# SociallyIneptWeeb/AICoverGen

Hardware: AMD Instinct MI355X
Metric: real-time factor (audio-sec/wall-sec) for MDX+RVC on 4-min 44.1 kHz track (higher is better)
Workload: dtype f32

## Files before the change

### aicovergen_amd/csrc/conv.hip

```cpp
#include <initializer_list>
#include "conv_ws3s.h"
#include "conv_ws3w.h"
#include "conv_w2d.h"
#include "conv_g1.h"
#include "conv_g1s.h"
#include "conv_g1w.h"
#ifdef AICG_DEV_SWITCHES
#include "conv_g1k.h"
#endif

namespace aicg {

#ifdef AICG_CONV_TRACE
__device__ unsigned long long g_conv_trace[kTraceWgs * kTraceSlots];
__device__ unsigned long long g_conv_trace2[kTrace2Wgs * 2 * 32 * 4];
#endif

template <bool FEW_IN>
__global__ void __launch_bounds__(256) conv_pointwise_kernel(ConvArgs p) {
    const long q = (long)blockIdx.x * 256 + threadIdx.x;
    const long per_img = (long)p.Ho * (p.Wo >> 2);
    if (q >= per_img) return;
    const int n = blockIdx.y;
    const int h = (int)(q / (p.Wo >> 2));
    const int w4 = (int)(q - (long)h * (p.Wo >> 2)) * 4;
    const float* xp = p.x + (long)n * p.x_sn + (long)h * p.x_sh + w4;
    float* yp = p.y + (long)n * p.y_sn + (long)h * p.y_sh + w4;
    const float* rp = p.res ? p.res + (long)n * p.r_sn + (long)h * p.r_sh + w4 : nullptr;
    auto finish = [&](float4 a, int co) __attribute__((always_inline)) {
        if (rp) {
            const float4 r = *reinterpret_cast<const float4*>(rp + (long)co * p.r_sc);
            if (p.res_first) { a.x += r.x; a.y += r.y; a.z += r.z; a.w += r.w; }
            a.x = apply_act(a.x, p.act, p.act_slope); a.y = apply_act(a.y, p.act, p.act_slope);
            a.z = apply_act(a.z, p.act, p.act_slope); a.w = apply_act(a.w, p.act, p.act_slope);
            if (!p.res_first) { a.x += r.x; a.y += r.y; a.z += r.z; a.w += r.w; }
        } else {
            a.x = apply_act(a.x, p.act, p.act_slope); a.y = apply_act(a.y, p.act, p.act_slope);
            a.z = apply_act(a.z, p.act, p.act_slope); a.w = apply_act(a.w, p.act, p.act_slope);
        }
        a.x *= p.out_scale; a.y *= p.out_scale; a.z *= p.out_scale; a.w *= p.out_scale;
        *reinterpret_cast<float4*>(yp + (long)co * p.y_sc) = a;
    };
    if (FEW_IN) {
        float4 xv[8];
#pragma unroll
        for (int ci = 0; ci < 8; ++ci)
            xv[ci] = ci < p.Cin_g ? *reinterpret_cast<const float4*>(xp + (long)ci * p.x_sc) : make_float4(0.f, 0.f, 0.f, 0.f);
        for (int co = 0; co < p.Cout_g; ++co) {
            const float b = p.bias ? p.bias[co] : 0.f;
            float4 a = make_float4(b, b, b, b);
#pragma unroll
            for (int ci = 0; ci < 8; ++ci) {
                if (ci < p.Cin_g) {
                    const float wv = p.w[ci * p.Mpad + co];
                    a.x += wv * xv[ci].x; a.y += wv * xv[ci].y; a.z += wv * xv[ci].z; a.w += wv * xv[ci].w;
                }
            }
            finish(a, co);
        }
    } else {
        float4 a[8];
#pragma unroll
        for (int co = 0; co < 8; ++co) {
            const float b = (p.bias && co < p.Cout_g) ? p.bias[co] : 0.f;
            a[co] = make_float4(b, b, b, b);
        }
        for (int ci = 0; ci < p.Cin_g; ++ci) {
            const float4 xv = *reinterpret_cast<const float4*>(xp + (long)ci * p.x_sc);
#pragma unroll
            for (int co = 0; co < 8; ++co) {
                if (co < p.Cout_g) {
                    const float wv = p.w[ci * p.Mpad + co];
                    a[co].x += wv * xv.x; a[co].y += wv * xv.y; a[co].z += wv * xv.z; a[co].w += wv * xv.w;
                }
            }
        }
#pragma unroll
        for (int co = 0; co < 8; ++co)
            if (co < p.Cout_g) finish(a[co], co);
    }
}

}

using namespace aicg;

#ifdef AICG_CONV_TRACE
extern "C" int aicg_conv_trace_read(unsigned long long* host, int clear) {
    (void)hipDeviceSynchronize();
    if (hipMemcpyFromSymbol(host, HIP_SYMBOL(g_conv_trace), sizeof(unsigned long long) * kTraceWgs * kTraceSlots) != hipSuccess)
        return fail(AICG_E_HIP, "trace copy failed");
    if (clear) { static unsigned long long z[kTraceWgs * kTraceSlots]; (void)hipMemcpyToSymbol(HIP_SYMBOL(g_conv_trace), z, sizeof(z)); }
    return AICG_OK;
}
extern "C" int aicg_conv_trace2_read(unsigned long long* host) {
    (void)hipDeviceSynchronize();
    if (hipMemcpyFromSymbol(host, HIP_SYMBOL(g_conv_trace2), sizeof(unsigned long long) * kTrace2Wgs * 2 * 32 * 4) != hipSuccess)
        return fail(AICG_E_HIP, "trace copy failed");
    return AICG_OK;
}
#endif

extern "C" int aicg_conv_bkc(int taps) {
    (void)taps;
    return 32;
}

extern "C" int aicg_conv_desc_size(void) { return (int)sizeof(aicg_conv_desc); }

namespace {

struct ConvCall {
    const aicg_conv_desc* d;
    int pad_h_end, pad_w_end;
    hipStream_t st;
};

typedef int (*run_fn)(ConvArgs&, hipStream_t);

int least_padded_bm(int M, std::initializer_list<int> cands) {
    int bm = 32;
    long best = 1L << 40;
    for (const int c : cands) {
        const long padded = (long)idiv_up(M, c) * c;
        if (padded < best) { best = padded; bm = c; }
    }
    return bm;
}

int validate_desc(const aicg_conv_desc* d, const float* x, const float* w_packed, const float* res, const float* y, ConvCall& c) {
    if (!d || !x || !w_packed || !y) return fail(AICG_E_ARG, "aicg_conv_forward: null pointer");
    if (d->groups < 1 || d->Cin % d->groups || d->Cout % d->groups)
        return fail(AICG_E_SHAPE, "aicg_conv_forward: channels not divisible by groups");
    if (d->KH < 1 || d->KW < 1 || d->stride_h < 1 || d->stride_w < 1 || d->dil_h < 1 || d->dil_w < 1)
        return fail(AICG_E_SHAPE, "aicg_conv_forward: bad kernel geometry");
    c.d = d;
    c.pad_h_end = d->pad_h_end < 0 ? d->pad_h : d->pad_h_end;
    c.pad_w_end = d->pad_w_end < 0 ? d->pad_w : d->pad_w_end;
    const int Ho = (d->H + d->pad_h + c.pad_h_end - d->dil_h * (d->KH - 1) - 1) / d->stride_h + 1;
    const int Wo = (d->W + d->pad_w + c.pad_w_end - d->dil_w * (d->KW - 1) - 1) / d->stride_w + 1;
    if (d->Ho > Ho || d->Wo > Wo || d->Ho < 0 || d->Wo < 0)
        return fail(AICG_E_SHAPE, "aicg_conv_forward: output %dx%d exceeds geometry (%dx%d)", d->Ho, d->Wo, Ho, Wo);
    if (d->N == 0 || d->Ho <= 0 || d->Wo <= 0) return AICG_OK;
    if (d->shuffle != 0 && (d->shuffle != 2 || d->Cout % 4 || d->groups != 1))
        return fail(AICG_E_ARG, "aicg_conv_forward: shuffle must be 0 or 2 (Cout %% 4 == 0, groups == 1)");
    if (d->res_mul && (!res || d->res_before_act)) return fail(AICG_E_ARG, "aicg_conv_forward: res_mul needs res and res_before_act == 0");
    return 1;
}

void fill_args(ConvArgs& p, const aicg_conv_desc* d, const float* x, const float* w_packed, const float* bias, const float* res, float* y) {
    p.stagger = p.stagger_first = p.wide_ok = 0;
    p.x = x; p.w = w_packed; p.bias = bias; p.res = res; p.y = y;
    p.N = d->N; p.Cin_g = d->Cin / d->groups; p.H = d->H; p.W = d->W; p.Cout_g = d->Cout / d->groups;
    p.Ho = d->Ho; p.Wo = d->Wo; p.KH = d->KH; p.KW = d->KW; p.sh = d->stride_h; p.sw = d->stride_w;
    p.ph = d->pad_h; p.pw = d->pad_w; p.dh = d->dil_h; p.dw = d->dil_w; p.groups = d->groups;
    p.x_sn = d->x_sn; p.x_sc = d->x_sc; p.x_sh = d->x_sh;
    p.y_sn = d->y_sn; p.y_sc = d->y_sc; p.y_sh = d->y_sh;
    p.r_sn = d->r_sn; p.r_sc = d->r_sc; p.r_sh = d->r_sh;
    p.pre_act = d->pre_act; p.pre_slope = d->pre_slope; p.act = d->act; p.act_slope = d->act_slope;
    p.out_scale = d->out_scale; p.accumulate = d->accumulate; p.res_first = d->res_before_act;
    p.shuffle = d->shuffle; p.res_mul = d->res_mul;
    p.taps = p.KH * p.KW;
    p.Mpad = idiv_up(p.Cout_g, 32) * 32;
    p.Cin_pad = idiv_up(p.Cin_g, 32) * 32;
    p.w_group_stride = (long)p.taps * p.Cin_pad * p.Mpad;
    p.w3 = d->packed_v3 ? w_packed + (long)p.groups * p.w_group_stride : nullptr;
    p.wsplit = d->packed_v3 && d->split == 1 ? w_packed + 2L * p.groups * p.w_group_stride : nullptr;
    p.f16 = d->split == 2;
}


int route_wino1d(ConvArgs& p, const ConvCall& c) {
    const aicg_conv_desc* d = c.d;
    if (d->wino != 8) return 1;
    if (!d->packed_v3 || (p.KW != 3 && p.KW != 5 && p.KW != 7 && p.KW != 11))
        return fail(AICG_E_ARG, "aicg_conv_forward: wino 8 needs a packed k = 3 / 5 / 7 / 11 one-dimensional layer");
    const int nslot = p.KW == 3 ? 4 : p.KW == 5 ? 7 : p.KW == 7 ? 10 : 15;
    p.w3 = p.w + (long)nslot * p.Cin_pad * p.Mpad;
    if (!conv_g1w_applicable(p, c.pad_w_end))
        return fail(AICG_E_ARG, "aicg_conv_forward: wino 8 needs stride 1, dilation 1 / 3 / 5, same padding, one group, W %% 4 == 0, 16-byte aligned "
                                "rows (strides %% 4 == 0), no input activation but a leaky ReLU");
    int rc;
    p.dbg = 0;
#ifdef AICG_DEV_SWITCHES
    p.dbg = d->gemm_tile == 7 ? 3 : 0;
    if (p.dw == 1 && d->gemm_tile == 2) rc = run_g1w_64x256(p, c.st);
    else if (p.dw == 1 && d->gemm_tile == 5) rc = run_g1w_32x512_sched(p, c.st);
    else if (p.dw == 1 && (d->gemm_tile == 6 || d->gemm_tile == 7)) rc = run_g1w_32x512_pers(p, c.st);
    else
#endif
        rc = p.f16 ? run_g1w_32x512_h(p, c.st) : run_g1w_32x512(p, c.st);
    if (rc == 1) return fail(AICG_E_SHAPE, "aicg_conv_forward: wino 8 layer does not fit the kernel's LDS budget");
    return rc;
}

int route_wino2d(ConvArgs& p, const ConvCall& c) {
    const aicg_conv_desc* d = c.d;
    AICG_SWITCH(w2d_ablate, "AICG_CONV_ABLATE", 0);
    p.dbg = w2d_ablate;
    p.w3 = p.w;
    if (w2d_ablate && (d->wino == 2 || d->wino == 12)) {
        const int ra = d->wino == 2 ? run_w2d_ablation(p, c.st, (int)w2d_ablate) : run_w2d_pairs_ablation(p, c.st, (int)w2d_ablate);
        if (ra != 1) return ra;
        return fail(AICG_E_ARG, "aicg_conv_forward: AICG_CONV_ABLATE=%ld is not an instantiated variant of conv_w2d (or not the dev library)", (long)w2d_ablate);
    }
#ifdef AICG_DEV_SWITCHES
    if (d->wino == 6) return run_w2d_ablation(p, c.st, 512);
    if (d->wino == 7) return run_w2d_ablation(p, c.st, 1024);
    if (d->wino == 9) return run_w2d_ablation(p, c.st, 2048);
    if (d->wino == 10) return run_w2d_ablation(p, c.st, 1);
    if (d->wino == 14) return run_w2d_pairs_ablation(p, c.st, 16384);
    if (d->wino == 15) return run_w2d_pairs_ablation(p, c.st, 65536);
    if (d->wino == 13) return run_w2d_pairs_ablation(p, c.st, 8192);
#endif
    const int rc = d->wino == 2 ? run_w2d_8(p, c.st) : d->wino == 3 ? run_w2d_4(p, c.st) : d->wino == 4 ? run_w2d_8q(p, c.st)
                 : d->wino == 12 ? run_w2d_8p(p, c.st) : d->wino == 16 ? run_w2d_4p2(p, c.st) : run_w2d_4q(p, c.st);
    if (rc == 1)
        return fail(AICG_E_ARG, "aicg_conv_forward: wino 2 needs Cout %% 48 == 0, W %% 4 == 0, 16-byte aligned x with strides %% 4 == 0");
    return rc;
}

int route_wino_rows(ConvArgs& p, const ConvCall& c) {
    AICG_SWITCH(wino_ablate, "AICG_CONV_ABLATE", 0);
    p.dbg = wino_ablate;
    p.taps = 12;
    p.w_group_stride = (long)p.taps * p.Cin_pad * p.Mpad;
    p.w3 = p.w + p.w_group_stride;
    const int M = p.Cout_g;
    AICG_SWITCH(wino_bm, "AICG_WINO_BM", 0);
    const int bm = wino_bm ? (int)wino_bm : least_padded_bm(M, {96, 64, 48, 32});
    auto run = [&](ConvArgs& a, int tile) {
        return tile == 96 ? run_ws3w_96(a, c.st) : tile == 64 ? run_ws3w_64(a, c.st) : tile == 48 ? run_ws3w_48(a, c.st) : run_ws3w_32(a, c.st);
    };
    int rc;
    AICG_SWITCH(wino_split, "AICG_WINO_SPLIT", 1);
    const long tiles4 = (long)p.N * idiv_up(p.Ho, 4) * idiv_up(p.Wo, 64);
    AICG_SWITCH(wino_split_tiles, "AICG_WINO_SPLIT_TILES", 1024);
    if (wino_split && !wino_bm && M > 48 && M % 96 == 48 && tiles4 >= wino_split_tiles) {
        ConvArgs a = p, b = p;
        a.Cout_g = M - 48;
        b.Cout_g = 48;
        if (b.bias) b.bias += M - 48;
        b.y += (long)(M - 48) * p.y_sc;
        b.w3 += (long)(M - 48) * 4;
        rc = run(a, 96);
        if (rc == 0) rc = run(b, 48);
    } else {
        rc = run(p, bm);
    }
    if (rc == 1) return fail(AICG_E_SHAPE, "aicg_conv_forward: wino layer too large for the kernel's 32-bit offsets");
    return rc;
}

int route_wino(ConvArgs& p, const ConvCall& c) {
    const aicg_conv_desc* d = c.d;
    if (!d->wino) return 1;
    if (p.KH != 3 || p.KW != 3 || p.sh != 1 || p.sw != 1 || p.dh != 1 || p.dw != 1 || p.ph != 1 || p.pw != 1 || c.pad_h_end != 1 ||
        c.pad_w_end != 1 || p.groups != 1 || p.res || p.accumulate || p.shuffle || p.res_mul || p.pre_act != AICG_ACT_NONE ||
        p.out_scale != 1.f || (!d->packed_v3 && d->wino < 2) || (p.act != AICG_ACT_NONE && p.act != AICG_ACT_RELU) || p.Ho != p.H || p.Wo != p.W)
        return fail(AICG_E_ARG, "aicg_conv_forward: wino needs a plain 3x3 / stride 1 / padding 1 layer (bias + none|ReLU epilogue)");
    return d->wino >= 2 ? route_wino2d(p, c) : route_wino_rows(p, c);
}


int route_pointwise(ConvArgs& p, const ConvCall& c) {
    AICG_SWITCH(pointwise, "AICG_CONV_POINTWISE", 1);
    const bool few_in = p.Cin_g <= 8, few_out = p.Cout_g <= 8;
    auto al4 = [](long v) { return (v & 3) == 0; };
    const bool aligned = (p.Wo & 3) == 0 && al4(p.x_sn) && al4(p.x_sc) && al4(p.x_sh) && al4(p.y_sn) && al4(p.y_sc) && al4(p.y_sh) &&
                         (!p.res || (al4(p.r_sn) && al4(p.r_sc) && al4(p.r_sh) && ((uintptr_t)p.res & 15) == 0)) &&
                         ((uintptr_t)p.x & 15) == 0 && ((uintptr_t)p.y & 15) == 0;
    if (!(pointwise && p.taps == 1 && p.groups == 1 && p.sh == 1 && p.sw == 1 && p.ph == 0 && p.pw == 0 && c.pad_h_end == 0 &&
          c.pad_w_end == 0 && (few_in || few_out) && p.Cin_g <= 512 && p.Cout_g <= 512 && p.pre_act == AICG_ACT_NONE &&
          !p.accumulate && aligned && p.Ho == p.H && p.Wo == p.W && !p.shuffle && !p.res_mul))
        return 1;
    const long per_img = (long)p.Ho * (p.Wo >> 2);
    dim3 grid((unsigned)ldiv_up(per_img, 256), (unsigned)p.N);
    if (few_in) hipLaunchKernelGGL(HIP_KERNEL_NAME(conv_pointwise_kernel<true>), grid, dim3(256), 0, c.st, p);
    else hipLaunchKernelGGL(HIP_KERNEL_NAME(conv_pointwise_kernel<false>), grid, dim3(256), 0, c.st, p);
    return check_launch("conv_pointwise_kernel");
}

int route_g1(ConvArgs& p, const ConvCall& c) {
    AICG_SWITCH(g1env, "AICG_CONV_G1", 0);
    const long g1 = c.d->gemm_tile ? c.d->gemm_tile : g1env;
    if (!(g1 != 1 && !p.wsplit && p.Cout_g > 32 && conv_g1_applicable(p, c.pad_h_end, c.pad_w_end))) return 1;
    const long HW = (long)p.H * p.W;
    const int M = p.Cout_g;
    auto wgs = [&](int bm) { return (long)p.N * idiv_up(M, bm) * ldiv_up(HW, 256); };
    if (p.f16 && !p.shuffle) {
        const long t64 = wgs(64), t128 = wgs(128);
        if (g1 == 3 || (g1 != 2 && ldiv_up(t64, 768) * 64 < ldiv_up(t128, 512) * 128)) return run_g1_64x256_h(p, c.st);
        return run_g1_128x256_h(p, c.st);
    }
    if (g1 == 2) return run_g1_128x256(p, c.st);
    if (g1 == 3) return run_g1_64x256(p, c.st);
    if (g1 == 4) return run_g1_192x256(p, c.st);
#ifdef AICG_DEV_SWITCHES
    if (g1 == 5) return run_g1_256x256(p, c.st);
    if (g1 == 6) return run_g1_128x512(p, c.st);
    if (g1 >= 12 && g1 <= 14) return run_g1_burst(p, c.st, (int)g1 - 10);
#endif
    if (wgs(64) < 256) return 1;
    auto cost = [&](int bm, double f) { return (double)ldiv_up(wgs(bm), 256) * bm * f; };
    const double c64 = cost(64, 1.04), c128 = cost(128, 1.0);
    const double c192 = (M % 192 == 0 && p.Cin_g >= 256) ? cost(192, 0.98) : 1e30;
    if (c192 <= c64 && c192 <= c128) return run_g1_192x256(p, c.st);
    if (c128 <= c64) return run_g1_128x256(p, c.st);
    return run_g1_64x256(p, c.st);
}

int route_g1s(ConvArgs& p, const ConvCall& c) {
    const int tile = c.d->gemm_tile;
    if (!(tile != 1 && !p.wsplit && p.Cout_g > 32 && conv_g1s_applicable(p, c.pad_w_end))) return 1;
    const long w64 = (long)p.N * idiv_up(p.Cout_g, 64) * idiv_up(p.Wo, 256);
    if (tile == 2) return run_g1s_128x256(p, c.st);
    if (tile == 3 || w64 >= 160) return run_g1s_64x256(p, c.st);
    return 1;
}

#ifdef AICG_DEV_SWITCHES
int route_g1k(ConvArgs& p, const ConvCall& c) {
    const int tile = c.d->gemm_tile;
    if (tile != 12 && tile != 13) return 1;
    if (!(!p.wsplit && p.Cout_g > 32 && conv_g1k_applicable(p, c.pad_w_end))) return 1;
    return tile == 12 ? run_g1k_128x256(p, c.st) : run_g1k_64x256(p, c.st);
}
#endif


struct TilePlan {
    int M, BM, groups;
    long npos, want;
    hipStream_t st;
    long blocks(int bm, int bn) const { return (long)idiv_up(M, bm) * groups * ldiv_up(npos, bn); }
    bool fills(int bm, int bn) const { return blocks(bm, bn) >= want; }
};

TilePlan plan_tiles(ConvArgs& p, const ConvCall& c) {
    TilePlan t;
    t.M = p.Cout_g;
    t.BM = least_padded_bm(t.M, {160, 128, 96, 64, 32});
    AICG_SWITCH(force_bm, "AICG_CONV_FORCE_BM", 0);
    if (force_bm) t.BM = (int)force_bm;
    t.groups = p.groups;
    t.npos = (long)p.N * p.Ho * p.Wo;
    t.st = c.st;
    AICG_SWITCH(ablate, "AICG_CONV_ABLATE", 0);
    p.dbg = ablate;
    AICG_SWITCH(want, "AICG_CONV_WANT", 512);
    t.want = want;
    return t;
}

int small_tiles(ConvArgs& p, const TilePlan& t, run_fn r64x64, run_fn r32x256, run_fn r32x128) {
    if (t.M > 32) return !t.fills(64, 128) && (t.fills(64, 64) || t.M > 64) ? r64x64(p, t.st) : 1;
    return t.fills(32, 256) ? r32x256(p, t.st) : r32x128(p, t.st);
}

int route_ws3s(ConvArgs& p, const TilePlan& t) {
    const int M = t.M;
    if (!(p.wsplit && p.Cin_g >= 16 && M > 16)) return 1;
    const int bm = least_padded_bm(M, {128, 96, 64, 32});
    int rc = 1;
    if (bm == 128 && t.fills(128, 128)) rc = run_ws3s_128x128(p, t.st);
    else if (bm == 96 && t.fills(96, 128)) rc = run_ws3s_96x128(p, t.st);
    else if (M > 32) {
        if (t.fills(64, 256)) rc = run_ws3s_64x256(p, t.st);
        if (rc == 1 && t.fills(64, 128)) rc = run_ws3s_64x128(p, t.st);
    }
    if (rc == 1) {
        rc = small_tiles(p, t, run_ws3s_64x64, run_ws3s_32x256, run_ws3s_32x128);
        if (rc == 1 && M <= 32 && t.fills(32, 256)) rc = run_ws3s_32x128(p, t.st);
    }
    return rc;
}

int route_m16(ConvArgs& p, const TilePlan& t) {
    const int M = t.M;
    AICG_SWITCH(use16, "AICG_CONV_M16", 1);
    if (!(use16 && t.npos >= 256L * 256)) return 1;
    const bool rows48 = M > 32 && M <= 48, rows16 = M <= 16;
    AICG_SWITCH(v3m16, "AICG_CONV_V3M16", 0);
#ifdef AICG_DEV_SWITCHES
    if (v3m16 && p.w3 && p.Cin_g >= 16) {
        const int rc = rows48 ? run_ws3m16_48(p, t.st) : rows16 ? run_ws3m16_16(p, t.st) : 1;
        if (rc <= 0) return rc;
    }
#else
    (void)v3m16;
#endif
    AICG_SWITCH(m16h, "AICG_CONV_M16H", 1);
    if (m16h && p.w3 && p.Cin_g >= 8) {
        const int rc = rows48 ? run_ws3m16h_48(p, t.st) : rows16 ? run_ws3m16h_16(p, t.st) : 1;
        if (rc <= 0) return rc;
    }
    if (p.Cin_g >= 3) return rows48 ? run_m16_48(p, t.st) : rows16 ? run_m16_16(p, t.st) : 1;
    return 1;
}

int route_ws3(ConvArgs& p, const TilePlan& t) {
    const int M = t.M, BM = t.BM;
    AICG_SWITCH(ws, "AICG_CONV_WS", 1);
    AICG_SWITCH(v3, "AICG_CONV_V3", 1);
    if (!(ws && v3 && p.w3 && p.Cin_g >= 8)) return 1;
    int rc = 1;
    AICG_SWITCH(v3_160, "AICG_CONV_V3_160", 1);
    if (BM == 160 && v3_160 && !p.shuffle && !p.res_mul && t.fills(160, 128)) rc = run_ws3_160x128(p, t.st);
    else if (BM == 128 && t.fills(128, 128)) rc = run_ws3_128x128(p, t.st);
    else if (BM == 96 && t.fills(96, 128)) rc = run_ws3_96x128(p, t.st);
    else if (BM != 160 && M > 32 && t.fills(64, 128)) rc = run_ws3_64x128(p, t.st);
    if (rc == 1 && BM != 160) rc = small_tiles(p, t, run_ws3_64x64, run_ws3_32x256, run_ws3_32x128);
    return rc;
}

int route_ws(ConvArgs& p, const TilePlan& t) {
    const int M = t.M, BM = t.BM;
    AICG_SWITCH(ws, "AICG_CONV_WS", 1);
    if (!ws) return 1;
    int rc = 1;
    AICG_SWITCH(v2, "AICG_CONV_V2", 0);
#ifdef AICG_DEV_SWITCHES
    if (v2 & 1) { if (BM == 128 && t.fills(128, 128)) rc = run_ws_128x128_k32(p, t.st); }
    if (rc == 1 && (v2 & 2)) { if (M > 32 && M <= 64 && t.fills(64, 256)) rc = run_ws_64x256(p, t.st); }
    if (rc == 1 && (v2 & 4)) { if (M <= 32 && t.fills(32, 512)) rc = run_ws_32x512(p, t.st); }
    if (rc <= 0) return rc;
#else
    (void)v2;
#endif
    if (BM == 160 && t.fills(160, 128)) rc = run_ws_160x128(p, t.st);
    else if (BM == 128 && t.fills(128, 128)) {
        AICG_SWITCH(bm128e, "AICG_CONV_BM128", 0);
        const bool use64 = bm128e ? bm128e == 64 : M >= 256;
        rc = use64 ? run_ws_64x128(p, t.st) : run_ws_128x128(p, t.st);
    }
    else if (BM == 96 && t.fills(96, 128)) rc = run_ws_96x128(p, t.st);
    else if (M > 32 && t.fills(64, 128)) rc = run_ws_64x128(p, t.st);
    if (rc <= 0) return rc;
    AICG_SWITCH(smallws, "AICG_CONV_SMALLWS", 1);
    return smallws ? small_tiles(p, t, run_ws_64x64, run_ws_32x256, run_ws_32x128) : 1;
}

int route_single_role(ConvArgs& p, const TilePlan& t) {
    const int M = t.M, BM = t.BM;
    AICG_SWITCH(eight, "AICG_CONV_8WAVE", 1);
    auto tile = [&]() -> int {
        if (BM == 160 && t.fills(160, 128)) return run_sr_160x128(p, t.st);
#ifdef AICG_DEV_SWITCHES
        if (BM == 128 && t.fills(128, 128) && !eight) return run_sr_128x128_4w(p, t.st);
#else
        (void)eight;
#endif
        if (BM == 128 && t.fills(128, 128)) return run_sr_128x128_8w(p, t.st);
        if (BM == 96 && t.fills(96, 128)) return run_sr_96x128(p, t.st);
        if (M > 32) {
            if (t.fills(64, 128)) return run_sr_64x128(p, t.st);
            if (t.fills(64, 64) || M > 64) return run_sr_64x64(p, t.st);
        }
        if (t.fills(32, 256)) return run_sr_32x256(p, t.st);
        return run_sr_32x128(p, t.st);
    };
    int rc = tile();
    if (rc == AICG_E_LDS) rc = run_sr_64x64(p, t.st);
    return rc;
}

}

extern "C" int aicg_conv_forward(const aicg_conv_desc* d, const float* x, const float* w_packed, const float* bias,
                                 const float* res, float* y, void* stream) {
    ConvCall c;
    int rc = validate_desc(d, x, w_packed, res, y, c);
    if (rc <= 0) return rc;
    c.st = (hipStream_t)stream;
    ConvArgs p;
    fill_args(p, d, x, w_packed, bias, res, y);
    if ((rc = route_wino1d(p, c)) != 1) return rc;
    if ((rc = route_wino(p, c)) != 1) return rc;
    if ((rc = route_pointwise(p, c)) != 1) return rc;
    if ((rc = route_g1(p, c)) != 1) return rc;
    if ((rc = route_g1s(p, c)) != 1) return rc;
#ifdef AICG_DEV_SWITCHES
    if ((rc = route_g1k(p, c)) != 1) return rc;
#endif
    const TilePlan t = plan_tiles(p, c);
    if ((rc = route_ws3s(p, t)) != 1) return rc;
    if ((rc = route_m16(p, t)) != 1) return rc;
    if ((rc = route_ws3(p, t)) != 1) return rc;
    if ((rc = route_ws(p, t)) != 1) return rc;
    return route_single_role(p, t);
}
```

### aicovergen_amd/csrc/elementwise.hip

```cpp
#include "common.h"

#include <cstdint>

namespace aicg {

struct Col2imArgs {
    const float* cols;
    const float* bias;
    const float* add;
    float* out;
    int N, Cout, Hi, Wi, Ho, Wo, KH, KW, sh, sw, ph, pw, act;
    float slope;
    long o_sn, o_sc, o_sh, a_sn, a_sc, a_sh;
};

__global__ void __launch_bounds__(256) col2im_kernel(Col2imArgs p) {
    const long total = (long)p.N * p.Cout * p.Ho * p.Wo;
    const long plane = (long)p.Hi * p.Wi;
    for (long i = (long)blockIdx.x * blockDim.x + threadIdx.x; i < total; i += (long)gridDim.x * blockDim.x) {
        const int wo = (int)(i % p.Wo);
        long t = i / p.Wo;
        const int ho = (int)(t % p.Ho);
        t /= p.Ho;
        const int co = (int)(t % p.Cout);
        const int n = (int)(t / p.Cout);
        float acc = p.bias ? p.bias[co] : 0.f;
        const float* cn = p.cols + (long)n * p.Cout * p.KH * p.KW * plane;
        for (int kh = (ho + p.ph) % p.sh; kh < p.KH; kh += p.sh) {
            const int hi = (ho + p.ph - kh) / p.sh;
            if (ho + p.ph - kh < 0) break;
            if (hi >= p.Hi) continue;
            for (int kw = (wo + p.pw) % p.sw; kw < p.KW; kw += p.sw) {
                const int wi = (wo + p.pw - kw) / p.sw;
                if (wo + p.pw - kw < 0) break;
                if (wi >= p.Wi) continue;
                acc += cn[((long)(co * p.KH + kh) * p.KW + kw) * plane + (long)hi * p.Wi + wi];
            }
        }
        acc = apply_act(acc, p.act, p.slope);
        if (p.add) acc += p.add[(long)n * p.a_sn + (long)co * p.a_sc + (long)ho * p.a_sh + wo];
        p.out[(long)n * p.o_sn + (long)co * p.o_sc + (long)ho * p.o_sh + wo] = acc;
    }
}

template <int S>
__global__ void __launch_bounds__(256) col2im1d_kernel(Col2imArgs p, int J) {
    HIP_DYNAMIC_SHARED(float, c2i_tile)
    const int s = S > 0 ? S : p.sw;
    const int co = blockIdx.y, n = blockIdx.z, tid = threadIdx.x;
    const int q0 = blockIdx.x * 256, q = q0 + tid;
    const float* cn = p.cols + ((long)n * p.Cout + co) * p.KW * (long)p.Wi;
    const float b = p.bias ? p.bias[co] : 0.f;
#pragma unroll 2
    for (int r = 0; r < s; ++r) {
        float acc = b;
        for (int j = 0; j < J; ++j) {
            const int kk = r + s * j, qi = q - j;
            if (kk < p.KW && qi >= 0 && qi < p.Wi) acc += cn[(long)kk * p.Wi + qi];
        }
        c2i_tile[tid * s + r] = apply_act(acc, p.act, p.slope);
    }
    __syncthreads();
    const long nbase = (long)s * q0 - p.pw;
    float* orow = p.out + (long)n * p.o_sn + (long)co * p.o_sc;
    const float* arow = p.add ? p.add + (long)n * p.a_sn + (long)co * p.a_sc : nullptr;
    for (int i = tid; i < 256 * s; i += 256) {
        const long no = nbase + i;
        if (no >= 0 && no < p.Wo) orow[no] = c2i_tile[i] + (arow ? arow[no] : 0.f);
    }
}

__global__ void __launch_bounds__(256) sine_frame_prefix_kernel(const float* __restrict__ f0, double* __restrict__ prefix,
                                                                int T, int upp, float sr) {
    __shared__ double part[256];
    const int tid = threadIdx.x;
    const int per = (T + 255) / 256;
    const int t0 = tid * per, t1 = imin(T, t0 + per);
    double s = 0.0;
    for (int t = t0; t < t1; ++t) {
        const float rad = fmodf(f0[t] / sr, 1.0f);
        s += (double)rad * (double)upp;
        s -= floor(s);
    }
    part[tid] = s;
    __syncthreads();
    if (tid == 0) {
        double run = 0.0;
        for (int i = 0; i < 256; ++i) {
            const double v = part[i];
            part[i] = run;
            run += v;
            run -= floor(run);
        }
    }
    __syncthreads();
    double run = part[tid];
    for (int t = t0; t < t1; ++t) {
        prefix[t] = run;
        const float rad = fmodf(f0[t] / sr, 1.0f);
        run += (double)rad * (double)upp;
        run -= floor(run);
    }
}

__global__ void __launch_bounds__(256) sine_source4_kernel(const float* __restrict__ f0, const double* __restrict__ prefix,
                                                           const float* __restrict__ noise, float* __restrict__ out,
                                                           int T, int upp, float sr, float sine_amp, float noise_std,
                                                           float lin_w, float lin_b) {
    const int q_per = upp >> 2;
    const long total4 = (long)T * q_per;
    for (long n4 = (long)blockIdx.x * blockDim.x + threadIdx.x; n4 < total4; n4 += (long)gridDim.x * blockDim.x) {
        const int t = (int)(n4 / q_per);
        const int i0 = (int)(n4 - (long)t * q_per) * 4;
        const float f = f0[t];
        const float rad = fmodf(f / sr, 1.0f);
        const double base = prefix[t];
        const float uv = f > 0.f ? 1.f : 0.f;
        const float namp = uv * noise_std + (1.f - uv) * sine_amp / 3.f;
        const float4 nz = *reinterpret_cast<const float4*>(noise + (long)t * upp + i0);
        const float nv[4] = {nz.x, nz.y, nz.z, nz.w};
        float o[4];
#pragma unroll
        for (int j = 0; j < 4; ++j) {
            double ph = base + (double)(i0 + j + 1) * (double)rad;
            ph -= floor(ph);
            const float sine = sinf((float)(ph * 6.283185307179586476925)) * sine_amp;
            const float v = sine * uv + namp * nv[j];
            o[j] = tanhf(lin_w * v + lin_b);
        }
        *reinterpret_cast<float4*>(out + (long)t * upp + i0) = make_float4(o[0], o[1], o[2], o[3]);
    }
}

__global__ void __launch_bounds__(256) sine_source_kernel(const float* __restrict__ f0, const double* __restrict__ prefix,
                                                          const float* __restrict__ noise, float* __restrict__ out,
                                                          int T, int upp, float sr, float sine_amp, float noise_std,
                                                          float lin_w, float lin_b) {
    const long total = (long)T * upp;
    for (long n = (long)blockIdx.x * blockDim.x + threadIdx.x; n < total; n += (long)gridDim.x * blockDim.x) {
        const int t = (int)(n / upp);
        const int i = (int)(n - (long)t * upp);
        const float f = f0[t];
        const float rad = fmodf(f / sr, 1.0f);
        double ph = prefix[t] + (double)(i + 1) * (double)rad;
        ph -= floor(ph);
        const float sine = sinf((float)(ph * 6.283185307179586476925)) * sine_amp;
        const float uv = f > 0.f ? 1.f : 0.f;
        const float namp = uv * noise_std + (1.f - uv) * sine_amp / 3.f;
        const float v = sine * uv + namp * noise[n];
        out[n] = tanhf(lin_w * v + lin_b);
    }
}

__global__ void __launch_bounds__(256) gate_kernel(const float* __restrict__ a, float* __restrict__ out, int N, int C,
                                                   long T) {
    const long total = (long)N * C * T;
    for (long i = (long)blockIdx.x * blockDim.x + threadIdx.x; i < total; i += (long)gridDim.x * blockDim.x) {
        const long t = i % T;
        const long nc = i / T;
        const int c = (int)(nc % C);
        const long n = nc / C;
        const float ta = a[(n * 2 * C + c) * T + t];
        const float sa = a[(n * 2 * C + C + c) * T + t];
        out[i] = tanhf(ta) * (1.f / (1.f + expf(-sa)));
    }
}

__global__ void __launch_bounds__(256) prior_sample_kernel(const float* __restrict__ stats, const float* __restrict__ noise,
                                                           float* __restrict__ out, int C, long T, float scale) {
    const long total = (long)C * T;
    for (long i = (long)blockIdx.x * blockDim.x + threadIdx.x; i < total; i += (long)gridDim.x * blockDim.x) {
        const float m = stats[i], logs = stats[total + i];
        out[i] = m + expf(logs) * noise[i] * scale;
    }
}

__global__ void __launch_bounds__(256) feats_prepare_kernel(const float* __restrict__ feats, const float* __restrict__ feats0,
                                                            const float* __restrict__ pitchf, float* __restrict__ out,
                                                            int Th, int C, int T, float protect) {
    __shared__ float tile[32][33];
    const int t0 = blockIdx.x * 32, c0 = blockIdx.y * 32;
    const int tx = threadIdx.x & 31, ty = threadIdx.x >> 5;
    for (int r = ty; r < 32; r += 8) {
        const int t = t0 + r, c = c0 + tx;
        float v = 0.f;
        if (t < T && c < C) {
            const int th = imin(t >> 1, Th - 1);
            v = feats[(long)th * C + c];
            if (feats0) {
                const float f = pitchf[t];
                float pf = f;
                if (f > 0.f) pf = 1.f;
                if (f < 1.f) pf = protect;
                v = v * pf + feats0[(long)th * C + c] * (1.f - pf);
            }
        }
        tile[r][tx] = v;
    }
    __syncthreads();
    for (int r = ty; r < 32; r += 8) {
        const int c = c0 + r, t = t0 + tx;
        if (c < C && t < T) out[(long)c * T + t] = tile[tx][r];
    }
}

static unsigned ew_grid(long total) { return (unsigned)lmax(1, lmin((total + 255) / 256, 256L * 16)); }

}

using namespace aicg;

extern "C" int aicg_col2im(const float* cols, const float* bias, const float* add, float* out, int N, int Cout, int Hi,
                           int Wi, int Ho, int Wo, int KH, int KW, int stride_h, int stride_w, int pad_h, int pad_w,
                           int act, float slope, int64_t o_sn, int64_t o_sc, int64_t o_sh, int64_t a_sn, int64_t a_sc,
                           int64_t a_sh, void* stream) {
    if (!cols || !out) return fail(AICG_E_ARG, "aicg_col2im: null pointer");
    if (KH < 1 || KW < 1 || stride_h < 1 || stride_w < 1) return fail(AICG_E_SHAPE, "aicg_col2im: bad geometry");
    const long total = (long)N * Cout * Ho * Wo;
    if (total == 0) return AICG_OK;
    Col2imArgs p{cols, bias, add, out, N, Cout, Hi, Wi, Ho, Wo, KH, KW, stride_h, stride_w, pad_h, pad_w, act, slope,
                 (long)o_sn, (long)o_sc, (long)o_sh, (long)a_sn, (long)a_sc, (long)a_sh};
    if (Hi == 1 && Ho == 1 && KH == 1 && stride_h == 1 && pad_h == 0 && Cout <= 65535 && N <= 65535 && stride_w <= 32) {
        const int J = (KW + stride_w - 1) / stride_w;
        const long nq = ((long)Wo + pad_w + stride_w - 1) / stride_w + 1;
        dim3 grid((unsigned)ldiv_up(nq, 256), (unsigned)Cout, (unsigned)N);
        const size_t lds = (size_t)256 * stride_w * sizeof(float);
        if (stride_w == 2) hipLaunchKernelGGL(HIP_KERNEL_NAME(col2im1d_kernel<2>), grid, dim3(256), lds, (hipStream_t)stream, p, J);
        else if (stride_w == 10) hipLaunchKernelGGL(HIP_KERNEL_NAME(col2im1d_kernel<10>), grid, dim3(256), lds, (hipStream_t)stream, p, J);
        else hipLaunchKernelGGL(HIP_KERNEL_NAME(col2im1d_kernel<0>), grid, dim3(256), lds, (hipStream_t)stream, p, J);
        return check_launch("col2im1d_kernel");
    }
    hipLaunchKernelGGL(col2im_kernel, dim3(ew_grid(total)), dim3(256), 0, (hipStream_t)stream, p);
    return check_launch("col2im_kernel");
}

extern "C" int aicg_sine_source(const float* f0, const float* noise, double* prefix_scratch, float* out, int T, int upp,
                                float sr, float sine_amp, float noise_std, float lin_w, float lin_b, void* stream) {
    if (!f0 || !noise || !prefix_scratch || !out) return fail(AICG_E_ARG, "aicg_sine_source: null pointer");
    if (T < 0 || upp < 1) return fail(AICG_E_SHAPE, "aicg_sine_source: bad shape");
    if (T == 0) return AICG_OK;
    hipLaunchKernelGGL(sine_frame_prefix_kernel, dim3(1), dim3(256), 0, (hipStream_t)stream, f0, prefix_scratch, T, upp, sr);
    if ((upp & 3) == 0 && ((uintptr_t)noise & 15) == 0 && ((uintptr_t)out & 15) == 0)
        hipLaunchKernelGGL(sine_source4_kernel, dim3(ew_grid((long)T * (upp >> 2))), dim3(256), 0, (hipStream_t)stream, f0,
                           (const double*)prefix_scratch, noise, out, T, upp, sr, sine_amp, noise_std, lin_w, lin_b);
    else
        hipLaunchKernelGGL(sine_source_kernel, dim3(ew_grid((long)T * upp)), dim3(256), 0, (hipStream_t)stream, f0,
                           (const double*)prefix_scratch, noise, out, T, upp, sr, sine_amp, noise_std, lin_w, lin_b);
    return check_launch("sine_source_kernel");
}

extern "C" int aicg_gate_tanh_sigmoid(const float* a, float* out, int N, int C, int64_t T, void* stream) {
    if (!a || !out) return fail(AICG_E_ARG, "aicg_gate_tanh_sigmoid: null pointer");
    const long total = (long)N * C * T;
    if (total == 0) return AICG_OK;
    hipLaunchKernelGGL(gate_kernel, dim3(ew_grid(total)), dim3(256), 0, (hipStream_t)stream, a, out, N, C, (long)T);
    return check_launch("gate_kernel");
}

extern "C" int aicg_prior_sample(const float* stats, const float* noise, float* out, int C, int64_t T, float scale,
                                 void* stream) {
    if (!stats || !noise || !out) return fail(AICG_E_ARG, "aicg_prior_sample: null pointer");
    if ((long)C * T == 0) return AICG_OK;
    hipLaunchKernelGGL(prior_sample_kernel, dim3(ew_grid((long)C * T)), dim3(256), 0, (hipStream_t)stream, stats, noise,
                       out, C, (long)T, scale);
    return check_launch("prior_sample_kernel");
}

extern "C" int aicg_feats_prepare(const float* feats, const float* feats0, const float* pitchf, float* out, int Th, int C,
                                  int T, float protect, void* stream) {
    if (!feats || !out || (feats0 && !pitchf)) return fail(AICG_E_ARG, "aicg_feats_prepare: null pointer");
    if (T > 2 * Th) return fail(AICG_E_SHAPE, "aicg_feats_prepare: T=%d exceeds 2*Th=%d", T, 2 * Th);
    if (T == 0 || C == 0) return AICG_OK;
    dim3 grid((unsigned)idiv_up(T, 32), (unsigned)idiv_up(C, 32));
    hipLaunchKernelGGL(feats_prepare_kernel, grid, dim3(256), 0, (hipStream_t)stream, feats, feats0, pitchf, out, Th, C, T,
                       protect);
    return check_launch("feats_prepare_kernel");
}

namespace aicg {
__global__ void __launch_bounds__(256) mul_kernel(const float* __restrict__ a, const float* __restrict__ b, float* __restrict__ out, long n) {
    for (long i = (long)blockIdx.x * blockDim.x + threadIdx.x; i < n; i += (long)gridDim.x * blockDim.x) out[i] = a[i] * b[i];
}
__global__ void __launch_bounds__(256) axpbypcz_kernel(const float* __restrict__ a, float alpha, const float* __restrict__ b,
                                                       float beta, const float* __restrict__ c, float gamma,
                                                       float* __restrict__ out, long n) {
    for (long i = (long)blockIdx.x * blockDim.x + threadIdx.x; i < n; i += (long)gridDim.x * blockDim.x) {
        float v = alpha * a[i];
        if (b) v += beta * b[i];
        if (c) v += gamma * c[i];
        out[i] = v;
    }
}
}

extern "C" int aicg_mul(const float* a, const float* b, float* out, int64_t n, void* stream) {
    if (!a || !b || !out) return aicg::fail(AICG_E_ARG, "aicg_mul: null pointer");
    if (n == 0) return AICG_OK;
    hipLaunchKernelGGL(aicg::mul_kernel, dim3(aicg::ew_grid(n)), dim3(256), 0, (hipStream_t)stream, a, b, out, (long)n);
    return aicg::check_launch("mul_kernel");
}

extern "C" int aicg_axpbypcz(const float* a, float alpha, const float* b, float beta, const float* c, float gamma, float* out,
                             int64_t n, void* stream) {
    if (!a || !out) return aicg::fail(AICG_E_ARG, "aicg_axpbypcz: null pointer");
    if (n == 0) return AICG_OK;
    hipLaunchKernelGGL(aicg::axpbypcz_kernel, dim3(aicg::ew_grid(n)), dim3(256), 0, (hipStream_t)stream, a, alpha, b, beta, c,
                       gamma, out, (long)n);
    return aicg::check_launch("axpbypcz_kernel");
}

namespace aicg {
__global__ void __launch_bounds__(256) frame_normalize_kernel(const float* __restrict__ x, float* __restrict__ out, int L) {
    __shared__ float sh[4];
    const float* xr = x + (long)blockIdx.x * L;
    float s = 0.f;
    for (int i = threadIdx.x; i < L; i += 256) s += xr[i];
    for (int o = 32; o > 0; o >>= 1) s += __shfl_xor(s, o);
    if ((threadIdx.x & 63) == 0) sh[threadIdx.x >> 6] = s;
    __syncthreads();
    const float mean = (sh[0] + sh[1] + sh[2] + sh[3]) / (float)L;
    __syncthreads();
    float v = 0.f;
    for (int i = threadIdx.x; i < L; i += 256) { const float d = xr[i] - mean; v += d * d; }
    for (int o = 32; o > 0; o >>= 1) v += __shfl_xor(v, o);
    if ((threadIdx.x & 63) == 0) sh[threadIdx.x >> 6] = v;
    __syncthreads();
    const float sd = fmaxf(1e-10f, sqrtf((sh[0] + sh[1] + sh[2] + sh[3]) / (float)(L - 1)));
    float* orow = out + (long)blockIdx.x * L;
    for (int i = threadIdx.x; i < L; i += 256) orow[i] = (xr[i] - mean) / sd;
}

__global__ void __launch_bounds__(256) affine_maxpool2_kernel(const float* __restrict__ x, const float* __restrict__ scale,
                                                              const float* __restrict__ shift, float* __restrict__ out, int C,
                                                              int Wo, long total) {
    for (long i = (long)blockIdx.x * blockDim.x + threadIdx.x; i < total; i += (long)gridDim.x * blockDim.x) {
        const int c = (int)((i / Wo) % C);
        const float s = scale[c], t = shift[c];
        const float a = x[2 * i] * s + t, b = x[2 * i + 1] * s + t;
        out[i] = fmaxf(a, b);
    }
}
}

extern "C" int aicg_frame_normalize(const float* x, float* out, int64_t n_frames, int frame_len, void* stream) {
    if (!x || !out) return aicg::fail(AICG_E_ARG, "aicg_frame_normalize: null pointer");
    if (frame_len < 2) return aicg::fail(AICG_E_SHAPE, "aicg_frame_normalize: frame too short");
    if (n_frames <= 0) return AICG_OK;
    hipLaunchKernelGGL(aicg::frame_normalize_kernel, dim3((unsigned)n_frames), dim3(256), 0, (hipStream_t)stream, x, out, frame_len);
    return aicg::check_launch("frame_normalize_kernel");
}

extern "C" int aicg_affine_maxpool2(const float* x, const float* scale, const float* shift, float* out, int N, int C, int W,
                                    void* stream) {
    if (!x || !scale || !shift || !out) return aicg::fail(AICG_E_ARG, "aicg_affine_maxpool2: null pointer");
    if (W & 1) return aicg::fail(AICG_E_SHAPE, "aicg_affine_maxpool2: W must be even");
    const long total = (long)N * C * (W / 2);
    if (total == 0) return AICG_OK;
    hipLaunchKernelGGL(aicg::affine_maxpool2_kernel, dim3(aicg::ew_grid(total)), dim3(256), 0, (hipStream_t)stream, x, scale, shift,
                       out, C, W / 2, total);
    return aicg::check_launch("affine_maxpool2_kernel");
}
```

### aicovergen_amd/infer_pack/models.py

```python
import contextlib
import math
import os
from collections import namedtuple

import numpy as np
import torch
from .. import _env
import torch.nn.functional as F

from .. import ops

_Incompatible = namedtuple("IncompatibleKeys", ["missing_keys", "unexpected_keys"])
LRELU_SLOPE = 0.1

sr2sr = {"32k": 32000, "40k": 40000, "48k": 48000}


def _fold_weight_norm(sd, name):
    if name + ".weight" in sd:
        return sd[name + ".weight"].float()
    v, g = sd[name + ".weight_v"].float(), sd[name + ".weight_g"].float()
    return v * (g / v.flatten(1).norm(dim=1).view(-1, *([1] * (v.dim() - 1))))


class _SynthesizerBase:
    phone_dim = 768
    use_f0 = True

    def __init__(self, spec_channels, segment_size, inter_channels, hidden_channels, filter_channels, n_heads,
                 n_layers, kernel_size, p_dropout, resblock, resblock_kernel_sizes, resblock_dilation_sizes,
                 upsample_rates, upsample_initial_channel, upsample_kernel_sizes, spk_embed_dim, gin_channels, sr=None,
                 **kwargs):
        if isinstance(sr, str):
            sr = sr2sr[sr]
        self.spec_channels, self.segment_size = spec_channels, segment_size
        self.inter_channels, self.hidden_channels, self.filter_channels = inter_channels, hidden_channels, filter_channels
        self.n_heads, self.n_layers, self.kernel_size, self.p_dropout = n_heads, n_layers, kernel_size, p_dropout
        self.resblock = str(resblock)
        self.resblock_kernel_sizes = list(resblock_kernel_sizes)
        self.resblock_dilation_sizes = [list(d) for d in resblock_dilation_sizes]
        self.upsample_rates = list(upsample_rates)
        self.upsample_initial_channel = upsample_initial_channel
        self.upsample_kernel_sizes = list(upsample_kernel_sizes)
        self.spk_embed_dim, self.gin_channels = spk_embed_dim, gin_channels
        self.sr = sr
        self.upp = int(np.prod(self.upsample_rates))
        self.is_half = bool(kwargs.get("is_half", False))
        self.enc_q = None
        self.device = torch.device("cpu")
        self._sd = None
        self._p = None
        assert kernel_size % 2 == 1, "FFN same-padding is symmetric only for odd kernels"
        print("gin_channels:", gin_channels, "self.spk_embed_dim:", self.spk_embed_dim)

    def load_state_dict(self, state_dict, strict=True):
        self._sd = {k: v.detach().to("cpu") for k, v in state_dict.items() if not k.startswith("enc_q.")}
        self._p = None
        unexpected = [k for k in state_dict if k.startswith("enc_q.")] if strict else []
        return _Incompatible([], unexpected)

    def eval(self):
        return self

    def to(self, device):
        self.device = torch.device(device)
        self._p = None
        return self

    def half(self):
        self._half = ops.half_requested()
        if self._p is not None:
            ops.mark_half(self._p, self._half)
        return self

    def float(self):
        self._half = False
        if self._p is not None:
            ops.mark_half(self._p, False)
        return self

    def remove_weight_norm(self):
        return None

    def _prepare(self):
        if self._p is not None:
            return self._p
        assert self._sd is not None, "load_state_dict() first"
        sd, dev = self._sd, self.device
        P = {}
        H, C = self.n_heads, self.hidden_channels
        dk = C // H
        P["emb_phone"] = ops.PackedConv(sd["enc_p.emb_phone.weight"].float(), sd["enc_p.emb_phone.bias"], device=dev)
        if self.use_f0:
            P["emb_pitch"] = sd["enc_p.emb_pitch.weight"].float().to(dev)
        layers = []
        for i in range(self.n_layers):
            a = "enc_p.encoder.attn_layers.%d." % i
            L = {}
            L["q"] = ops.PackedConv(sd[a + "conv_q.weight"].float(), sd[a + "conv_q.bias"], device=dev)
            L["kv"] = ops.PackedConv(torch.cat([sd[a + "conv_k.weight"], sd[a + "conv_v.weight"]], 0).float(),
                                     torch.cat([sd[a + "conv_k.bias"], sd[a + "conv_v.bias"]], 0), device=dev)
            ek = sd[a + "emb_rel_k"].float()
            ev = sd[a + "emb_rel_v"].float()
            assert ek.shape[0] == 1, "heads_share=True is the only configuration the reference instantiates"
            self.window = (ek.shape[1] - 1) // 2
            L["relk"] = ops.PackedConv(ek[0].repeat(H, 1).unsqueeze(-1).contiguous(), None, groups=H, device=dev)
            L["relv"] = ev[0].contiguous().to(dev)
            L["o"] = ops.PackedConv(sd[a + "conv_o.weight"].float(), sd[a + "conv_o.bias"], device=dev)
            for n in (1, 2):
                L["g%d" % n] = sd["enc_p.encoder.norm_layers_%d.%d.gamma" % (n, i)].float().to(dev)
                L["b%d" % n] = sd["enc_p.encoder.norm_layers_%d.%d.beta" % (n, i)].float().to(dev)
            f = "enc_p.encoder.ffn_layers.%d." % i
            pad = (self.kernel_size - 1) // 2
            L["ffn1"] = ops.PackedConv(sd[f + "conv_1.weight"].float(), sd[f + "conv_1.bias"], padding=pad, device=dev)
            L["ffn2"] = ops.PackedConv(sd[f + "conv_2.weight"].float(), sd[f + "conv_2.bias"], padding=pad, device=dev)
            layers.append(L)
        P["enc_layers"] = layers
        P["proj"] = ops.PackedConv(sd["enc_p.proj.weight"].float(), sd["enc_p.proj.bias"], device=dev)
        P["emb_g"] = sd["emb_g.weight"].float().to(dev)
        flows = {}
        for fidx in (0, 2, 4, 6):
            p = "flow.flows.%d." % fidx
            Fl = {"pre": ops.PackedConv(sd[p + "pre.weight"].float(), sd[p + "pre.bias"], device=dev)}
            n_wn = 0
            while (p + "enc.in_layers.%d.weight_v" % n_wn) in sd or (p + "enc.in_layers.%d.weight" % n_wn) in sd:
                n_wn += 1
            Fl["n_wn"] = n_wn
            in_bias = []
            for l in range(n_wn):
                w = _fold_weight_norm(sd, p + "enc.in_layers.%d" % l)
                Fl["in%d" % l] = ops.PackedConv(w, None, padding=(w.shape[2] - 1) // 2, device=dev)
                in_bias.append(sd[p + "enc.in_layers.%d.bias" % l].float())
                rs_w = _fold_weight_norm(sd, p + "enc.res_skip_layers.%d" % l)
                rs_b = sd[p + "enc.res_skip_layers.%d.bias" % l].float()
                if l < n_wn - 1:
                    Fl["res%d" % l] = ops.PackedConv(rs_w[:C], rs_b[:C], device=dev)
                    Fl["skip%d" % l] = ops.PackedConv(rs_w[C:], rs_b[C:], device=dev)
                else:
                    Fl["skip%d" % l] = ops.PackedConv(rs_w, rs_b, device=dev)
            Fl["cond"] = ops.PackedConv(_fold_weight_norm(sd, p + "enc.cond_layer"), sd[p + "enc.cond_layer.bias"], device=dev)
            Fl["in_bias"] = torch.cat(in_bias).view(1, -1, 1).contiguous().to(dev)
            Fl["post_neg"] = ops.PackedConv(-sd[p + "post.weight"].float(), -sd[p + "post.bias"].float(), device=dev)
            flows[fidx] = Fl
        P["flows"] = flows
        up_init = self.upsample_initial_channel
        P["conv_pre"] = ops.PackedConv(sd["dec.conv_pre.weight"].float(), None, padding=3, device=dev)
        P["conv_pre_bias"] = sd["dec.conv_pre.bias"].float().view(1, -1, 1).contiguous().to(dev)
        P["cond"] = ops.PackedConv(sd["dec.cond.weight"].float(), sd["dec.cond.bias"], device=dev)
        ups, noise = [], []
        for i, (u, k) in enumerate(zip(self.upsample_rates, self.upsample_kernel_sizes)):
            ups.append(ops.PackedConvTranspose(_fold_weight_norm(sd, "dec.ups.%d" % i), sd["dec.ups.%d.bias" % i], stride=u,
                                               padding=(k - u) // 2, device=dev))
            if self.use_f0:
                w, b = sd["dec.noise_convs.%d.weight" % i].float(), sd["dec.noise_convs.%d.bias" % i]
                cc = w.shape[0]
                if i + 1 < len(self.upsample_rates):
                    s = int(np.prod(self.upsample_rates[i + 1:]))
                    assert w.shape[2] == 2 * s
                    w2 = w.view(cc, 2, s).permute(0, 2, 1).contiguous()
                    noise.append((s, ops.PackedConv(w2, b, device=dev)))
                else:
                    noise.append((1, ops.PackedConv(w, b, device=dev)))
        P["ups"], P["noise"] = ups, noise
        rbs = []
        nres = len(self.upsample_rates) * len(self.resblock_kernel_sizes)
        for j in range(nres):
            k = self.resblock_kernel_sizes[j % len(self.resblock_kernel_sizes)]
            dil = self.resblock_dilation_sizes[j % len(self.resblock_kernel_sizes)]
            r = "dec.resblocks.%d." % j
            convs = []
            if self.resblock == "1":
                for m, d in enumerate(dil):
                    c1 = ops.PackedConv(_fold_weight_norm(sd, r + "convs1.%d" % m), sd[r + "convs1.%d.bias" % m], dilation=d,
                                        padding=(k * d - d) // 2, device=dev)
                    c2 = ops.PackedConv(_fold_weight_norm(sd, r + "convs2.%d" % m), sd[r + "convs2.%d.bias" % m],
                                        padding=(k - 1) // 2, device=dev)
                    convs.append((c1, c2))
            else:
                for m, d in enumerate(dil):
                    convs.append((ops.PackedConv(_fold_weight_norm(sd, r + "convs.%d" % m), sd[r + "convs.%d.bias" % m],
                                                 dilation=d, padding=(k * d - d) // 2, device=dev), None))
            rbs.append(convs)
        P["resblocks"] = rbs
        P["conv_post"] = ops.PackedConv(sd["dec.conv_post.weight"].float(), None, padding=3, device=dev)
        if self.use_f0:
            P["lin_w"] = float(sd["dec.m_source.l_linear.weight"].reshape(-1)[0])
            P["lin_b"] = float(sd["dec.m_source.l_linear.bias"].reshape(-1)[0])
        if getattr(self, "_half", False):
            ops.mark_half(P, True)
        self._p = P
        return P

    def _enc_p(self, P, phone_ct, pitch):
        C, H = self.hidden_channels, self.n_heads
        dk = C // H
        T = phone_ct.shape[2]
        res = None
        if pitch is not None:
            res = P["emb_pitch"][pitch[0]].t().contiguous().unsqueeze(0)
        x = ops.conv(phone_ct, P["emb_phone"], res=res, res_before_act=True, act=ops.ACT_LRELU, act_slope=0.1,
                     out_scale=math.sqrt(C))
        for L in P["enc_layers"]:
            q = ops.conv(x, L["q"], out_scale=1.0 / math.sqrt(dk))
            kv = ops.conv(x, L["kv"])
            relk = ops.conv(q, L["relk"])
            o = ops.attention(q[0], kv[0, :C], kv[0, C:], H, relk=relk[0].view(H, 2 * self.window + 1, T),
                              relv_emb=L["relv"], window=self.window)
            y = ops.conv(o.unsqueeze(0), L["o"])
            x = ops.layernorm_ct(x, L["g1"], L["b1"], res=y)
            y = ops.conv(x, L["ffn1"], act=ops.ACT_RELU)
            y = ops.conv(y, L["ffn2"])
            x = ops.layernorm_ct(x, L["g2"], L["b2"], res=y)
        return ops.conv(x, P["proj"])

    def _flow_reverse(self, P, z, g):
        C = self.hidden_channels
        half = self.inter_channels // 2
        for fidx in (6, 4, 2, 0):
            Fl = P["flows"][fidx]
            z = torch.flip(z, [1])
            x0, x1 = z[:, :half], z[:, half:]
            h = ops.conv(x0, Fl["pre"])
            bias_all = ops.conv(g, Fl["cond"], res=Fl["in_bias"])
            out = None
            for l in range(Fl["n_wn"]):
                a = ops.conv(h, Fl["in%d" % l], bias=bias_all[0, 2 * C * l: 2 * C * (l + 1), 0].contiguous())
                acts = ops.gate_tanh_sigmoid(a)
                if l < Fl["n_wn"] - 1:
                    if out is None:
                        out = ops.conv(acts, Fl["skip%d" % l])
                    else:
                        ops.conv(acts, Fl["skip%d" % l], out=out, accumulate=True)
                    ops.conv(acts, Fl["res%d" % l], res=h, out=h)
                else:
                    if out is None:
                        out = ops.conv(acts, Fl["skip%d" % l])
                    else:
                        ops.conv(acts, Fl["skip%d" % l], out=out, accumulate=True)
            ops.conv(out, Fl["post_neg"], res=x1, out=x1)
        return z

    def _decoder(self, P, x, f0, g, noise_src):
        T = x.shape[2]
        har = None
        if self.use_f0:
            if noise_src is None:
                noise_src = torch.randn(T * self.upp, device=x.device)
            har = ops.sine_source(f0.reshape(-1)[:T], noise_src.to(x.device).reshape(-1), self.upp, float(self.sr), P["lin_w"], P["lin_b"])
        pre_bias = ops.conv(g, P["cond"], res=P["conv_pre_bias"])
        x = ops.conv(x, P["conv_pre"], bias=pre_bias.reshape(-1))
        nk = len(self.resblock_kernel_sizes)
        for i, pt in enumerate(P["ups"]):
            add = None
            if har is not None:
                s, nc = P["noise"][i]
                L = har.numel()
                if s > 1:
                    xp = F.pad(har, (s // 2, s // 2))
                    phases = xp.view(L // s + 1, s).t().contiguous()
                    add = ops.conv(phases.unsqueeze(0), nc)
                else:
                    add = ops.conv(har.view(1, 1, L), nc)
            x = ops.conv_transpose(x, pt, add=add, pre_act=ops.ACT_LRELU, pre_slope=LRELU_SLOPE)
            acc = torch.empty_like(x)
            streams = self._rb_streams(x.device, nk)
            main = torch.cuda.current_stream(x.device) if streams else None
            bufs = [tuple(torch.empty_like(x) for _ in range(3)) for _ in range(nk if streams else 1)]
            if streams:
                ready = torch.cuda.Event()
                ready.record(main)
            prev_acc = None
            for j in range(nk):
                convs = P["resblocks"][i * nk + j]
                st = streams[j - 1] if (streams and j > 0) else main
                if streams and j > 0:
                    st.wait_event(ready)
                with (torch.cuda.stream(st) if streams else contextlib.nullcontext()):
                    tmp, ya, yb = bufs[j] if streams else bufs[0]
                    y = x
                    for m, (c1, c2) in enumerate(convs):
                        last = m == len(convs) - 1
                        if c2 is None:
                            src = c1
                            inp = y
                        else:
                            ops.conv(y, c1, out=tmp, pre_act=ops.ACT_LRELU, pre_slope=LRELU_SLOPE, act=ops.ACT_LRELU, act_slope=LRELU_SLOPE)
                            src, inp = c2, tmp
                        if last:
                            if streams and prev_acc is not None:
                                st.wait_event(prev_acc)
                            pre = ops.ACT_NONE if c2 is not None else ops.ACT_LRELU
                            ops.conv(inp, src, res=y, out=acc, pre_act=pre, pre_slope=LRELU_SLOPE, out_scale=1.0 / nk, accumulate=j > 0)
                            if streams:
                                prev_acc = torch.cuda.Event()
                                prev_acc.record(st)
                        else:
                            dst = ya if y is not ya else yb
                            ops.conv(inp, src, res=y, out=dst, pre_act=ops.ACT_NONE if c2 is not None else ops.ACT_LRELU, pre_slope=LRELU_SLOPE)
                            y = dst
            if streams:
                main.wait_event(prev_acc)
            x = acc
        return ops.conv(x, P["conv_post"], pre_act=ops.ACT_LRELU, pre_slope=0.01, act=ops.ACT_TANH)

    def _rb_streams(self, device, nk):
        if device.type != "cuda" or nk < 2 or _env.dev("AICG_RB_STREAMS", "0") != "1":
            return None
        have = getattr(self, "_rb_side", None)
        if have is None or len(have) != nk - 1:
            have = self._rb_side = [torch.cuda.Stream(device=device) for _ in range(nk - 1)]
        return have

    def infer(self, phone, phone_lengths, pitch=None, nsff0=None, sid=None, max_len=None, noise_z=None, noise_src=None,
              phone_ct=None):
        if not self.use_f0 and sid is None:
            sid, pitch = pitch, None
        P = self._prepare()
        dev = self.device
        if phone_ct is None:
            phone = phone.to(dev).float()
            assert phone.shape[0] == 1, "batch 1 (the reference pipeline never batches chunks)"
            T = phone.shape[1]
            phone_ct = phone[0].t().contiguous().unsqueeze(0)
        else:
            T = phone_ct.shape[2]
        front = self.infer_front(phone_ct, pitch, sid, noise_z)
        return self.infer_back(front, nsff0, noise_src, max_len)

    def infer_front(self, phone_ct, pitch, sid, noise_z=None):
        P = self._prepare()
        dev = self.device
        T = phone_ct.shape[2]
        g = P["emb_g"][sid.to(dev).reshape(-1)[:1]].unsqueeze(-1).contiguous()
        stats = self._enc_p(P, phone_ct, None if pitch is None else pitch.to(dev))
        if noise_z is None:
            noise_z = torch.randn((1, self.inter_channels, T), device=dev)
        z_p = ops.prior_sample(stats, noise_z.to(dev).float().contiguous(), 0.66666)
        z = self._flow_reverse(P, z_p.clone(), g)
        return {"z": z, "z_p": z_p, "stats": stats, "g": g, "T": T}

    def infer_back(self, front, nsff0=None, noise_src=None, max_len=None):
        P = self._prepare()
        dev = self.device
        z, z_p, stats, g, T = front["z"], front["z_p"], front["stats"], front["g"], front["T"]
        zz = z if max_len is None else z[:, :, :max_len].contiguous()
        o = self._decoder(P, zz, None if nsff0 is None else nsff0.to(dev).float(), g, noise_src)
        x_mask = torch.ones((1, 1, T), dtype=torch.float32, device=dev)
        m_p, logs_p = stats[:, : self.inter_channels], stats[:, self.inter_channels:]
        return o, x_mask, (z, z_p, m_p, logs_p)


class SynthesizerTrnMs768NSFsid(_SynthesizerBase):
    phone_dim, use_f0 = 768, True


class SynthesizerTrnMs256NSFsid(_SynthesizerBase):
    phone_dim, use_f0 = 256, True


class SynthesizerTrnMs768NSFsid_nono(_SynthesizerBase):
    phone_dim, use_f0 = 768, False


class SynthesizerTrnMs256NSFsid_nono(_SynthesizerBase):
    phone_dim, use_f0 = 256, False
```

### aicovergen_amd/ops.py

```python
import contextlib
import functools
import math
import os
import threading

import numpy as np
import torch
from . import _env

from . import _lib


def _ptr(t):
    return 0 if t is None else t.data_ptr()


def _stream(t):
    if t.is_cuda:
        return torch.cuda.current_stream(t.device).cuda_stream
    return 0


_tls = threading.local()


def _check(*tensors):
    be = _lib.backend()
    dev = None
    for t in tensors:
        if t is None:
            continue
        if be == "hip" and not t.is_cuda:
            raise RuntimeError("aicovergen_amd: tensor on %s, but the HIP kernels need device memory" % t.device)
        if be == "emu" and t.is_cuda:
            raise RuntimeError("emulator backend needs host tensors")
        if t.is_cuda:
            if dev is None:
                dev = t.device.index
            elif dev != t.device.index:
                raise RuntimeError("aicovergen_amd: operands on different devices (cuda:%d and cuda:%d)" % (dev, t.device.index))
    _tls.dev = dev


def _call(name, *args):
    dev = getattr(_tls, "dev", None)
    if dev is not None and dev != torch.cuda.current_device():
        with torch.cuda.device(dev):
            return _lib.call(name, *args)
    return _lib.call(name, *args)


_fft_tables = {}


def fft_tables(n_fft, device, window=None):
    key = (n_fft, str(device))
    if key not in _fft_tables:
        m = n_fft // 2
        k = np.arange(m, dtype=np.float64)
        th = np.exp(-2j * np.pi * k / m)
        k2 = np.arange(m + 1, dtype=np.float64)
        tf = np.exp(-2j * np.pi * k2 / n_fft)
        tw_half = torch.from_numpy(np.stack([th.real, th.imag], -1).astype(np.float32)).contiguous().to(device)
        tw_full = torch.from_numpy(np.stack([tf.real, tf.imag], -1).astype(np.float32)).contiguous().to(device)
        hann = torch.hann_window(n_fft, periodic=True, dtype=torch.float32).to(device)
        _fft_tables[key] = (hann, tw_half, tw_full)
    hann, tw_half, tw_full = _fft_tables[key]
    if window is None:
        window = hann
    return window, tw_half, tw_full


def stft(x, n_fft, hop, n_bins_out=None, frame_major=False, window=None):
    assert x.dim() == 2 and x.dtype == torch.float32
    x = x.contiguous()
    n_sig, L = x.shape
    n_frames = 1 + L // hop
    nb = n_fft // 2 + 1 if n_bins_out is None else n_bins_out
    window, tw_half, tw_full = fft_tables(n_fft, x.device, window)
    _check(x, window)
    if frame_major:
        out = torch.empty((n_sig, 2, n_frames, nb), dtype=torch.float32, device=x.device)
        o_bin, o_frame = 1, nb
    else:
        out = torch.empty((n_sig, 2, nb, n_frames), dtype=torch.float32, device=x.device)
        o_bin, o_frame = n_frames, 1
    _call("aicg_stft", _ptr(x), _ptr(out), _ptr(window), _ptr(tw_half), _ptr(tw_full), n_sig, L, n_fft, hop,
              n_frames, nb, 2 * nb * n_frames, nb * n_frames, o_bin, o_frame, _stream(x))
    return out


def istft(spec, n_fft, hop, length, frame_major=False, window=None):
    assert spec.dim() == 4 and spec.shape[1] == 2 and spec.dtype == torch.float32
    spec = spec.contiguous()
    n_sig = spec.shape[0]
    if frame_major:
        n_frames, nb = spec.shape[2], spec.shape[3]
        i_bin, i_frame = 1, nb
    else:
        nb, n_frames = spec.shape[2], spec.shape[3]
        i_bin, i_frame = n_frames, 1
    window, tw_half, tw_full = fft_tables(n_fft, spec.device, window)
    _check(spec, window)
    frames = torch.empty((n_sig, n_frames, n_fft), dtype=torch.float32, device=spec.device)
    out = torch.empty((n_sig, length), dtype=torch.float32, device=spec.device)
    st = _stream(spec)
    _call("aicg_istft_frames", _ptr(spec), _ptr(frames), _ptr(window), _ptr(tw_half), _ptr(tw_full), n_sig,
              n_fft, n_frames, nb, 2 * nb * n_frames, nb * n_frames, i_bin, i_frame, st)
    _call("aicg_istft_ola", _ptr(frames), _ptr(window), _ptr(out), n_sig, length, n_fft, hop, n_frames, st)
    return out


import ctypes

ACT_NONE, ACT_RELU, ACT_LRELU, ACT_GELU, ACT_TANH, ACT_SIGMOID = 0, 1, 2, 3, 4, 5


class ConvDesc(ctypes.Structure):
    _fields_ = [(n, ctypes.c_int32) for n in
                ("N", "Cin", "H", "W", "Cout", "Ho", "Wo", "KH", "KW", "stride_h", "stride_w", "pad_h", "pad_w",
                 "dil_h", "dil_w", "groups")] + \
               [(n, ctypes.c_int64) for n in ("x_sn", "x_sc", "x_sh", "y_sn", "y_sc", "y_sh", "r_sn", "r_sc", "r_sh")] + \
               [("pre_act", ctypes.c_int32), ("pre_slope", ctypes.c_float), ("act", ctypes.c_int32),
                ("act_slope", ctypes.c_float), ("out_scale", ctypes.c_float), ("accumulate", ctypes.c_int32),
                ("res_before_act", ctypes.c_int32), ("pad_h_end", ctypes.c_int32), ("pad_w_end", ctypes.c_int32),
                ("shuffle", ctypes.c_int32), ("res_mul", ctypes.c_int32), ("packed_v3", ctypes.c_int32),
                ("split", ctypes.c_int32), ("wino", ctypes.c_int32), ("gemm_tile", ctypes.c_int32)]


def conv_bkc(taps):
    return _lib.get().aicg_conv_bkc(int(taps))


split_precision = os.environ.get("AICG_PRECISION", "fp32").lower() in ("bf16x3", "split")


def half_requested():
    return os.environ.get("AICG_HALF", "0") == "1"


def mark_half(tree, on=True):
    if isinstance(tree, PackedConv):
        tree.f16 = bool(on) and not tree.fp32_only and not tree.split
    elif isinstance(tree, PackedConvTranspose):
        mark_half(tree.gemm, on)
    elif isinstance(tree, dict):
        for v in tree.values():
            mark_half(v, on)
    elif isinstance(tree, (list, tuple)):
        for v in tree:
            mark_half(v, on)


_fp32_depth = 0


@contextlib.contextmanager
def fp32_layers():
    global split_precision, _fp32_depth
    old, split_precision = split_precision, False
    _fp32_depth += 1
    try:
        yield
    finally:
        split_precision = old
        _fp32_depth -= 1


def fp32_only(fn):
    @functools.wraps(fn)
    def wrapped(*a, **k):
        with fp32_layers():
            return fn(*a, **k)
    return wrapped


def _split_image(out):
    g, taps, cpad, mpad = out.shape
    hi = out.to(torch.bfloat16)
    lo = (out - hi.to(torch.float32)).to(torch.bfloat16)
    both = torch.stack([hi, lo], 0)
    both = both.reshape(2, g, taps, cpad // 16, 2, 8, mpad).permute(1, 2, 3, 0, 4, 6, 5).contiguous()
    return both.view(torch.int16).reshape(-1).view(torch.float32)


def pack_conv_weight(w, groups=1, split=False):
    w = w.detach().to(torch.float32)
    cout, cin_g, kh, kw = w.shape
    taps = kh * kw
    cpad = (cin_g + 31) // 32 * 32
    cout_g = cout // groups
    mpad = (cout_g + 31) // 32 * 32
    out = torch.zeros((groups, taps, cpad, mpad), dtype=torch.float32, device=w.device)
    out[:, :, :cin_g, :cout_g] = w.reshape(groups, cout_g, cin_g, taps).permute(0, 3, 2, 1)
    v3 = out.reshape(groups, taps, cpad // 8, 4, 2, mpad).permute(0, 1, 2, 4, 5, 3)
    parts = [out.reshape(-1), v3.reshape(-1)]
    if split:
        parts.append(_split_image(out))
    return torch.cat(parts).contiguous()


winograd = _env.dev("AICG_WINOGRAD", "1") != "0"
winograd_min_positions = 32768


def winograd_kernel(w):
    g0, g1, g2 = w[..., 0], w[..., 1], w[..., 2]
    return torch.stack([g0, (g0 + g1 + g2) * 0.5, (g0 - g1 + g2) * 0.5, g2], -1).contiguous()


winograd2d = _env.dev("AICG_WINOGRAD", "2") == "2"
winograd2d_waves = int(_env.dev("AICG_W2D_WAVES", "8"))


winograd2d_code = int(_env.dev("AICG_W2D_CODE", "0"))
winograd2d_quads = _env.dev("AICG_W2D_QUADS", "0") == "1"
winograd2d_pairs = _env.dev("AICG_W2D_PAIRS", "1") != "0"


def _w2d_code():
    code = winograd2d_code or ((4 if winograd2d_quads else 12 if winograd2d_pairs else 2) if winograd2d_waves == 8
                               else (5 if winograd2d_quads else 3))
    return code, ("pairs" if code in (12, 13, 14, 15, 16) else "quads" if code in (4, 5) else "dword")


def winograd2d_image(w, quads=False, pairs=False):
    co, ci = w.shape[:2]
    assert co % 48 == 0 and tuple(w.shape[2:]) == (3, 3)
    G = torch.tensor([[1.0, 0.0, 0.0], [0.5, 0.5, 0.5], [0.5, -0.5, 0.5], [0.0, 0.0, 1.0]], dtype=torch.float64, device=w.device)
    U = torch.einsum("ia,ocab,jb->ocij", G, w.double(), G).to(torch.float32)
    cpad = (ci + 7) // 8 * 8
    Up = torch.zeros((co, cpad, 16), dtype=torch.float32, device=w.device)
    Up[:, :ci] = U.reshape(co, ci, 16)
    if quads:
        return Up.view(co // 48, 48, cpad // 8, 2, 4, 4, 4).permute(0, 2, 3, 5, 4, 1, 6).contiguous().view(-1)
    if pairs:
        return Up.view(co // 48, 48, cpad // 8, 2, 4, 8, 2).permute(0, 2, 3, 5, 4, 1, 6).contiguous().view(-1)
    return Up.view(co // 48, 48, cpad // 8, 2, 4, 16).permute(0, 2, 3, 5, 4, 1).contiguous().view(-1)


winograd1d = _env.dev("AICG_WINOGRAD1D", "1") != "0"
winograd1d_min_positions = int(_env.dev("AICG_WINOGRAD1D_MIN", "16384"))


def winograd1d_kernel(w):
    k = w.shape[-1]
    assert k in (3, 5, 7, 11)
    wd = w.detach().double()
    slots = []
    for g in range(k // 3):
        g0, g1, g2 = wd[..., 3 * g], wd[..., 3 * g + 1], wd[..., 3 * g + 2]
        slots += [g0, (g0 + g1 + g2) * 0.5, (g0 - g1 + g2) * 0.5, g2]
    if k % 3 == 2:
        a, b = wd[..., k - 2], wd[..., k - 1]
        slots += [a, a + b, b]
    elif k % 3 == 1:
        a = wd[..., k - 1]
        slots += [a, -a]
    return torch.stack(slots, -1).to(torch.float32).contiguous()


class PackedConv:

    def __init__(self, weight, bias=None, stride=1, padding=0, dilation=1, groups=1, device=None, padding_end=None):
        self.padding_end = None if padding_end is None else (0, _one(padding_end)) if weight.dim() == 3 else _pair(padding_end)
        if weight.dim() == 3:
            weight = weight.unsqueeze(2)
            stride, padding, dilation = (1, _one(stride)), (0, _one(padding)), (1, _one(dilation))
        elif weight.dim() == 2:
            weight = weight[:, :, None, None]
            stride, padding, dilation = (1, 1), (0, 0), (1, 1)
        else:
            stride, padding, dilation = _pair(stride), _pair(padding), _pair(dilation)
        self.cout, cin_g, self.kh, self.kw = weight.shape
        self.cin = cin_g * groups
        self.groups = groups
        self.stride, self.padding, self.dilation = stride, padding, dilation
        device = weight.device if device is None else device
        self.split = bool(split_precision)
        self.fp32_only = _fp32_depth > 0
        self.f16 = False
        self.w = pack_conv_weight(weight.to(device), groups, self.split)
        self.bias = None if bias is None else bias.detach().to(device=device, dtype=torch.float32).contiguous()
        self.w_wino = self.w_wino2 = self.w_wino1 = None
        if (winograd1d and not self.split and not _fp32_depth and self.kh == 1 and self.kw in (3, 5, 7, 11) and stride == (1, 1)
                and dilation[1] in ((1, 3, 5) if self.kw != 5 else (1,)) and padding == (0, (self.kw - 1) // 2 * dilation[1]) and self.padding_end is None
                and groups == 1 and cin_g >= 16):
            self.w_wino1 = pack_conv_weight(winograd1d_kernel(weight.detach().to(device=device, dtype=torch.float32)[:, :, 0]).unsqueeze(2), 1, False)
        if (winograd and not self.split and not _fp32_depth and (self.kh, self.kw) == (3, 3) and stride == (1, 1) and dilation == (1, 1)
                and padding == (1, 1) and self.padding_end is None and groups == 1 and cin_g >= 8):
            self.w_wino = pack_conv_weight(winograd_kernel(weight.detach().to(device=device, dtype=torch.float32)), 1, False)
            if winograd2d and self.cout % 48 == 0:
                self._wino2_src, self._wino2_dev, self._wino2_images = weight.detach(), device, {}
                self.w_wino2 = self.wino2_image(_w2d_code()[1])

    def wino2_image(self, kind):
        if kind not in self._wino2_images:
            self._wino2_images[kind] = winograd2d_image(self._wino2_src.to(device=self._wino2_dev, dtype=torch.float32),
                                                         quads=kind == "quads", pairs=kind == "pairs")
        return self._wino2_images[kind]

    def wino2q(self):
        return self.wino2_image("quads")

    def out_hw(self, h, w):
        pe = self.padding if self.padding_end is None else self.padding_end
        ho = (h + self.padding[0] + pe[0] - self.dilation[0] * (self.kh - 1) - 1) // self.stride[0] + 1
        wo = (w + self.padding[1] + pe[1] - self.dilation[1] * (self.kw - 1) - 1) // self.stride[1] + 1
        return ho, wo


def _one(v):
    return int(v[0]) if isinstance(v, (tuple, list)) else int(v)


def _pair(v):
    return (int(v[0]), int(v[1])) if isinstance(v, (tuple, list)) else (int(v), int(v))


def _as4d(t):
    return t.unsqueeze(2) if t.dim() == 3 else t


class ConvProfile:

    def __init__(self):
        self.events = []
        self.flops = 0.0
        self.flops_executed = 0.0
        self.bytes = 0.0
        self.launches = 0
        self.shapes = []

    def by_shape(self):
        torch.cuda.synchronize()
        agg = {}
        for (key, fl), (a, b) in zip(self.shapes, self.events):
            r = agg.setdefault(key, [0, 0.0, 0.0])
            r[0] += 1
            r[1] += a.elapsed_time(b)
            r[2] += fl
        rows = [{"shape": k, "launches": v[0], "ms": v[1], "gflop": v[2] / 1e9, "tflops": v[2] / (v[1] * 1e-3) / 1e12 if v[1] > 0 else 0.0}
                for k, v in agg.items()]
        return sorted(rows, key=lambda r: -r["ms"])

    def summary(self):
        torch.cuda.synchronize()
        ms = sum(a.elapsed_time(b) for a, b in self.events)
        return {"launches": self.launches, "flops": self.flops, "flops_executed": self.flops_executed, "ms": ms, "bytes": self.bytes,
                "tflops": (self.flops / (ms * 1e-3) / 1e12) if ms > 0 else 0.0,
                "tflops_executed": (self.flops_executed / (ms * 1e-3) / 1e12) if ms > 0 else 0.0}


conv_profile = None

gemm_tile = 0


def conv(x, pc, res=None, out=None, pre_act=ACT_NONE, pre_slope=0.0, act=ACT_NONE, act_slope=0.0, out_scale=1.0,
         accumulate=False, bias=None, res_before_act=False, out_len=None, shuffle=0, res_mul=False):
    is1d = x.dim() == 3
    x4 = _as4d(x)
    n, c, h, w = x4.shape
    assert c == pc.cin, "conv: input has %d channels, layer expects %d" % (c, pc.cin)
    assert x4.stride(3) == 1 or w == 1
    assert h == 1 or c == 1 or x4.stride(1) >= x4.stride(2) * (h - 1) + w, "conv: input rows must lie inside the channel stride"
    ho, wo = pc.out_hw(h, w)
    if out_len is not None:
        assert out_len <= wo
        wo = out_len
    oshape = (n, pc.cout // 4, 2 * ho, 2 * wo) if shuffle else (n, pc.cout, ho, wo)
    if out is None:
        out = torch.empty((n, pc.cout, wo) if is1d else oshape, dtype=torch.float32, device=x.device)
        assert not accumulate
    o4 = _as4d(out)
    assert o4.shape == oshape, (o4.shape, oshape)
    assert o4.stride(3) == 1 or wo == 1
    r4 = None
    if res is not None:
        r4 = _as4d(res)
        assert r4.shape == o4.shape and (r4.stride(3) == 1 or wo == 1)
    b = pc.bias if bias is None else bias
    if o4.numel() == 0:
        return out
    _check(x, out, res, pc.w, b)
    d = ConvDesc()
    d.N, d.Cin, d.H, d.W, d.Cout, d.Ho, d.Wo = n, c, h, w, pc.cout, ho, wo
    d.KH, d.KW = pc.kh, pc.kw
    d.stride_h, d.stride_w = pc.stride
    d.pad_h, d.pad_w = pc.padding
    d.dil_h, d.dil_w = pc.dilation
    d.groups = pc.groups
    d.x_sn, d.x_sc, d.x_sh = x4.stride(0), x4.stride(1), x4.stride(2)
    d.y_sn, d.y_sc, d.y_sh = o4.stride(0), o4.stride(1), o4.stride(2)
    if r4 is not None:
        d.r_sn, d.r_sc, d.r_sh = r4.stride(0), r4.stride(1), r4.stride(2)
    d.pre_act, d.pre_slope, d.act, d.act_slope = pre_act, pre_slope, act, act_slope
    d.out_scale, d.accumulate = out_scale, 1 if accumulate else 0
    d.res_before_act = 1 if res_before_act else 0
    d.pad_h_end, d.pad_w_end = (-1, -1) if pc.padding_end is None else pc.padding_end
    d.shuffle, d.res_mul = int(shuffle), 1 if res_mul else 0
    d.packed_v3 = 1
    d.split = 1 if getattr(pc, "split", False) else 2 if getattr(pc, "f16", False) else 0
    wino = (getattr(pc, "w_wino", None) is not None and not is1d and res is None and not accumulate and pre_act == ACT_NONE
            and out_scale == 1.0 and act in (ACT_NONE, ACT_RELU) and not shuffle and out_len is None and wo % 2 == 0
            and n * ho * wo >= winograd_min_positions)
    wino2 = (wino and winograd2d and getattr(pc, "w_wino2", None) is not None and w % 4 == 0 and x4.stride(0) % 4 == 0 and x4.stride(1) % 4 == 0
             and x4.stride(2) % 4 == 0 and x4.data_ptr() % 16 == 0)
    wino1 = (winograd1d and getattr(pc, "w_wino1", None) is not None and pc.cout >= 16 and is1d and not shuffle and out_len is None and w % 4 == 0
             and n * w >= winograd1d_min_positions and pre_act in (ACT_NONE, ACT_LRELU) and 0.0 <= pre_slope <= 1.0
             and not res_mul and w < (1 << 24) and x4.stride(1) < (1 << 24)
             and 15 * (-(-(c // pc.groups) // 32) * 32) * (-(-pc.cout // 32) * 32) * 4 < (1 << 31)
             and x4.data_ptr() % 16 == 0 and x4.stride(0) % 4 == 0 and x4.stride(1) % 4 == 0 and x4.stride(1) >= w
             and o4.data_ptr() % 16 == 0 and o4.stride(0) % 4 == 0 and o4.stride(1) % 4 == 0
             and (r4 is None or (r4.data_ptr() % 16 == 0 and r4.stride(0) % 4 == 0 and r4.stride(1) % 4 == 0)))
    d.gemm_tile = gemm_tile
    w2code, w2kind = _w2d_code()
    d.wino = w2code if wino2 else 1 if wino else 8 if wino1 else 0
    prof = conv_profile
    if prof is not None and x.is_cuda:
        e0, e1 = torch.cuda.Event(enable_timing=True), torch.cuda.Event(enable_timing=True)
        e0.record()
    _call("aicg_conv_forward", ctypes.addressof(d), _ptr(x4), _ptr(pc.wino2_image(w2kind) if wino2 else pc.w_wino if wino else pc.w_wino1 if wino1 else pc.w), _ptr(b), _ptr(r4), _ptr(o4), _stream(x))
    if prof is not None and x.is_cuda:
        e1.record()
        prof.events.append((e0, e1))
        prof.flops += 2.0 * n * pc.cout * (pc.cin // pc.groups) * pc.kh * pc.kw * ho * wo
        exe = 4.0 / 9.0 if wino2 else 2.0 / 3.0 if wino else 1.0
        if wino1:
            exe = {3: 4, 5: 7, 7: 10, 11: 15}[pc.kw] / (2.0 * pc.kw) * (1.0 if pc.dilation[1] == 1 else 32.0 / 30.0)
        prof.flops_executed += 2.0 * n * pc.cout * (pc.cin // pc.groups) * pc.kh * pc.kw * ho * wo * exe
        prof.bytes += 4.0 * (n * c * h * w + pc.cout * (pc.cin // pc.groups) * pc.kh * pc.kw
                             + n * pc.cout * ho * wo * (1 + (r4 is not None) + bool(accumulate)))
        prof.launches += 1
        prof.shapes.append(("N%d C%d>%d %dx%d k%dx%d s%d,%d d%d,%d g%d%s%s%s" % (
            n, c, pc.cout, h, w, pc.kh, pc.kw, pc.stride[0], pc.stride[1], pc.dilation[0], pc.dilation[1], pc.groups,
            " res" if r4 is not None else "", " acc" if accumulate else "", (" shuf" if shuffle else "") + (" wino2" if wino2 else " wino" if wino else " wino1d" if wino1 else "")),
            2.0 * n * pc.cout * (pc.cin // pc.groups) * pc.kh * pc.kw * ho * wo))
    return out


class PackedConvTranspose:

    def __init__(self, weight, bias=None, stride=1, padding=0, output_padding=0, device=None):
        if weight.dim() == 3:
            weight = weight.unsqueeze(2)
            stride, padding, output_padding = (1, _one(stride)), (0, _one(padding)), (0, _one(output_padding))
        else:
            stride, padding, output_padding = _pair(stride), _pair(padding), _pair(output_padding)
        self.cin, self.cout, self.kh, self.kw = weight.shape
        self.stride, self.padding, self.output_padding = stride, padding, output_padding
        device = weight.device if device is None else device
        gemm_w = weight.detach().permute(1, 2, 3, 0).reshape(self.cout * self.kh * self.kw, self.cin)
        self.gemm = PackedConv(gemm_w.contiguous(), None, device=device)
        self.bias = None if bias is None else bias.detach().to(device=device, dtype=torch.float32).contiguous()
        self.bias4 = None if self.bias is None else self.bias.repeat_interleave(self.kh * self.kw).contiguous()

    def out_hw(self, h, w):
        ho = (h - 1) * self.stride[0] - 2 * self.padding[0] + self.kh + self.output_padding[0]
        wo = (w - 1) * self.stride[1] - 2 * self.padding[1] + self.kw + self.output_padding[1]
        return ho, wo


def conv_transpose(x, pt, out=None, add=None, pre_act=ACT_NONE, pre_slope=0.0, act=ACT_NONE, act_slope=0.0, mul=None):
    is1d = x.dim() == 3
    x4 = _as4d(x)
    n, c, h, w = x4.shape
    assert add is None or mul is None
    if (not is1d and (pt.kh, pt.kw) == (2, 2) and pt.stride == (2, 2) and pt.padding == (0, 0)
            and pt.output_padding == (0, 0)):
        return conv(x4, pt.gemm, res=add if mul is None else mul, out=out, pre_act=pre_act, pre_slope=pre_slope, act=act,
                    act_slope=act_slope, bias=pt.bias4, shuffle=2, res_mul=mul is not None)
    cols = conv(x4, pt.gemm, pre_act=pre_act, pre_slope=pre_slope)
    ho, wo = pt.out_hw(h, w)
    if out is None:
        out = torch.empty((n, pt.cout, wo) if is1d else (n, pt.cout, ho, wo), dtype=torch.float32, device=x.device)
    o4 = _as4d(out)
    assert o4.shape == (n, pt.cout, ho, wo) and (o4.stride(3) == 1 or wo == 1)
    a4 = None if add is None else _as4d(add)
    if a4 is not None:
        assert a4.shape == o4.shape and (a4.stride(3) == 1 or wo == 1)
    _check(cols, out, add, pt.bias)
    asn, asc, ash = (a4.stride(0), a4.stride(1), a4.stride(2)) if a4 is not None else (0, 0, 0)
    _call("aicg_col2im", _ptr(cols), _ptr(pt.bias), _ptr(a4), _ptr(o4), n, pt.cout, h, w, ho, wo, pt.kh, pt.kw,
              pt.stride[0], pt.stride[1], pt.padding[0], pt.padding[1], act, act_slope,
              o4.stride(0), o4.stride(1), o4.stride(2), asn, asc, ash, _stream(x))
    if mul is not None:
        globals()["mul"](out, mul, out=out)
    return out


def sine_source(f0, noise, upp, sr, lin_w, lin_b, sine_amp=0.1, noise_std=0.003):
    f0 = f0.contiguous().float()
    noise = noise.contiguous().float()
    t = f0.numel()
    assert noise.numel() == t * upp
    _check(f0, noise)
    prefix = torch.empty(t, dtype=torch.float64, device=f0.device)
    out = torch.empty(t * upp, dtype=torch.float32, device=f0.device)
    _call("aicg_sine_source", _ptr(f0), _ptr(noise), _ptr(prefix), _ptr(out), t, int(upp), float(sr), sine_amp,
              noise_std, float(lin_w), float(lin_b), _stream(f0))
    return out


def gate_tanh_sigmoid(a, out=None):
    assert a.is_contiguous() and a.dim() == 3 and a.shape[1] % 2 == 0
    n, c2, t = a.shape
    if out is None:
        out = torch.empty((n, c2 // 2, t), dtype=torch.float32, device=a.device)
    assert out.is_contiguous()
    _check(a, out)
    _call("aicg_gate_tanh_sigmoid", _ptr(a), _ptr(out), n, c2 // 2, t, _stream(a))
    return out


def prior_sample(stats, noise, scale):
    assert stats.is_contiguous() and noise.is_contiguous() and stats.shape[0] == 1
    c, t = noise.shape[1], noise.shape[2]
    assert stats.shape[1] == 2 * c and stats.shape[2] == t
    out = torch.empty_like(noise)
    _check(stats, noise)
    _call("aicg_prior_sample", _ptr(stats), _ptr(noise), _ptr(out), c, t, float(scale), _stream(stats))
    return out


def feats_prepare(feats, t_out, feats0=None, pitchf=None, protect=0.5):
    feats = feats.contiguous()
    th, c = feats.shape
    out = torch.empty((1, c, t_out), dtype=torch.float32, device=feats.device)
    if feats0 is not None:
        feats0 = feats0.contiguous()
        pitchf = pitchf.contiguous().float()
        assert pitchf.numel() >= t_out
    _check(feats, feats0, pitchf)
    _call("aicg_feats_prepare", _ptr(feats), _ptr(feats0), _ptr(pitchf), _ptr(out), th, c, int(t_out), float(protect),
              _stream(feats))
    return out


def layernorm_ct(x, gamma, beta, res=None, out=None, eps=1e-5):
    assert x.is_contiguous() and x.dim() == 3
    n, c, t = x.shape
    if out is None:
        out = torch.empty_like(x)
    if res is not None:
        assert res.is_contiguous() and res.shape == x.shape
    _check(x, res, gamma, beta, out)
    _call("aicg_layernorm_ct", _ptr(x), _ptr(res), _ptr(gamma), _ptr(beta), _ptr(out), n, c, t, float(eps), c * t, c * t,
              c * t, _stream(x))
    return out


def rownorm_act(x, gamma, beta, act=ACT_NONE, eps=1e-5, out=None):
    assert x.dim() == 2 and (x.stride(1) == 1 or x.shape[1] == 1)
    rows, t = x.shape
    ld = x.stride(0) if rows > 1 else max(x.stride(0), t)
    if out is None:
        out = torch.empty((rows, ld), dtype=torch.float32, device=x.device)[:, :t] if ld != t else torch.empty_like(x)
    assert out.shape == x.shape and (out.stride(1) == 1 or t == 1) and (rows <= 1 or out.stride(0) == ld)
    _check(x, gamma, beta, out)
    need = ctypes.c_int64(0)
    _call("aicg_rownorm_act_workspace_floats", rows, t, ctypes.addressof(need))
    ws = torch.empty(need.value, dtype=torch.float32, device=x.device) if need.value else None
    _call("aicg_rownorm_act_ld", _ptr(x), _ptr(gamma), _ptr(beta), _ptr(out), rows, t, ld, float(eps), act, _ptr(ws), _stream(x))
    return out


def attention(q, k, v, n_heads, relk=None, relv_emb=None, window=0, scale=1.0, n_splits=None):
    c, t = q.shape
    d = c // n_heads
    assert q.stride(1) == 1 and k.stride(1) == 1 and v.stride(1) == 1
    o = torch.empty((c, t), dtype=torch.float32, device=q.device)
    lse = torch.empty((n_heads, t), dtype=torch.float32, device=q.device) if relv_emb is not None else None
    if relk is not None:
        assert relk.is_contiguous() and relk.shape == (n_heads, 2 * window + 1, t)
    _check(q, k, v, relk, relv_emb)
    st = _stream(q)
    blocks = -(-t // 128) * n_heads
    splits = max(1, min(4, -(-t // 32), -(-1024 // blocks))) if n_splits is None else n_splits
    if splits > 1:
        scratch = torch.empty(splits * n_heads * (d + 2) * t, dtype=torch.float32, device=q.device)
        _call("aicg_attention_split", _ptr(q), _ptr(k), _ptr(v), _ptr(relk), _ptr(o), _ptr(lse), t, n_heads, d, window,
                  q.stride(0), k.stride(0), v.stride(0), o.stride(0), float(scale), splits, _ptr(scratch), st)
    else:
        _call("aicg_attention", _ptr(q), _ptr(k), _ptr(v), _ptr(relk), _ptr(o), _ptr(lse), t, n_heads, d, window,
                  q.stride(0), k.stride(0), v.stride(0), o.stride(0), float(scale), st)
    if relv_emb is not None:
        relv_emb = relv_emb.contiguous()
        _call("aicg_attention_relv", _ptr(q), _ptr(k), _ptr(relk), _ptr(relv_emb), _ptr(lse), _ptr(o), t, n_heads, d,
                  window, q.stride(0), k.stride(0), o.stride(0), float(scale), st)
    return o


ACT_LOGCLAMP = 6


def complex_abs(re, im):
    assert re.is_contiguous() and im.is_contiguous() and re.shape == im.shape
    out = torch.empty_like(re)
    _check(re, im)
    _call("aicg_complex_abs", _ptr(re), _ptr(im), _ptr(out), re.numel(), _stream(re))
    return out


def channel_affine(x, scale, shift, act=ACT_NONE):
    assert x.is_contiguous() and x.dim() >= 2
    n, c = x.shape[0], x.shape[1]
    hw = x.numel() // (n * c)
    out = torch.empty_like(x)
    _check(x, scale, shift)
    _call("aicg_channel_affine", _ptr(x), _ptr(scale), _ptr(shift), _ptr(out), n, c, hw, act, _stream(x))
    return out


def avgpool2x2(x):
    n, c, h, w = x.shape
    assert x.stride(3) == 1
    out = torch.empty((n, c, h // 2, w // 2), dtype=torch.float32, device=x.device)
    _check(x)
    _call("aicg_avgpool2x2", _ptr(x), _ptr(out), n, c, h, w, x.stride(0), x.stride(1), x.stride(2), _stream(x))
    return out


GRU_TWO_WORKGROUPS = _env.dev("AICG_GRU_2WG", "1") != "0"
GRU_WORKGROUPS = int(_env.dev("AICG_GRU_WG", "4"))


_gru_pending = []


def gru_timed_out():
    pend, _gru_pending[:] = list(_gru_pending), []
    bad = False
    for f, _ in pend:
        bad = bad or int(f.item()) != 0
    return bad


def gru_check_pending():
    if gru_timed_out():
        raise RuntimeError("aicg_gru_bidir_2wg: partner workgroup exchange timed out")


def _gru_repair_backlog():
    import warnings
    pend, _gru_pending[:] = list(_gru_pending), []
    for f, (gi, whh_t, bhh, out, hidden) in pend:
        if int(f.item()) != 0:
            warnings.warn("aicg_gru_bidir: a multi-workgroup launch timed out %d launches ago and nobody polled gru_timed_out(); its "
                          "output is recomputed in place now -- results already derived from it are stale" % len(pend))
            _call("aicg_gru_bidir", _ptr(gi), _ptr(whh_t), _ptr(bhh), _ptr(out), hidden, gi.shape[1], _stream(gi))


def gru_bidir(gi, whh_t, bhh, hidden, two_workgroups=None):
    assert gi.is_contiguous() and gi.shape[0] == 6 * hidden
    t = gi.shape[1]
    out = torch.empty((2 * hidden, t), dtype=torch.float32, device=gi.device)
    _check(gi, whh_t, bhh)
    if GRU_TWO_WORKGROUPS if two_workgroups is None else two_workgroups:
        scratch = torch.empty(32 * hidden + 64, dtype=torch.uint8, device=gi.device)
        _call("aicg_gru_bidir_4wg" if hidden == 256 and GRU_WORKGROUPS == 4 else "aicg_gru_bidir_2wg", _ptr(gi), _ptr(whh_t), _ptr(bhh),
              _ptr(out), hidden, t, _ptr(scratch), _stream(gi))
        _gru_pending.append((scratch[32 * hidden: 32 * hidden + 4].view(torch.int32), (gi, whh_t, bhh, out, hidden)))
        if len(_gru_pending) > 16:
            _gru_repair_backlog()
        return out
    _call("aicg_gru_bidir", _ptr(gi), _ptr(whh_t), _ptr(bhh), _ptr(out), hidden, t, _stream(gi))
    return out


class GruSegments:

    def __init__(self, gi, whh_t, bhh, hidden, two_workgroups=None):
        assert gi.is_contiguous() and gi.shape[0] == 6 * hidden
        _check(gi, whh_t, bhh)
        self.gi, self.whh_t, self.bhh, self.hidden, self.T = gi, whh_t, bhh, hidden, gi.shape[1]
        self.out = torch.empty((2 * hidden, self.T), dtype=torch.float32, device=gi.device)
        self.state = torch.zeros((2, hidden), dtype=torch.float32, device=gi.device)
        multi = GRU_TWO_WORKGROUPS if two_workgroups is None else two_workgroups
        self.multi = bool(multi) and hidden == 256 and GRU_WORKGROUPS == 4
        self.scratch = torch.empty(32 * hidden + 64, dtype=torch.uint8, device=gi.device) if self.multi else None
        self.done = 0
        self._first_done = None

    def run(self, s1):
        s0, s1 = self.done, min(int(s1), self.T)
        if s1 <= s0:
            return
        if self.multi:
            _call("aicg_gru_bidir_4wg_seg", _ptr(self.gi), _ptr(self.whh_t), _ptr(self.bhh), _ptr(self.out), self.hidden, self.T, s0, s1,
                  _ptr(self.state), _ptr(self.scratch), _stream(self.gi))
            if s0 == 0 and self.gi.is_cuda:
                self._first_done = torch.cuda.Event()
                self._first_done.record(torch.cuda.current_stream(self.gi.device))
            if s1 == self.T:
                _gru_pending.append((self.scratch[32 * self.hidden: 32 * self.hidden + 4].view(torch.int32),
                                     (self.gi, self.whh_t, self.bhh, self.out, self.hidden)))
        else:
            _call("aicg_gru_bidir_seg", _ptr(self.gi), _ptr(self.whh_t), _ptr(self.bhh), _ptr(self.out), self.hidden, self.T, s0, s1,
                  _ptr(self.state), _stream(self.gi))
        self.done = s1

    def timed_out(self):
        if not self.multi or self.done == 0:
            return False
        if self._first_done is not None and not self._first_done.query():
            return False
        return int(self.scratch[32 * self.hidden: 32 * self.hidden + 4].view(torch.int32).item()) != 0

    def ready(self):
        return max(0, self.T - self.done), min(self.T, self.done)


def salience_decode(salience, thred=0.03, want_center=False):
    salience = salience.contiguous().float()
    t, nb = salience.shape
    cents = torch.empty(t, dtype=torch.float64, device=salience.device)
    f0 = torch.empty(t, dtype=torch.float64, device=salience.device)
    center = torch.empty(t, dtype=torch.int32, device=salience.device) if want_center else None
    _check(salience)
    _call("aicg_salience_decode", _ptr(salience), _ptr(cents), _ptr(f0), _ptr(center), t, nb, float(thred), _stream(salience))
    return (cents, f0, center) if want_center else (cents, f0)


def f0_coarse(f0, factor, mel_min, mel_max):
    f0 = f0.contiguous().double()
    out = torch.empty_like(f0)
    coarse = torch.empty(f0.shape, dtype=torch.int64, device=f0.device)
    _check(f0)
    _call("aicg_f0_coarse", _ptr(f0), float(factor), _ptr(out), _ptr(coarse), f0.numel(), float(mel_min), float(mel_max),
              _stream(f0))
    return out, coarse


def linear_last(x, weight, bias=None, ch_scale=None, ch_shift=None, act=ACT_NONE, res=None, out=None, fp32=False):
    assert x.is_contiguous() and x.dim() == 4 and weight.is_contiguous()
    b, c, t, f = x.shape
    o = weight.shape[0]
    assert weight.shape[1] == f
    if out is None:
        out = torch.empty((b, c, t, o), dtype=torch.float32, device=x.device)
    if res is not None:
        assert res.is_contiguous() and res.shape == out.shape
    _check(x, weight, bias, ch_scale, ch_shift, res, out)
    _call("aicg_gemm_nt_split" if split_precision and not fp32 else "aicg_gemm_nt", _ptr(x), _ptr(weight), _ptr(bias), _ptr(ch_scale),
          _ptr(ch_shift), _ptr(res), _ptr(out), b * c * t, f, o, f, f, o, o, t, c, act, _stream(x))
    return out


def pack_tdf_w1(w1):
    h, f = w1.shape
    assert f % 8 == 0
    return w1.detach().float().t().reshape(f // 8, 4, 2, h).permute(0, 2, 3, 1).contiguous()


def pack_tdf_w2(w2):
    f, h = w2.shape
    assert f % 32 == 0
    slab = (32 * (h + 4) + 255) // 256 * 256
    out = torch.zeros((f // 32, slab), dtype=torch.float32, device=w2.device)
    rows = torch.zeros((f // 32, 32, h + 4), dtype=torch.float32, device=w2.device)
    rows[:, :, :h] = w2.detach().float().reshape(f // 32, 32, h)
    out[:, : 32 * (h + 4)] = rows.reshape(f // 32, -1)
    return out.contiguous()


def tdf_pair_supported(f, h, rows_per_ch):
    return bool(_lib.get().aicg_tdf_pair_supported(int(f), int(h), int(rows_per_ch)))


def tdf_pair(x, w1p, b1, s1, t1, w2p, b2, s2, t2, out=None):
    assert x.is_contiguous() and x.dim() == 4 and w2p.is_contiguous() and w1p.is_contiguous()
    b, c, t, f = x.shape
    h = w1p.numel() // f
    assert w1p.numel() == f * h and w2p.shape[0] == f // 32
    if out is None:
        out = torch.empty_like(x)
    _check(x, w1p, b1, s1, t1, w2p, b2, s2, t2, out)
    _call("aicg_tdf_pair", _ptr(x), _ptr(w1p), _ptr(b1), _ptr(s1), _ptr(t1), _ptr(w2p), _ptr(b2), _ptr(s2), _ptr(t2), _ptr(out),
          b * c * t, f, h, t, c, _stream(x))
    return out


def mul(a, b, out=None):
    assert a.is_contiguous() and b.is_contiguous() and a.shape == b.shape
    if out is None:
        out = torch.empty_like(a)
    _check(a, b, out)
    _call("aicg_mul", _ptr(a), _ptr(b), _ptr(out), a.numel(), _stream(a))
    return out


def axpbypcz(a, alpha, b=None, beta=0.0, c=None, gamma=0.0, out=None):
    assert a.is_contiguous() and (b is None or b.is_contiguous()) and (c is None or c.is_contiguous())
    if out is None:
        out = torch.empty_like(a)
    _check(a, b, c, out)
    _call("aicg_axpbypcz", _ptr(a), float(alpha), _ptr(b), float(beta), _ptr(c), float(gamma), _ptr(out), a.numel(),
              _stream(a))
    return out


def box_sum_f64(x, n, window):
    x = x.contiguous()
    assert x.dtype == torch.float64 and x.numel() >= n + window - 1
    out = torch.empty(n, dtype=torch.float64, device=x.device)
    _check(x)
    _call("aicg_box_sum_f64", _ptr(x), _ptr(out), n, window, _stream(x))
    return out


def argmin_abs_f64(x, starts, lens):
    assert x.dtype == torch.float64
    st = torch.tensor(list(starts), dtype=torch.int64, device=x.device)
    ln = torch.tensor(list(lens), dtype=torch.int64, device=x.device)
    out = torch.empty(len(st), dtype=torch.int64, device=x.device)
    _check(x)
    _call("aicg_argmin_abs_f64", _ptr(x), _ptr(st), _ptr(ln), _ptr(out), len(st), _stream(x))
    return out


def frame_rms(x, frame_length, hop_length):
    x = x.contiguous()
    assert x.dim() == 1 and x.dtype in (torch.float32, torch.float64)
    n = x.numel()
    out = torch.empty(1 + n // hop_length, dtype=torch.float64, device=x.device)
    _check(x)
    _call("aicg_frame_rms", _ptr(x), 1 if x.dtype == torch.float64 else 0, _ptr(out), n, frame_length, hop_length, _stream(x))
    return out


def rms_mix_(data, rms1, rms2, rate):
    assert data.is_contiguous() and data.dtype == torch.float32
    _check(data, rms1, rms2)
    _call("aicg_rms_mix", _ptr(data), data.numel(), _ptr(rms1), rms1.numel(), _ptr(rms2), rms2.numel(), float(rate),
              _stream(data))
    return data


def absmax(x):
    assert x.is_contiguous() and x.dtype == torch.float32
    out = torch.zeros(1, dtype=torch.float32, device=x.device)
    _check(x)
    _call("aicg_absmax", _ptr(x), x.numel(), _ptr(out), _stream(x))
    return out


def to_int16(x, scale):
    assert x.is_contiguous() and x.dtype == torch.float32
    out = torch.empty(x.shape, dtype=torch.int16, device=x.device)
    _check(x)
    _call("aicg_to_int16", _ptr(x), _ptr(out), x.numel(), float(scale), _stream(x))
    return out


FX_HPF, FX_COMP = 1, 2


def fx_reverb_state_size(sr):
    n = ctypes.c_int64(0)
    _lib.call("aicg_fx_reverb_state_size", int(sr), ctypes.addressof(n))
    return n.value


def fx_dynamics(x, state_in, seg_len, warm, coefs, flags):
    assert x.dim() == 2 and x.is_contiguous() and x.dtype == torch.float32
    C, n = x.shape
    y = torch.empty_like(x)
    st = torch.empty((C, 2), dtype=torch.float32, device=x.device)
    assert state_in is None or (state_in.shape == st.shape and state_in.is_contiguous() and state_in.dtype == torch.float32)
    _check(x, state_in)
    _call("aicg_fx_dynamics", _ptr(x), _ptr(y), _ptr(state_in), _ptr(st), C, n, int(seg_len), int(warm),
          *[float(v) for v in coefs], int(flags), _stream(x))
    return y, st


def fx_reverb(x, sr, state_in, seg_len, warm, coefs):
    assert x.dim() == 2 and x.is_contiguous() and x.dtype == torch.float32
    C, n = x.shape
    y = torch.empty_like(x)
    st = torch.empty((C, fx_reverb_state_size(sr)), dtype=torch.float32, device=x.device)
    assert state_in is None or (state_in.shape == st.shape and state_in.is_contiguous() and state_in.dtype == torch.float32)
    _check(x, state_in)
    _call("aicg_fx_reverb", _ptr(x), _ptr(y), _ptr(state_in), _ptr(st), C, n, int(sr), int(seg_len), int(warm),
          *[float(v) for v in coefs], _stream(x))
    return y, st


def fx_to_pcm16(x):
    assert x.dim() == 2 and x.is_contiguous() and x.dtype == torch.float32
    C, n = x.shape
    out = torch.empty((n, C), dtype=torch.int16, device=x.device)
    _check(x)
    _call("aicg_fx_to_pcm16", _ptr(x), _ptr(out), C, n, _stream(x))
    return out


def pcm16_mix(a, a_rate, a_gains, b, b_rate, b_gains, out_frames):
    for t in (a, b):
        assert t.dim() == 2 and t.is_contiguous() and t.dtype == torch.int16
    ch = max(a.shape[1], b.shape[1])
    out = torch.empty((int(out_frames), ch), dtype=torch.int16, device=a.device)
    _check(a, b, out)
    _call("aicg_pcm16_mix", _ptr(a), a.shape[1], int(a_rate), a.shape[0], float(a_gains[0]), float(a_gains[1]),
          _ptr(b), b.shape[1], int(b_rate), b.shape[0], float(b_gains[0]), float(b_gains[1]), _ptr(out), int(out_frames), _stream(a))
    return out


STEM_PCM16, STEM_F32 = 0, 1


def stem_normalise(x):
    if x.dim() != 2:
        raise ValueError("stem_normalise takes (frames, channels) int16 or (channels, n) float32, got %s" % (tuple(x.shape),))
    if not x.is_contiguous():
        raise ValueError("stem_normalise takes a contiguous tensor (strides %s of shape %s)" % (x.stride(), tuple(x.shape)))
    fmt = {torch.int16: STEM_PCM16, torch.float32: STEM_F32}.get(x.dtype, -1)
    n, C = (x.shape[1], x.shape[0]) if fmt == STEM_F32 else (x.shape[0], x.shape[1])
    out = torch.empty((2, n), dtype=torch.float32, device=x.device)
    peak = torch.empty(1, dtype=torch.float32, device=x.device)
    _check(x)
    _call("aicg_stem_normalise", _ptr(x), fmt, C, n, _ptr(out), _ptr(peak), _stream(x))
    return out, peak


def mdx_stems_pcm16(wave, separated, peak, compensation, want_main=True, want_inverted=True):
    for t in (wave, separated):
        if t.dtype != torch.float32 or t.dim() != 2 or t.shape[0] != 2:
            raise TypeError("mdx_stems_pcm16 takes (2, n) float32 signals, got %s %s" % (t.dtype, tuple(t.shape)))
        if not t.is_contiguous():
            raise ValueError("mdx_stems_pcm16 takes contiguous tensors (strides %s of shape %s)" % (t.stride(), tuple(t.shape)))
    if wave.shape != separated.shape:
        raise ValueError("mdx_stems_pcm16: wave %s and separated %s differ in shape" % (tuple(wave.shape), tuple(separated.shape)))
    if peak.dtype != torch.float32 or peak.numel() != 1:
        raise TypeError("mdx_stems_pcm16: peak is one float32 on the device, got %s %s" % (peak.dtype, tuple(peak.shape)))
    n = wave.shape[1]
    main = torch.empty((n, 2), dtype=torch.int16, device=wave.device) if want_main else None
    inv = torch.empty((n, 2), dtype=torch.int16, device=wave.device) if want_inverted else None
    _check(wave, separated, peak)
    _call("aicg_mdx_stems_pcm16", _ptr(wave), _ptr(separated), _ptr(peak), float(compensation), n, _ptr(main), _ptr(inv), _stream(wave))
    return main, inv


def tempo_wsola_geometry(sr, tempo, n):
    g = (ctypes.c_int64 * 6)()
    _lib.call("aicg_tempo_wsola_geometry", int(sr), float(tempo), int(n), ctypes.addressof(g))
    return tuple(int(v) for v in g)


def tempo_wsola(x, sr, tempo, offsets=None):
    assert x.dim() in (2, 3) and x.is_contiguous() and x.dtype == torch.float32
    S = 1 if x.dim() == 2 else x.shape[0]
    C, n = x.shape[-2:]
    steps, n_out = tempo_wsola_geometry(sr, tempo, n)[4:]
    y = torch.empty(x.shape[:-1] + (n_out,), dtype=torch.float32, device=x.device)
    offs = torch.zeros(x.shape[:-2] + (steps,), dtype=torch.int32, device=x.device)
    if offsets is not None:
        assert offsets.shape == offs.shape and offsets.dtype == torch.int32 and offsets.is_contiguous()
    _check(x, offsets)
    _call("aicg_tempo_wsola", _ptr(x), _ptr(y), _ptr(offs), _ptr(offsets), S, C, n, int(sr), float(tempo), _stream(x))
    return y, offs


RESAMPLE_ATT_DB = 100.0
RESAMPLE_PASS = 0.90
RESAMPLE_PHASES = 1024


def resample_ratio_design(ratio):
    nu = min(1.0, 1.0 / float(ratio))
    beta = 0.1102 * (RESAMPLE_ATT_DB - 8.7)
    width = (1.0 - RESAMPLE_PASS) * nu / 2.0
    half = int(math.ceil((RESAMPLE_ATT_DB - 7.95) / (2.285 * 2.0 * math.pi * width) / 2.0))
    return (1.0 + RESAMPLE_PASS) / 2.0 * nu / 2.0, beta, half


def resample_ratio_filter(tau, ratio):
    fc, beta, half = resample_ratio_design(ratio)
    tau = np.asarray(tau, np.float64)
    u = 1.0 - (tau / half) ** 2
    w = np.where(u > 0.0, np.i0(beta * np.sqrt(np.maximum(u, 0.0))) / np.i0(beta), 0.0)
    return 2.0 * fc * np.sinc(2.0 * fc * tau) * w


_ratio_tables = {}


def resample_ratio_table(ratio):
    half = resample_ratio_design(ratio)[2]
    r = np.arange(RESAMPLE_PHASES + 1, dtype=np.float64)[:, None] / RESAMPLE_PHASES
    j = np.arange(-half, half + 1, dtype=np.float64)[None, :]
    return resample_ratio_filter(r + j, ratio).astype(np.float32), half


def resample_ratio(x, ratio, n_out):
    assert x.dim() in (2, 3) and x.is_contiguous() and x.dtype == torch.float32
    S = 1 if x.dim() == 2 else x.shape[0]
    C, n_in = x.shape[-2:]
    key = (float(ratio), str(x.device))
    if key not in _ratio_tables:
        t, half = resample_ratio_table(ratio)
        _ratio_tables[key] = (torch.from_numpy(t).to(x.device), half)
    table, half = _ratio_tables[key]
    y = torch.empty(x.shape[:-1] + (int(n_out),), dtype=torch.float32, device=x.device)
    _check(x, table)
    _call("aicg_resample_ratio", _ptr(x), _ptr(y), S, C, n_in, int(n_out), float(ratio), _ptr(table), RESAMPLE_PHASES, half, _stream(x))
    return y


def frame_normalize(frames):
    assert frames.is_contiguous() and frames.dim() == 2
    out = torch.empty_like(frames)
    _check(frames)
    _call("aicg_frame_normalize", _ptr(frames), _ptr(out), frames.shape[0], frames.shape[1], _stream(frames))
    return out


def affine_maxpool2(x, scale, shift):
    assert x.is_contiguous() and x.dim() == 3
    n, c, w = x.shape
    out = torch.empty((n, c, w // 2), dtype=torch.float32, device=x.device)
    _check(x, scale, shift)
    _call("aicg_affine_maxpool2", _ptr(x), _ptr(scale), _ptr(shift), _ptr(out), n, c, w, _stream(x))
    return out


def crepe_viterbi(probs, seq_len, bin_lo, bin_hi):
    probs = probs.contiguous()
    n_seq, nb, ms = probs.shape
    sl = torch.tensor(list(seq_len), dtype=torch.int32, device=probs.device)
    logp = torch.empty((n_seq, ms, nb), dtype=torch.float32, device=probs.device)
    ptr = torch.empty((n_seq, ms, nb), dtype=torch.int16, device=probs.device)
    bins = torch.zeros((n_seq, ms), dtype=torch.int64, device=probs.device)
    _check(probs)
    _call("aicg_crepe_viterbi", _ptr(probs), _ptr(sl), _ptr(logp), _ptr(ptr), _ptr(bins), n_seq, nb, ms, int(bin_lo),
              int(bin_hi), _stream(probs))
    return bins


def filter3(x, mode):
    x = x.contiguous().float()
    out = torch.empty_like(x)
    _check(x)
    _call("aicg_filter3", _ptr(x), _ptr(out), x.numel(), {"median": 0, "mean": 1}[mode], _stream(x))
    return out


_filtfilt_plans = {}


def _filtfilt_plan(b, a):
    key = (tuple(np.asarray(b, np.float64)), tuple(np.asarray(a, np.float64)))
    if key not in _filtfilt_plans:
        from scipy.signal import lfilter_zi
        bb, aa = np.asarray(b, np.float64), np.asarray(a, np.float64)
        n = max(len(aa), len(bb))
        bb = np.concatenate([bb, np.zeros(n - len(bb))])
        aa = np.concatenate([aa, np.zeros(n - len(aa))])
        zi = np.ascontiguousarray(lfilter_zi(bb, aa), dtype=np.float64)
        rmax = float(np.max(np.abs(np.roots(aa)))) if n > 1 else 0.0
        if not rmax < 1.0:
            raise ValueError("filtfilt: unstable filter (max |pole| = %g)" % rmax)
        from scipy.signal import lfilter
        imp = np.zeros(1 << 17)
        imp[0] = 1.0
        env = np.maximum.accumulate(np.abs(lfilter(bb, aa, imp))[::-1])[::-1]
        below = np.nonzero(env < 1e-18 * env[0])[0]
        if len(below) == 0:
            raise ValueError("filtfilt: impulse response too long for the block-parallel recurrence")
        warm = (int(below[0]) + 255) // 256 * 256
        _filtfilt_plans[key] = (np.ascontiguousarray(bb), np.ascontiguousarray(aa), zi, n - 1, 3 * n, warm)
    return _filtfilt_plans[key]


def filtfilt_f64(x, b, a, block=1024):
    x = x.contiguous().double()
    bb, aa, zi, order, padlen, warm = _filtfilt_plan(b, a)
    n = x.numel()
    y = torch.empty_like(x)
    ext = torch.empty(n + 2 * padlen, dtype=torch.float64, device=x.device)
    mid = torch.empty_like(ext)
    _check(x)
    _call("aicg_filtfilt_f64", _ptr(x), _ptr(y), n, bb.ctypes.data, aa.ctypes.data, zi.ctypes.data, order, padlen, int(block),
          int(warm), _ptr(ext), _ptr(mid), _stream(x))
    return y


_resample_plans = {}


def _resample_plan(up, down, n_in, device):
    g = math.gcd(int(up), int(down))
    up, down = int(up) // g, int(down) // g
    key = (up, down, str(device))
    if key not in _resample_plans:
        from scipy.signal import firwin
        max_rate = max(up, down)
        half_len = 10 * max_rate
        h = firwin(2 * half_len + 1, 1.0 / max_rate, window=("kaiser", 5.0)).astype(np.float32)
        h *= up
        n_pre_pad = down - half_len % down
        hpad = np.concatenate([np.zeros(n_pre_pad, np.float32), h])
        taps = (len(hpad) + up - 1) // up
        table = np.zeros((up, taps), np.float32)
        for ph in range(up):
            col = hpad[ph::up]
            table[ph, :len(col)] = col
        _resample_plans[key] = (torch.from_numpy(table).to(device), taps, (half_len + n_pre_pad) // down)
    table, taps, pre = _resample_plans[key]
    n_out = n_in * up
    n_out = n_out // down + bool(n_out % down)
    return up, down, table, taps, pre, n_out


def resample_poly_mono(x, sr_in, sr_out):
    x = x.float()
    if x.dim() == 1:
        x = x.unsqueeze(0)
    assert x.stride(1) == 1
    c, n = x.shape
    up, down, table, taps, pre, n_out = _resample_plan(sr_out, sr_in, n, x.device)
    y = torch.empty(n_out, dtype=torch.float32, device=x.device)
    _check(x, table)
    _call("aicg_resample_poly", _ptr(x), _ptr(y), n, n_out, c, x.stride(0), up, down, _ptr(table), taps, pre, _stream(x))
    return y


def row_sqnorm(v):
    v = v.contiguous().float()
    out = torch.empty(v.shape[0], dtype=torch.float32, device=v.device)
    _check(v)
    _call("aicg_row_sqnorm", _ptr(v), _ptr(out), v.shape[0], v.shape[1], _stream(v))
    return out


def knn8_update(dots, xnorm, qnorm, col_off, best_d, best_i, merge):
    assert dots.dim() == 2 and dots.stride(1) == 1
    _check(dots, xnorm, qnorm, best_d, best_i)
    _call("aicg_knn8", _ptr(dots), dots.stride(0), _ptr(xnorm), _ptr(qnorm), dots.shape[0], dots.shape[1], int(col_off),
          _ptr(best_d), _ptr(best_i), 1 if merge else 0, _stream(dots))


def ivf_scan8(feats, vecs, list_off, probe, nprobe):
    assert feats.is_contiguous() and vecs.is_contiguous() and probe.is_contiguous() and list_off.dtype == torch.int64
    rows, dim = feats.shape
    best_d = torch.empty((rows, 8), dtype=torch.float32, device=feats.device)
    best_p = torch.empty((rows, 8), dtype=torch.int64, device=feats.device)
    _check(feats, vecs, list_off, probe)
    _call("aicg_ivf_scan8", _ptr(feats), _ptr(vecs), _ptr(list_off), _ptr(probe), probe.shape[1], int(nprobe), rows, dim,
          _ptr(best_d), _ptr(best_p), _stream(feats))
    return best_d, best_p


def index_mix_(feats, big, best_d, best_i, rate, recompute=False):
    assert feats.is_contiguous() and big.is_contiguous() and best_d.is_contiguous() and best_i.is_contiguous()
    _check(feats, big, best_d, best_i)
    _call("aicg_index_mix", _ptr(feats), _ptr(big), _ptr(best_d), _ptr(best_i), feats.shape[0], feats.shape[1], float(rate),
          1 if recompute else 0, _stream(feats))
    return feats


class StageProfile:

    def __init__(self):
        self.rec = {}

    def add(self, name, e0, e1, flops, nbytes):
        r = self.rec.setdefault(name, {"events": [], "flops": 0.0, "bytes": 0.0, "launches": 0})
        r["events"].append((e0, e1))
        r["flops"] += flops
        r["bytes"] += nbytes
        r["launches"] += 1

    def summary(self):
        torch.cuda.synchronize()
        out = {}
        for name, r in self.rec.items():
            ms = sum(a.elapsed_time(b) for a, b in r["events"])
            out[name] = {"launches": r["launches"], "ms": ms, "flops": r["flops"], "bytes": r["bytes"]}
        return out


stage_profile = None


def _staged(name, fn, work):
    def wrapped(*a, **k):
        prof = stage_profile
        t = a[0] if a and torch.is_tensor(a[0]) else None
        if prof is None or t is None or not t.is_cuda:
            return fn(*a, **k)
        e0, e1 = torch.cuda.Event(enable_timing=True), torch.cuda.Event(enable_timing=True)
        e0.record()
        r = fn(*a, **k)
        e1.record()
        fl, by = work(a, k, r)
        prof.add(name, e0, e1, fl, by)
        return r
    wrapped.__name__, wrapped.__doc__ = fn.__name__, fn.__doc__
    return wrapped


def _numel(*ts):
    return float(sum(t.numel() for t in ts if t is not None))


stft = _staged("stft", stft, lambda a, k, r: (0.0, 4.0 * _numel(a[0], r)))
istft = _staged("istft", istft, lambda a, k, r: (0.0, 4.0 * _numel(a[0], r)))
def dense_nt(x, weight, bias=None, act=ACT_NONE):
    return _linear_last_raw(x.view(1, 1, x.shape[0], x.shape[1]), weight, bias, act=act, fp32=True).view(x.shape[0], weight.shape[0])


_linear_last_raw = linear_last
_gemm_work = lambda a, k, r: (2.0 * r.numel() * a[1].shape[1], 4.0 * _numel(a[0], a[1], r, k.get("res")))
linear_last = _staged("tdf_gemm_nt", linear_last, _gemm_work)
tdf_pair = _staged("tdf_pair", tdf_pair, lambda a, k, r: (4.0 * a[0].numel() * (a[1].numel() // a[0].shape[3]),
                                                          4.0 * _numel(a[0], r, a[1], a[1])))
dense_nt = _staged("dense_gemm_nt", dense_nt, _gemm_work)
attention = _staged("attention", attention, lambda a, k, r: (4.0 * a[0].numel() * a[0].shape[1],
                                                             4.0 * _numel(a[0], a[1], a[2], r)))
sine_source = _staged("sine_source", sine_source, lambda a, k, r: (0.0, 4.0 * _numel(a[0], a[1], r)))
layernorm_ct = _staged("layernorm", layernorm_ct, lambda a, k, r: (0.0, 4.0 * _numel(a[0], k.get("res"), r)))
rownorm_act = _staged("groupnorm_gelu", rownorm_act, lambda a, k, r: (0.0, 4.0 * _numel(a[0], r)))
```

### aicovergen_amd/vc_infer_pipeline.py

```python
import functools
import os
import traceback
import warnings
from time import time as ttime

import numpy as np
import torch
import torch.nn.functional as F
from scipy import signal

from . import _env
from . import ops
from . import dist as adist

BASE_DIR = os.path.dirname(os.path.dirname(os.path.abspath(__file__)))

bh, ah = signal.butter(N=5, Wn=48, btype="high", fs=16000)

input_audio_path2wav = {}

_NO_GROUP = "single"


class _HostStream:

    def wait_stream(self, other): pass
    def wait_event(self, ev): pass
    def synchronize(self): pass
    def __enter__(self): return self
    def __exit__(self, *a): return False


class _HostEvent:
    def record(self, stream=None): pass


def _rms_frames(y, frame_length, hop_length):
    y = np.asarray(y)
    pad = frame_length // 2
    yp = np.pad(y, (pad, pad), mode="reflect")
    n_frames = 1 + (len(yp) - frame_length) // hop_length
    idx = np.arange(frame_length)[None, :] + hop_length * np.arange(n_frames)[:, None]
    power = np.mean(np.abs(yp[idx]) ** 2, axis=1)
    return np.sqrt(power)[None, :].astype(y.dtype if y.dtype in (np.float32, np.float64) else np.float32)


def change_rms(data1, sr1, data2, sr2, rate):
    rms1 = _rms_frames(data1, sr1 // 2 * 2, sr1 // 2)
    rms2 = _rms_frames(data2, sr2 // 2 * 2, sr2 // 2)
    rms1 = F.interpolate(torch.from_numpy(rms1).unsqueeze(0), size=data2.shape[0], mode="linear").squeeze()
    rms2 = F.interpolate(torch.from_numpy(rms2).unsqueeze(0), size=data2.shape[0], mode="linear").squeeze()
    rms2 = torch.max(rms2, torch.zeros_like(rms2) + 1e-6)
    data2 *= (torch.pow(rms1, torch.tensor(1 - rate)) * torch.pow(rms2, torch.tensor(rate - 1))).numpy()
    return data2


def _bracket_pipeline(fn):
    @functools.wraps(fn)
    def wrapper(self, *args, **kwargs):
        self._in_pipeline = True
        try:
            return fn(self, *args, **kwargs)
        finally:
            self._in_pipeline = False
            self._group = None
    return wrapper


class _Call:

    def __init__(self, **args):
        self.__dict__.update(args)
        self.overlap, self.progressive = self.schedule != "serial", self.schedule == "progressive"
        self.pitch = self.pitchf = self.main = self.side = self.enc = None
        self.pad_dev = None
        self.feats_of, self.pieces = {}, {}
        self.fronts = {}
        self.gru_seg, self.f0_bad = None, False
        self.marks, self.cover = [], (self.p_len, 0)
        self.tf0 = self.t2 = self.f0_wait = 0.0

    def noise(self, ci):
        return self.noise_fn(ci, *self.bounds[ci]) if self.noise_fn is not None else None

    def frames_of(self, ci):
        s, e = self.bounds[ci]
        return s // self.window, (self.p_len if ci == len(self.bounds) - 1 else (e - self.window) // self.window)

    def chunk_pitch(self, ci):
        if self.if_f0 != 1:
            return None, None
        fa, fb = self.frames_of(ci)
        return self.pitch[:, fa:fb], self.pitchf[:, fa:fb]

    def publish(self, lo, hi, f0bak, coarse):
        hi = min(hi, self.p_len)
        if lo < hi:
            self.pitch[0, lo:hi] = coarse[: hi - lo]
            self.pitchf[0, lo:hi] = f0bak[: hi - lo].float()
        self.cover = (min(self.cover[0], lo), max(self.cover[1], hi))
        ev = torch.cuda.Event() if self.on_gpu else _HostEvent()
        ev.record(self.side)
        self.marks.append(self.cover + (ev,))

    def mark_of(self, ci):
        fa, fb = self.frames_of(ci)
        for m, (lo, hi, _) in enumerate(self.marks):
            if lo <= fa and min(fb, self.p_len) <= hi:
                return m
        return len(self.marks) - 1

    def order(self):
        return sorted(self.mine, key=lambda ci: (self.mark_of(ci), ci)) if self.progressive else list(self.mine)

    def wait_pitch(self, stream, ci):
        if self.progressive:
            stream.wait_event(self.marks[self.mark_of(ci)][2])

    def drain(self):
        if not self.on_gpu:
            return
        if self.progressive:
            torch.cuda.current_stream(self.device).synchronize()
        else:
            torch.cuda.synchronize()


class VC(object):
    def __init__(self, tgt_sr, config):
        self.x_pad, self.x_query, self.x_center, self.x_max, self.is_half = (
            config.x_pad, config.x_query, config.x_center, config.x_max, config.is_half)
        self.sr = 16000
        self.window = 160
        self.t_pad = self.sr * self.x_pad
        self.t_pad_tgt = tgt_sr * self.x_pad
        self.t_pad2 = self.t_pad * 2
        self.t_query = self.sr * self.x_query
        self.t_center = self.sr * self.x_center
        self.t_max = self.sr * self.x_max
        self.device = config.device
        self.rmvpe_path = None

    def get_optimal_torch_device(self, index: int = 0) -> torch.device:
        if torch.cuda.is_available():
            return torch.device(f"cuda:{index % torch.cuda.device_count()}")
        return torch.device("cpu")

    def get_f0_crepe_computation(self, x, f0_min, f0_max, p_len, hop_length=160, model="full", dither=None):
        from . import crepe
        print("Initiating prediction with a crepe_hop_length of: " + str(hop_length))
        return crepe.mangio_crepe_f0(self._crepe(model), x, p_len, hop_length, dither=dither, group=self._f0_group(False))

    def _crepe(self, model):
        from . import crepe
        if not hasattr(self, "model_crepe"):
            self.model_crepe = {}
        if model not in self.model_crepe:
            self.model_crepe[model] = crepe.load_crepe(model, self.device)
        return self.model_crepe[model]

    def get_f0_official_crepe_computation(self, x, f0_min, f0_max, model="full", dither=None):
        from . import crepe
        return crepe.official_crepe_f0(self._crepe(model), x, self.window, f0_min, f0_max, dither=dither,
                                       group=self._f0_group(False))

    def get_f0_hybrid_computation(self, methods_str, input_audio_path, x, f0_min, f0_max, p_len, filter_radius,
                                  crepe_hop_length, time_step):
        methods = methods_str.split("hybrid")[1].replace("[", "").replace("]", "").split("+")
        print("Calculating f0 pitch estimations for methods: %s" % str(methods))
        x = x.astype(np.float32)
        x = x / np.quantile(np.abs(x), 0.999)
        stack = []
        for method in methods:
            if method in ("crepe", "crepe-tiny"):
                f0 = self.get_f0_official_crepe_computation(x, f0_min, f0_max, "tiny" if method.endswith("tiny") else "full")[1:]
            elif method in ("mangio-crepe", "mangio-crepe-tiny"):
                f0 = self.get_f0_crepe_computation(x, f0_min, f0_max, p_len, crepe_hop_length,
                                                   "tiny" if method.endswith("tiny") else "full")
            else:
                raise NotImplementedError("hybrid f0: method %r needs parselmouth / pyworld (supported inside hybrid[...]: "
                                          "crepe, crepe-tiny, mangio-crepe, mangio-crepe-tiny)" % method)
            stack.append(np.asarray(f0, dtype=np.float64))
        for fc in stack:
            print(len(fc))
        print("Calculating hybrid median f0 from the stack of: %s" % str(methods))
        if len(stack) == 1:
            return stack[0]
        return np.nanmedian(stack, axis=0)

    def _f0_group(self, explicit=True):
        import torch.distributed as td
        if not getattr(self, "_in_pipeline", False) or not (td.is_available() and td.is_initialized()):
            return _NO_GROUP if not explicit else None
        g = getattr(self, "_group", None)
        if adist.single(td.get_world_size(g) if g is not None else td.get_world_size(), g):
            return _NO_GROUP if not explicit else None
        return g if (g is not None or not explicit) else td.group.WORLD

    _rmvpe_group = _f0_group

    @staticmethod
    def _default_rmvpe_path():
        import sys
        cands = []
        for name in ("__main__", "main"):
            d = getattr(sys.modules.get(name), "rvc_models_dir", None)
            if isinstance(d, str):
                cands.append(os.path.join(d, "rmvpe.pt"))
        for q in sys.path:
            if q:
                cands.append(os.path.join(os.path.dirname(os.path.abspath(q)), "rvc_models", "rmvpe.pt"))
        cands.append(os.path.join(BASE_DIR, "rvc_models", "rmvpe.pt"))
        for c in cands:
            if os.path.exists(c):
                return c
        return cands[-1]

    def _rmvpe(self):
        if not hasattr(self, "model_rmvpe"):
            from .rmvpe import RMVPE
            self.model_rmvpe = RMVPE(self.rmvpe_path or self._default_rmvpe_path(), is_half=self.is_half, device=self.device)
        return self.model_rmvpe

    def get_f0(self, input_audio_path, x, p_len, f0_up_key, f0_method, filter_radius, crepe_hop_length, inp_f0=None,
               _raw_f0=None):
        f0_min, f0_max = 50, 1100
        f0_mel_min = 1127 * np.log(1 + f0_min / 700)
        f0_mel_max = 1127 * np.log(1 + f0_max / 700)
        def host(a):
            return a.detach().cpu().numpy() if torch.is_tensor(a) else np.asarray(a)

        if _raw_f0 is not None:
            f0 = _raw_f0
        elif f0_method == "rmvpe":
            f0 = self._rmvpe().infer_from_audio(x, thred=0.03, group=self._rmvpe_group())
        elif f0_method in ("mangio-crepe", "mangio-crepe-tiny"):
            f0 = self.get_f0_crepe_computation(host(x), f0_min, f0_max, p_len, crepe_hop_length,
                                               "tiny" if f0_method.endswith("tiny") else "full")
        elif f0_method in ("crepe", "crepe-tiny"):
            f0 = self.get_f0_official_crepe_computation(host(x), f0_min, f0_max, "tiny" if f0_method.endswith("tiny") else "full")
        elif "hybrid" in f0_method:
            f0 = self.get_f0_hybrid_computation(f0_method, input_audio_path, host(x), f0_min, f0_max, p_len, filter_radius,
                                                crepe_hop_length, self.window / self.sr * 1000)
        else:
            raise NotImplementedError(
                "f0_method %r needs parselmouth / pyworld, which are outside the MI355X hot path "
                "(supported: rmvpe, mangio-crepe[-tiny], crepe[-tiny], hybrid[...] of the crepe methods)" % f0_method)
        tf0 = self.sr // self.window
        f0 = np.asarray(self._estimated_f0(0, len(f0), np.asarray(f0, dtype=np.float64)), dtype=np.float64)
        factor = pow(2, f0_up_key / 12)
        if inp_f0 is not None:
            f0 = f0 * factor
            factor = 1.0
            delta_t = np.round((inp_f0[:, 0].max() - inp_f0[:, 0].min()) * tf0 + 1).astype("int16")
            replace_f0 = np.interp(list(range(delta_t)), inp_f0[:, 0] * 100, inp_f0[:, 1])
            shape = f0[self.x_pad * tf0: self.x_pad * tf0 + len(replace_f0)].shape[0]
            f0[self.x_pad * tf0: self.x_pad * tf0 + len(replace_f0)] = replace_f0[:shape]
        f0bak, coarse = self._f0_tail(torch.from_numpy(f0).to(self.device), factor)
        return coarse.cpu().numpy(), f0bak.cpu().numpy()

    def _estimated_f0(self, lo, hi, f0):
        return f0

    def _f0_tail(self, f0, factor):
        f0_mel_min = 1127 * np.log(1 + 50 / 700)
        f0_mel_max = 1127 * np.log(1 + 1100 / 700)
        return ops.f0_coarse(f0, factor, f0_mel_min, f0_mel_max)

    def vc(self, model, net_g, sid, audio0, pitch, pitchf, times, index, big_npy, index_rate, version, protect,
           noise=None, keep_on_device=False):
        t0 = ttime()
        feats, feats0 = self._vc_features(model, audio0, index, big_npy, index_rate, version,
                                          protect < 0.5 and pitch is not None and pitchf is not None)
        if self._sync():
            torch.cuda.synchronize()
        t1 = ttime()
        o = self._vc_synth(net_g, sid, audio0.shape[0], feats, feats0, pitch, pitchf, protect, noise)
        if keep_on_device:
            if self._sync():
                torch.cuda.synchronize()
            audio1 = o[0, 0]
        else:
            audio1 = o[0, 0].data.cpu().float().numpy()
        t2 = ttime()
        times[0] += t1 - t0
        times[2] += t2 - t1
        return audio1

    def _vc_features(self, model, audio0, index, big_npy, index_rate, version, use_protect):
        return self._vc_features_many(model, [audio0], index, big_npy, index_rate, version, use_protect)[0]

    def _vc_features_many(self, model, audios, index, big_npy, index_rate, version, use_protect):
        srcs = []
        for audio0 in audios:
            feats = audio0.float() if torch.is_tensor(audio0) else torch.from_numpy(np.ascontiguousarray(audio0)).float()
            if feats.dim() == 2:
                feats = feats.mean(-1)
            assert feats.dim() == 1, feats.dim()
            srcs.append(feats.view(1, -1).to(self.device))
        layer = 9 if version == "v1" else 12
        if len(srcs) > 1 and hasattr(model, "extract_features_many"):
            logits = model.extract_features_many(srcs, layer)
        else:
            logits = [model.extract_features(source=s, padding_mask=torch.zeros(s.shape, dtype=torch.bool), output_layer=layer)[0]
                      for s in srcs]
        return [self._vc_features_post(model, lg, index, big_npy, index_rate, version, use_protect) for lg in logits]

    def _vc_features_post(self, model, logits, index, big_npy, index_rate, version, use_protect):
        feats = model.final_proj(logits) if version == "v1" else logits
        feats0 = feats.clone() if use_protect else None
        if index is not None and hasattr(index, "mix_") and index_rate != 0:
            feats = index.mix_(feats[0].contiguous(), index_rate).unsqueeze(0)
        elif index is not None and big_npy is not None and index_rate != 0:
            npy = feats[0].cpu().numpy().astype("float32")
            score, ix = index.search(npy, k=8)
            weight = np.square(1 / score)
            weight /= weight.sum(axis=1, keepdims=True)
            npy = np.sum(big_npy[ix] * np.expand_dims(weight, axis=2), axis=1)
            feats = torch.from_numpy(npy.astype("float32")).unsqueeze(0).to(self.device) * index_rate + (1 - index_rate) * feats
        return feats, feats0

    def _vc_synth(self, net_g, sid, n_samples, feats, feats0, pitch, pitchf, protect, noise):
        return self._vc_synth_back(net_g, self._vc_synth_front(net_g, sid, n_samples, feats, feats0, pitch, pitchf, protect, noise))

    def _vc_synth_back(self, net_g, st):
        if "front" not in st:
            return st["o"]
        return net_g.infer_back(st["front"], st["pitchf"], st["ns"])[0]

    def _vc_synth_front(self, net_g, sid, n_samples, feats, feats0, pitch, pitchf, protect, noise):
        p_len = n_samples // self.window
        if 2 * feats.shape[1] < p_len:
            p_len = 2 * feats.shape[1]
        if pitch is not None and pitchf is not None:
            pitch = pitch[:, :p_len]
            pitchf = pitchf[:, :p_len]
        use_protect = feats0 is not None
        phone_ct = ops.feats_prepare(feats[0], p_len, feats0[0] if use_protect else None,
                                     pitchf[0].float() if use_protect else None, protect)
        nz, ns = noise if noise is not None else (None, None)
        if hasattr(net_g, "infer_front"):
            return {"front": net_g.infer_front(phone_ct, pitch, sid, nz), "pitchf": pitchf, "ns": ns}
        lens = torch.tensor([p_len], device=self.device).long()
        if pitch is not None and pitchf is not None:
            return {"o": net_g.infer(None, lens, pitch, pitchf, sid, noise_z=nz, noise_src=ns, phone_ct=phone_ct)[0]}
        return {"o": net_g.infer(None, lens, sid, noise_z=nz, noise_src=ns, phone_ct=phone_ct)[0]}

    def _sync(self):
        return torch.cuda.is_available() and str(self.device).startswith("cuda")

    def plan(self, audio):
        dev = self.device if ops._lib.backend() != "emu" else torch.device("cpu")
        if torch.is_tensor(audio):
            a = audio.detach().to(dev).double().view(-1)
        else:
            a = torch.from_numpy(np.ascontiguousarray(audio, dtype=np.float64)).to(dev)
        if _env.dev("AICG_FILTFILT", "device") == "host" or a.numel() <= 3 * max(len(ah), len(bh)):
            audio = torch.from_numpy(np.ascontiguousarray(signal.filtfilt(bh, ah, a.cpu().numpy()))).to(dev)
        else:
            audio = ops.filtfilt_f64(a, bh, ah)
        n = audio.numel()

        def reflect_pad(x, k):
            if k < n:
                return F.pad(x.view(1, 1, -1), (k, k), mode="reflect").view(-1)
            period = max(2 * (n - 1), 1)
            i = (torch.arange(-k, n + k, device=x.device) % period)
            return x[torch.where(i >= n, period - i, i)]

        opt_ts = []
        if n + self.window > self.t_max:
            audio_sum = ops.box_sum_f64(reflect_pad(audio, self.window // 2), n, self.window)
            centers = list(range(self.t_center, n, self.t_center))
            starts = [t - self.t_query for t in centers]
            lens = [min(t + self.t_query, n) - (t - self.t_query) for t in centers]
            idx = ops.argmin_abs_f64(audio_sum, starts, lens).cpu().numpy()
            opt_ts = [int(s0 + i) for s0, i in zip(starts, idx)]
        audio_pad = reflect_pad(audio, self.t_pad)
        return audio, audio_pad, opt_ts, audio_pad.shape[0] // self.window

    def chunk_bounds(self, audio_pad, opt_ts):
        bounds = []
        s = 0
        t = None
        for t in opt_ts:
            t = t // self.window * self.window
            bounds.append((s, t + self.t_pad2 + self.window))
            s = t
        bounds.append((t if t is not None else 0, audio_pad.shape[0]))
        return bounds

    def _seeded_noise(self, net_g, seed):
        inter, upp = net_g.inter_channels, net_g.upp

        def noise_fn(ci, s, e, _seed=int(seed)):
            g = torch.Generator(device=self.device).manual_seed(_seed + ci)
            T = 2 * ((e - s - 400) // 320 + 1)
            return (torch.randn((1, inter, T), generator=g, device=self.device),
                    torch.randn(T * upp, generator=g, device=self.device))
        return noise_fn

    def _load_index(self, file_index, index_rate):
        if file_index == "" or not os.path.exists(file_index) or index_rate == 0:
            return None, None
        try:
            if _env.dev("AICG_GPU_KNN", "1") != "0":
                from . import retrieval
                return retrieval.load_index(file_index, self.device), None
            import faiss
            index = faiss.read_index(file_index)
            return index, index.reconstruct_n(0, index.ntotal)
        except Exception:
            traceback.print_exc()
            return None, None

    @staticmethod
    def _read_f0_file(f0_file):
        try:
            with open(f0_file.name, "r") as f:
                lines = f.read().strip("\n").split("\n")
            return np.array([[float(i) for i in line.split(",")] for line in lines], dtype="float32")
        except Exception:
            traceback.print_exc()

    def _schedule(self, net_g, if_f0, f0_method, world, inp_f0):
        on_gpu = self._sync()
        env_seg = int(_env.dev("AICG_F0_SEGMENTS", "0"))
        nseg = env_seg or (16 if world > 1 else (8 if on_gpu else 0))
        if not (if_f0 == 1 and f0_method == "rmvpe" and (on_gpu or nseg > 1) and _env.dev("AICG_OVERLAP_F0", "1") != "0"):
            return "serial", nseg, False
        two_streams = on_gpu and hasattr(net_g, "infer_front") and _env.dev("AICG_OVERLAP_SYNTH", "1") != "0"
        return ("progressive" if nseg > 1 and inp_f0 is None else "one_launch"), nseg, two_streams

    def _run_f0(self, c, raw=None):
        pc, pcf = self.get_f0(*c.f0_args, _raw_f0=raw)
        return (torch.tensor(pc[:c.p_len], device=self.device).unsqueeze(0).long(),
                torch.tensor(pcf[:c.p_len], device=self.device).unsqueeze(0).float())

    def _features(self, c):
        many = self._vc_features_many(c.model, [c.pad_dev[c.bounds[ci][0]:c.bounds[ci][1]] for ci in c.mine], c.index, c.big_npy,
                                      c.index_rate, c.version, c.protect < 0.5 and c.if_f0 == 1)
        c.feats_of = dict(zip(c.mine, many))

    def _f0_serial(self, c):
        if c.if_f0 == 1:
            c.pitch, c.pitchf = self._run_f0(c)
        if self._sync():
            torch.cuda.synchronize()
        c.t2 = ttime()
        c.times[1] += c.t2 - c.t1

    def _open_side(self, c):
        c.main = torch.cuda.current_stream(self.device) if c.on_gpu else _HostStream()
        c.side = getattr(self, "_f0_stream", None) if c.on_gpu else _HostStream()
        if c.side is None:
            prio = -1 if _env.dev("AICG_F0_PRIORITY", "1") != "0" else 0
            c.side = self._f0_stream = torch.cuda.Stream(device=self.device, priority=prio)
        c.pad_dev = c.audio_pad.float()

    def _f0_one_launch(self, c):
        self._open_side(c)
        c.side.wait_stream(c.main)
        c.tf0 = ttime()
        with (torch.cuda.stream(c.side) if c.on_gpu else c.side):
            f0_dev = self._rmvpe().infer_from_audio_device(c.pad_dev, thred=0.03, group=self._rmvpe_group())
        self._features(c)
        self._settle(c, f0_dev)
        self._open_enc(c)

    def _f0_progressive(self, c):
        self._open_side(c)
        c.pitch = torch.ones((1, c.p_len), dtype=torch.long, device=self.device)
        c.pitchf = torch.zeros((1, c.p_len), dtype=torch.float32, device=self.device)
        c.side.wait_stream(c.main)
        c.tf0 = ttime()
        factor = pow(2, c.f0_args[3] / 12)

        def on_f0(lo, hi, f0):
            c.publish(lo, hi, *self._f0_tail(self._estimated_f0(lo, hi, f0), factor))
        with (torch.cuda.stream(c.side) if c.on_gpu else c.side):
            self._rmvpe().infer_progressive(c.pad_dev, 0.03, c.nseg, on_f0, group=self._rmvpe_group())
        c.gru_seg = self._rmvpe().last_segments
        self._features(c)
        self._open_enc(c)
        self._settle(c)

    def _settle(self, c, f0_dev=None):
        c.main.synchronize()
        tf1 = c.t2 = ttime()
        c.f0_bad = bool(c.progressive and c.gru_seg.timed_out())
        if f0_dev is not None:
            c.side.synchronize()
            c.main.wait_stream(c.side)
            f0_host = f0_dev.cpu().numpy()
            if ops.gru_timed_out():
                f0_host = self._rmvpe().infer_from_audio_device(c.pad_dev, thred=0.03, two_workgroups=False).cpu().numpy()
            c.pitch, c.pitchf = self._run_f0(c, f0_host)
            c.t2 = ttime()
        c.f0_wait = c.t2 - tf1
        c.times[0] += tf1 - c.tf0
        c.times[1] += c.t2 - c.tf0

    def _open_enc(self, c):
        if not c.two_streams:
            return
        c.enc = getattr(self, "_enc_stream", None)
        if c.enc is None:
            c.enc = self._enc_stream = torch.cuda.Stream(device=self.device)
        c.enc.wait_stream(c.main)
        if c.order():
            self._queue_front(c, c.order()[0])

    def _queue_front(self, c, ci):
        s, e = c.bounds[ci]
        pc, pcf = c.chunk_pitch(ci)
        feats, feats0 = c.feats_of.pop(ci)
        c.wait_pitch(c.enc, ci)
        with torch.cuda.stream(c.enc):
            noise = c.noise(ci)
            st = self._vc_synth_front(c.net_g, c.sid, e - s, feats, feats0, pc, pcf, c.protect, noise)
            ev = torch.cuda.Event()
            ev.record(c.enc)
        c.fronts[ci] = (st, ev, (feats, feats0, pc, pcf, noise))

    def _chunk(self, c, ci, front=None, after=None):
        s, e = c.bounds[ci]
        pc, pcf = c.chunk_pitch(ci)
        if not c.overlap:
            out = self.vc(c.model, c.net_g, c.sid, c.audio_pad[s:e], pc, pcf, c.times, c.index, c.big_npy, c.index_rate, c.version,
                          c.protect, noise=c.noise(ci), keep_on_device=True)
        else:
            noise = c.noise(ci) if front is None else None
            ts0 = ttime()
            if front is not None:
                st, ev, keep = front
                c.main.wait_event(ev)
                out = self._vc_synth_back(c.net_g, st)[0, 0]
                if after is not None:
                    self._queue_front(c, after)
            else:
                feats, feats0 = c.feats_of.pop(ci)
                c.wait_pitch(c.main, ci)
                out = self._vc_synth(c.net_g, c.sid, e - s, feats, feats0, pc, pcf, c.protect, noise)[0, 0]
            c.drain()
            c.times[2] += ttime() - ts0
        c.pieces[ci] = out[self.t_pad_tgt: -self.t_pad_tgt]
        return c.pieces[ci]

    def _chunk_loop(self, c):
        order = c.order()
        for ci, after in zip(order, order[1:] + [None]):
            if c.f0_bad:
                break
            self._chunk(c, ci, c.fronts.pop(ci, None), after)
            if c.progressive and c.gru_seg.timed_out():
                c.f0_bad = True
        if c.progressive:
            if c.on_gpu:
                torch.cuda.synchronize()
            c.fronts.clear()

    def _recover(self, c):
        warnings.warn("aicovergen_amd: the multi-workgroup BiGRU timed out waiting for its partner workgroups (busy or shared GPU); "
                      "f0 and this rank's chunks are recomputed on the single-workgroup kernel -- this call costs about twice "
                      "its usual time", RuntimeWarning)
        c.pitch, c.pitchf = self._run_f0(c, self._rmvpe().infer_from_audio_device(c.pad_dev, thred=0.03, two_workgroups=False).cpu().numpy())
        self._features(c)
        for ci in c.mine:
            self._chunk(c, ci)
        if c.on_gpu:
            torch.cuda.synchronize()

    def _post(self, audio_opt, audio, tgt_sr, resample_sr, rms_mix_rate, device_out=False):
        if resample_sr >= 16000 and tgt_sr != resample_sr:
            a = audio_opt.cpu().numpy()
            if rms_mix_rate != 1:
                a = change_rms(audio.cpu().numpy(), 16000, a, tgt_sr, rms_mix_rate)
            g = np.gcd(int(tgt_sr), int(resample_sr))
            audio_opt = torch.from_numpy(signal.resample_poly(a, resample_sr // g, tgt_sr // g).astype(np.float32)).to(self.device)
        elif rms_mix_rate != 1:
            rms1 = ops.frame_rms(audio, 16000 // 2 * 2, 16000 // 2)
            rms2 = ops.frame_rms(audio_opt, tgt_sr // 2 * 2, tgt_sr // 2)
            ops.rms_mix_(audio_opt, rms1, rms2, rms_mix_rate)
        audio_max = float(ops.absmax(audio_opt).item()) / 0.99
        max_int16 = 32768
        if audio_max > 1:
            max_int16 /= audio_max
        out = ops.to_int16(audio_opt, max_int16)
        return out if device_out else out.cpu().numpy()

    @_bracket_pipeline
    def pipeline(self, model, net_g, sid, audio, input_audio_path, times, f0_up_key, f0_method, file_index, index_rate,
                 if_f0, filter_radius, tgt_sr, resample_sr, rms_mix_rate, version, protect, crepe_hop_length, f0_file=None,
                 noise_fn=None, group=None, noise_seed=None, device_out=False):
        if noise_fn is None and noise_seed is not None:
            noise_fn = self._seeded_noise(net_g, noise_seed)
        index, big_npy = self._load_index(file_index, index_rate)
        self._group = group
        tp0 = ttime()
        audio, audio_pad, opt_ts, p_len = self.plan(audio)
        t1 = ttime()
        inp_f0 = self._read_f0_file(f0_file) if hasattr(f0_file, "name") else None
        sid = torch.tensor(sid, device=self.device).unsqueeze(0).long()
        bounds = self.chunk_bounds(audio_pad, opt_ts)
        rank, world = adist.world(group)
        schedule, nseg, two_streams = self._schedule(net_g, if_f0, f0_method, world, inp_f0)
        c = _Call(device=self.device, on_gpu=self._sync(), window=self.window, model=model, net_g=net_g, sid=sid, index=index,
                  big_npy=big_npy, index_rate=index_rate, version=version, protect=protect, if_f0=if_f0, noise_fn=noise_fn, times=times,
                  f0_args=(input_audio_path, audio_pad, p_len, f0_up_key, f0_method, filter_radius, crepe_hop_length, inp_f0),
                  audio_pad=audio_pad, bounds=bounds, mine=[ci for ci in range(len(bounds)) if ci % world == rank], p_len=p_len,
                  schedule=schedule, nseg=nseg, two_streams=two_streams, t1=t1)
        {"serial": self._f0_serial, "one_launch": self._f0_one_launch, "progressive": self._f0_progressive}[schedule](c)
        self._chunk_loop(c)
        if c.progressive and (ops.gru_timed_out() or c.f0_bad):
            self._recover(c)
        tc1 = ttime()
        pieces = adist.gather_pieces(c.pieces, len(bounds), self.device, group)
        tj1 = ttime()
        audio_opt = self._post(torch.cat([pieces[i] for i in range(len(bounds))]).contiguous(), audio, tgt_sr, resample_sr, rms_mix_rate,
                               device_out)
        self.last_profile = {"plan_s": t1 - tp0, "f0_s": c.t2 - t1, "chunks_s": tc1 - c.t2, "post_s": ttime() - tc1,
                             "f0_wait_s": c.f0_wait, "overlap_f0": float(c.overlap), "join_s": tj1 - tc1,
                             "f0_progressive": float(c.progressive)}
        return audio_opt


Pipeline = VC
```

### include/aicg.h

```cpp
#ifndef AICG_H_
#define AICG_H_

#include <stdint.h>

#ifdef __cplusplus
extern "C" {
#endif

#define AICG_OK 0
#define AICG_E_SHAPE (-1)
#define AICG_E_ARG (-2)
#define AICG_E_HIP (-3)
#define AICG_E_LDS (-4)

#define AICG_ACT_NONE 0
#define AICG_ACT_RELU 1
#define AICG_ACT_LRELU 2
#define AICG_ACT_GELU 3
#define AICG_ACT_TANH 4
#define AICG_ACT_SIGMOID 5
#define AICG_ACT_LOGCLAMP 6

const char* aicg_last_error(void);
const char* aicg_last_launch(void);
int aicg_abi_version(void);
int aicg_mfma_probe(float* out, int n_blocks, int iters, float seed, void* stream);


int aicg_stft(const float* x, float* out, const float* window, const float* tw_half, const float* tw_full,
              int n_sig, int L, int n_fft, int hop, int n_frames, int n_bins_out,
              int64_t o_sig, int64_t o_im, int64_t o_bin, int64_t o_frame, void* stream);

int aicg_istft_frames(const float* spec, float* frames, const float* window, const float* tw_half,
                      const float* tw_full, int n_sig, int n_fft, int n_frames, int n_bins_in,
                      int64_t i_sig, int64_t i_im, int64_t i_bin, int64_t i_frame, void* stream);
int aicg_istft_ola(const float* frames, const float* window, float* out, int n_sig, int L, int n_fft,
                   int hop, int n_frames, void* stream);

typedef struct aicg_conv_desc {
    int32_t N, Cin, H, W;
    int32_t Cout, Ho, Wo;
    int32_t KH, KW, stride_h, stride_w, pad_h, pad_w, dil_h, dil_w, groups;
    int64_t x_sn, x_sc, x_sh;
    int64_t y_sn, y_sc, y_sh;
    int64_t r_sn, r_sc, r_sh;
    int32_t pre_act;
    float pre_slope;
    int32_t act;
    float act_slope;
    float out_scale;
    int32_t accumulate;
    int32_t res_before_act;
    int32_t pad_h_end, pad_w_end;
    int32_t shuffle;
    int32_t res_mul;
    int32_t packed_v3;
    int32_t split;
    int32_t wino;
    int32_t gemm_tile;
} aicg_conv_desc;

int aicg_conv_bkc(int taps);
int aicg_conv_desc_size(void);
int aicg_conv_forward(const aicg_conv_desc* desc, const float* x, const float* w_packed, const float* bias,
                      const float* res, float* y, void* stream);

int aicg_col2im(const float* cols, const float* bias, const float* add, float* out, int N, int Cout, int Hi,
                int Wi, int Ho, int Wo, int KH, int KW, int stride_h, int stride_w, int pad_h, int pad_w,
                int act, float slope, int64_t o_sn, int64_t o_sc, int64_t o_sh, int64_t a_sn, int64_t a_sc,
                int64_t a_sh, void* stream);

int aicg_sine_source(const float* f0, const float* noise, double* prefix_scratch, float* out, int T, int upp,
                     float sr, float sine_amp, float noise_std, float lin_w, float lin_b, void* stream);

int aicg_gate_tanh_sigmoid(const float* a, float* out, int N, int C, int64_t T, void* stream);

int aicg_prior_sample(const float* stats, const float* noise, float* out, int C, int64_t T, float scale, void* stream);

int aicg_feats_prepare(const float* feats, const float* feats0, const float* pitchf, float* out, int Th, int C,
                       int T, float protect, void* stream);

int aicg_layernorm_ct(const float* x, const float* res, const float* gamma, const float* beta, float* out, int N,
                      int C, int64_t T, float eps, int64_t x_sn, int64_t r_sn, int64_t o_sn, void* stream);

int aicg_rownorm_act_workspace_floats(int rows, int64_t T, int64_t* n_floats);
int aicg_rownorm_act(const float* x, const float* gamma, const float* beta, float* out, int rows, int64_t T,
                     float eps, int act, float* workspace, void* stream);
int aicg_rownorm_act_ld(const float* x, const float* gamma, const float* beta, float* out, int rows, int64_t T, int64_t ld,
                        float eps, int act, float* workspace, void* stream);

int aicg_attention(const float* q, const float* k, const float* v, const float* relk, float* o, float* lse, int T,
                   int H, int D, int window, int64_t ldq, int64_t ldk, int64_t ldv, int64_t ldo, float scale,
                   void* stream);
int aicg_attention_split(const float* q, const float* k, const float* v, const float* relk, float* o, float* lse,
                         int T, int H, int D, int window, int64_t ldq, int64_t ldk, int64_t ldv, int64_t ldo,
                         float scale, int n_splits, float* scratch, void* stream);
int aicg_attention_relv(const float* q, const float* k, const float* relk, const float* relv_emb,
                        const float* lse, float* o, int T, int H, int D, int window, int64_t ldq, int64_t ldk,
                        int64_t ldo, float scale, void* stream);

int aicg_complex_abs(const float* re, const float* im, float* out, int64_t n, void* stream);
int aicg_channel_affine(const float* x, const float* scale, const float* shift, float* out, int N, int C,
                        int64_t HW, int act, void* stream);
int aicg_avgpool2x2(const float* x, float* out, int N, int C, int H, int W, int64_t x_sn, int64_t x_sc,
                    int64_t x_sh, void* stream);
int aicg_gru_bidir(const float* gi, const float* whh_t, const float* bhh, float* out, int hidden, int64_t T,
                   void* stream);
int aicg_gru_bidir_2wg(const float* gi, const float* whh_t, const float* bhh, float* out, int hidden, int64_t T,
                       void* xchg_scratch, void* stream);
int aicg_gru_bidir_4wg(const float* gi, const float* whh_t, const float* bhh, float* out, int hidden, int64_t T,
                       void* xchg_scratch, void* stream);
int aicg_gru_bidir_seg(const float* gi, const float* whh_t, const float* bhh, float* out, int hidden, int64_t T, int64_t s_begin,
                       int64_t s_end, float* h_state, void* stream);
int aicg_gru_bidir_4wg_seg(const float* gi, const float* whh_t, const float* bhh, float* out, int hidden, int64_t T, int64_t s_begin,
                           int64_t s_end, float* h_state, void* xchg_scratch, void* stream);
int aicg_salience_decode(const float* salience, double* cents, double* f0, int* center, int64_t T, int n_bins,
                         float thred, void* stream);
int aicg_f0_coarse(const double* f0_in, double factor, double* f0_out, int64_t* coarse, int64_t n, double mel_min,
                   double mel_max, void* stream);

int aicg_gemm_nt(const float* a, const float* w, const float* bias, const float* row_scale,
                 const float* row_shift, const float* res, float* c, int64_t R, int K, int O, int64_t lda,
                 int64_t ldw, int64_t ldc, int64_t ldr, int rows_per_ch, int n_ch, int act, void* stream);
int aicg_gemm_nt_split(const float* a, const float* w, const float* bias, const float* row_scale,
                       const float* row_shift, const float* res, float* c, int64_t R, int K, int O, int64_t lda,
                       int64_t ldw, int64_t ldc, int64_t ldr, int rows_per_ch, int n_ch, int act, void* stream);

int aicg_tdf_pair_supported(int F, int H, int rows_per_ch);
int aicg_tdf_pair(const float* x, const float* w1_packed, const float* b1, const float* s1, const float* t1, const float* w2_packed,
                  const float* b2, const float* s2, const float* t2, float* out, int64_t R, int F, int H, int rows_per_ch,
                  int n_ch, void* stream);
int aicg_mul(const float* a, const float* b, float* out, int64_t n, void* stream);
int aicg_axpbypcz(const float* a, float alpha, const float* b, float beta, const float* c, float gamma, float* out,
                  int64_t n, void* stream);

int aicg_box_sum_f64(const double* x, double* out, int64_t n, int window, void* stream);
int aicg_argmin_abs_f64(const double* x, const int64_t* starts, const int64_t* lens, int64_t* out, int n_seg,
                        void* stream);
int aicg_frame_rms(const void* x, int is_f64, double* out, int64_t n, int frame_length, int hop_length, void* stream);
int aicg_rms_mix(float* data, int64_t n, const double* rms1, int64_t m1, const double* rms2, int64_t m2, double rate,
                 void* stream);
int aicg_absmax(const float* x, int64_t n, float* out, void* stream);
int aicg_to_int16(const float* x, int16_t* out, int64_t n, float scale, void* stream);

int aicg_frame_normalize(const float* x, float* out, int64_t n_frames, int frame_len, void* stream);
int aicg_affine_maxpool2(const float* x, const float* scale, const float* shift, float* out, int N, int C, int W,
                         void* stream);
int aicg_crepe_viterbi(const float* probs, const int* seq_len, float* logp_scratch, uint16_t* ptr_scratch,
                       int64_t* bins_out, int n_seq, int n_bins, int max_steps, int bin_lo, int bin_hi, void* stream);


int aicg_filter3(const float* x, float* out, int64_t n, int mode, void* stream);

int aicg_filtfilt_f64(const double* x, double* y, int64_t n, const double* b, const double* a, const double* zi, int order,
                      int padlen, int block, int warm, double* ext, double* mid, void* stream);

int aicg_resample_poly(const float* x, float* y, int64_t n_in, int64_t n_out, int n_channels, int64_t x_sc, int up, int down,
                       const float* hp, int taps, int64_t pre, void* stream);

int aicg_row_sqnorm(const float* v, float* out, int64_t rows, int dim, void* stream);
int aicg_knn8(const float* dots, int64_t ld, const float* xnorm, const float* qnorm, int rows, int cols, int64_t col_off,
              float* best_d, int64_t* best_i, int merge, void* stream);
int aicg_ivf_scan8(const float* q, const float* vecs, const int64_t* list_off, const int64_t* probe, int probe_ld, int nprobe,
                   int rows, int dim, float* best_d, int64_t* best_pos, void* stream);
int aicg_index_mix(float* feats, const float* big, float* best_d, const int64_t* best_i, int rows, int dim, float rate,
                   int recompute, void* stream);

int aicg_fx_reverb_state_size(int sample_rate, int64_t* floats_per_channel);
int aicg_fx_dynamics(const float* x, float* y, const float* state_in, float* state_out, int n_channels, int64_t n,
                     int64_t seg_len, int64_t warm, float b0, float b1, float a1, float cte_attack, float cte_release,
                     float threshold, float threshold_inv, float ratio_inv, int flags, void* stream);
int aicg_fx_reverb(const float* x, float* y, const float* state_in, float* state_out, int n_channels, int64_t n,
                   int sample_rate, int64_t seg_len, int64_t warm, float gain, float damp, float feedback, float wet1,
                   float wet2, float dry, void* stream);
int aicg_fx_to_pcm16(const float* x, int16_t* out, int n_channels, int64_t n, void* stream);
int aicg_pcm16_mix(const int16_t* a, int a_channels, int a_rate, int64_t a_frames, double a_gain1, double a_gain2,
                   const int16_t* b, int b_channels, int b_rate, int64_t b_frames, double b_gain1, double b_gain2,
                   int16_t* out, int64_t out_frames, void* stream);

int aicg_tempo_wsola_geometry(int sample_rate, double tempo, int64_t n, int64_t* geom);
int aicg_tempo_wsola(const float* x, float* y, int* offsets_out, const int* offsets_in, int n_signals, int n_channels, int64_t n,
                     int sample_rate, double tempo, void* stream);
int aicg_resample_ratio(const float* x, float* y, int n_signals, int n_channels, int64_t n_in, int64_t n_out, double ratio,
                        const float* table, int phases, int half_taps, void* stream);

int aicg_stem_normalise(const void* x, int in_format, int n_channels, int64_t n, float* out, float* peak, void* stream);
int aicg_mdx_stems_pcm16(const float* wave, const float* separated, const float* peak, float compensation, int64_t n,
                         int16_t* main_out, int16_t* inverted_out, void* stream);

#ifdef __cplusplus
}
#endif
#endif
```

Baseline: 385.6.

## Run RVC decoder only on the kept window plus receptive-field halo

Computes the decoder's receptive-field reach and alignment granule, then runs the HiFi-GAN/NSF decoder only on the frame window needed to produce the untrimmed output samples of each chunk, instead of on the full padded chunk whose edges get discarded. Adds a windowed sine-source kernel and a planned-width conv entry so tile routing still decides on the full-size geometry and numerics match. Cuts decoder compute proportional to the trimmed padding, at the cost of extra complexity and a risk of boundary mismatch if the reach computation is off.

```diff
diff --git a/aicovergen_amd/csrc/conv.hip b/aicovergen_amd/csrc/conv.hip
--- a/aicovergen_amd/csrc/conv.hip
+++ b/aicovergen_amd/csrc/conv.hip
@@ -113,6 +113,7 @@
 struct ConvCall {
     const aicg_conv_desc* d;
     int pad_h_end, pad_w_end;
+    long plan_w, plan_wo;
     hipStream_t st;
 };
 
@@ -285,7 +286,7 @@
     AICG_SWITCH(g1env, "AICG_CONV_G1", 0);
     const long g1 = c.d->gemm_tile ? c.d->gemm_tile : g1env;
     if (!(g1 != 1 && !p.wsplit && p.Cout_g > 32 && conv_g1_applicable(p, c.pad_h_end, c.pad_w_end))) return 1;
-    const long HW = (long)p.H * p.W;
+    const long HW = (long)p.H * c.plan_w;
     const int M = p.Cout_g;
     auto wgs = [&](int bm) { return (long)p.N * idiv_up(M, bm) * ldiv_up(HW, 256); };
     if (p.f16 && !p.shuffle) {
@@ -313,7 +314,7 @@
 int route_g1s(ConvArgs& p, const ConvCall& c) {
     const int tile = c.d->gemm_tile;
     if (!(tile != 1 && !p.wsplit && p.Cout_g > 32 && conv_g1s_applicable(p, c.pad_w_end))) return 1;
-    const long w64 = (long)p.N * idiv_up(p.Cout_g, 64) * idiv_up(p.Wo, 256);
+    const long w64 = (long)p.N * idiv_up(p.Cout_g, 64) * ldiv_up(c.plan_wo, 256);
     if (tile == 2) return run_g1s_128x256(p, c.st);
     if (tile == 3 || w64 >= 160) return run_g1s_64x256(p, c.st);
     return 1;
@@ -344,7 +345,7 @@
     AICG_SWITCH(force_bm, "AICG_CONV_FORCE_BM", 0);
     if (force_bm) t.BM = (int)force_bm;
     t.groups = p.groups;
-    t.npos = (long)p.N * p.Ho * p.Wo;
+    t.npos = (long)p.N * p.Ho * c.plan_wo;
     t.st = c.st;
     AICG_SWITCH(ablate, "AICG_CONV_ABLATE", 0);
     p.dbg = ablate;
@@ -469,9 +470,17 @@
 
 extern "C" int aicg_conv_forward(const aicg_conv_desc* d, const float* x, const float* w_packed, const float* bias,
                                  const float* res, float* y, void* stream) {
+    return aicg_conv_forward_planned(d, x, w_packed, bias, res, y, 0, stream);
+}
+
+extern "C" int aicg_conv_forward_planned(const aicg_conv_desc* d, const float* x, const float* w_packed, const float* bias,
+                                         const float* res, float* y, int plan_w, void* stream) {
     ConvCall c;
     int rc = validate_desc(d, x, w_packed, res, y, c);
     if (rc <= 0) return rc;
+    if (plan_w && plan_w < d->W) return fail(AICG_E_SHAPE, "aicg_conv_forward_planned: plan_w %d is shorter than the map (%d)", plan_w, d->W);
+    c.plan_w = plan_w ? plan_w : d->W;
+    c.plan_wo = d->Wo + (c.plan_w - d->W) / d->stride_w;
     c.st = (hipStream_t)stream;
     ConvArgs p;
     fill_args(p, d, x, w_packed, bias, res, y);
diff --git a/aicovergen_amd/csrc/elementwise.hip b/aicovergen_amd/csrc/elementwise.hip
--- a/aicovergen_amd/csrc/elementwise.hip
+++ b/aicovergen_amd/csrc/elementwise.hip
@@ -106,12 +106,17 @@
 __global__ void __launch_bounds__(256) sine_source4_kernel(const float* __restrict__ f0, const double* __restrict__ prefix,
                                                            const float* __restrict__ noise, float* __restrict__ out,
                                                            int T, int upp, float sr, float sine_amp, float noise_std,
-                                                           float lin_w, float lin_b) {
-    const int q_per = upp >> 2;
-    const long total4 = (long)T * q_per;
+                                                           float lin_w, float lin_b, long first, long count) {
+    const long total = (long)T * upp;
+    const long total4 = count >> 2;
     for (long n4 = (long)blockIdx.x * blockDim.x + threadIdx.x; n4 < total4; n4 += (long)gridDim.x * blockDim.x) {
-        const int t = (int)(n4 / q_per);
-        const int i0 = (int)(n4 - (long)t * q_per) * 4;
+        const long n0 = first + 4 * n4;
+        if (n0 < 0 || n0 >= total) {
+            *reinterpret_cast<float4*>(out + 4 * n4) = make_float4(0.f, 0.f, 0.f, 0.f);
+            continue;
+        }
+        const int t = (int)(n0 / upp);
+        const int i0 = (int)(n0 - (long)t * upp);
         const float f = f0[t];
         const float rad = fmodf(f / sr, 1.0f);
         const double base = prefix[t];
@@ -128,16 +133,21 @@
             const float v = sine * uv + namp * nv[j];
             o[j] = tanhf(lin_w * v + lin_b);
         }
-        *reinterpret_cast<float4*>(out + (long)t * upp + i0) = make_float4(o[0], o[1], o[2], o[3]);
+        *reinterpret_cast<float4*>(out + 4 * n4) = make_float4(o[0], o[1], o[2], o[3]);
     }
 }
 
 __global__ void __launch_bounds__(256) sine_source_kernel(const float* __restrict__ f0, const double* __restrict__ prefix,
                                                           const float* __restrict__ noise, float* __restrict__ out,
                                                           int T, int upp, float sr, float sine_amp, float noise_std,
-                                                          float lin_w, float lin_b) {
+                                                          float lin_w, float lin_b, long first, long count) {
     const long total = (long)T * upp;
-    for (long n = (long)blockIdx.x * blockDim.x + threadIdx.x; n < total; n += (long)gridDim.x * blockDim.x) {
+    for (long j = (long)blockIdx.x * blockDim.x + threadIdx.x; j < count; j += (long)gridDim.x * blockDim.x) {
+        const long n = first + j;
+        if (n < 0 || n >= total) {
+            out[j] = 0.f;
+            continue;
+        }
         const int t = (int)(n / upp);
         const int i = (int)(n - (long)t * upp);
         const float f = f0[t];
@@ -148,7 +158,7 @@
         const float uv = f > 0.f ? 1.f : 0.f;
         const float namp = uv * noise_std + (1.f - uv) * sine_amp / 3.f;
         const float v = sine * uv + namp * noise[n];
-        out[n] = tanhf(lin_w * v + lin_b);
+        out[j] = tanhf(lin_w * v + lin_b);
     }
 }
 
@@ -242,10 +252,32 @@
     hipLaunchKernelGGL(sine_frame_prefix_kernel, dim3(1), dim3(256), 0, (hipStream_t)stream, f0, prefix_scratch, T, upp, sr);
     if ((upp & 3) == 0 && ((uintptr_t)noise & 15) == 0 && ((uintptr_t)out & 15) == 0)
         hipLaunchKernelGGL(sine_source4_kernel, dim3(ew_grid((long)T * (upp >> 2))), dim3(256), 0, (hipStream_t)stream, f0,
-                           (const double*)prefix_scratch, noise, out, T, upp, sr, sine_amp, noise_std, lin_w, lin_b);
+                           (const double*)prefix_scratch, noise, out, T, upp, sr, sine_amp, noise_std, lin_w, lin_b, 0L, (long)T * upp);
     else
         hipLaunchKernelGGL(sine_source_kernel, dim3(ew_grid((long)T * upp)), dim3(256), 0, (hipStream_t)stream, f0,
-                           (const double*)prefix_scratch, noise, out, T, upp, sr, sine_amp, noise_std, lin_w, lin_b);
+                           (const double*)prefix_scratch, noise, out, T, upp, sr, sine_amp, noise_std, lin_w, lin_b, 0L, (long)T * upp);
+    return check_launch("sine_source_kernel");
+}
+
+extern "C" int aicg_sine_source_window(const float* f0, const float* noise, double* prefix_scratch, float* out, int T, int upp,
+                                       float sr, float sine_amp, float noise_std, float lin_w, float lin_b, int64_t first,
+                                       int64_t count, void* stream) {
+    if (!f0 || !noise || !prefix_scratch || !out) return fail(AICG_E_ARG, "aicg_sine_source_window: null pointer");
+    if (T < 0 || upp < 1 || count < 0) return fail(AICG_E_SHAPE, "aicg_sine_source_window: bad shape");
+    if (count == 0) return AICG_OK;
+    if ((upp & 3) == 0 && ((first & 3) != 0 || (count & 3) != 0))
+        return fail(AICG_E_ARG, "aicg_sine_source_window: upp %% 4 == 0 needs first and count to be multiples of 4");
+    const long total = (long)T * upp;
+    const long last = lmin(total, (long)first + (long)count);
+    const int Tscan = last <= 0 ? 0 : (int)((last + upp - 1) / upp);
+    if (Tscan > 0 && first < total)
+        hipLaunchKernelGGL(sine_frame_prefix_kernel, dim3(1), dim3(256), 0, (hipStream_t)stream, f0, prefix_scratch, Tscan, upp, sr);
+    if ((upp & 3) == 0 && ((uintptr_t)noise & 15) == 0 && ((uintptr_t)out & 15) == 0)
+        hipLaunchKernelGGL(sine_source4_kernel, dim3(ew_grid((long)count >> 2)), dim3(256), 0, (hipStream_t)stream, f0,
+                           (const double*)prefix_scratch, noise, out, T, upp, sr, sine_amp, noise_std, lin_w, lin_b, (long)first, (long)count);
+    else
+        hipLaunchKernelGGL(sine_source_kernel, dim3(ew_grid((long)count)), dim3(256), 0, (hipStream_t)stream, f0,
+                           (const double*)prefix_scratch, noise, out, T, upp, sr, sine_amp, noise_std, lin_w, lin_b, (long)first, (long)count);
     return check_launch("sine_source_kernel");
 }
 
diff --git a/aicovergen_amd/infer_pack/models.py b/aicovergen_amd/infer_pack/models.py
--- a/aicovergen_amd/infer_pack/models.py
+++ b/aicovergen_amd/infer_pack/models.py
@@ -240,28 +240,95 @@
             ops.conv(out, Fl["post_neg"], res=x1, out=x1)
         return z
 
-    def _decoder(self, P, x, f0, g, noise_src):
+    def _decoder_geometry(self):
+        sd = self._sd
+        assert sd is not None, "load_state_dict() first"
+        noise = [sd["dec.noise_convs.%d.weight" % i].shape[2] for i in range(len(self.upsample_rates))] if self.use_f0 else []
+        return sd["dec.conv_pre.weight"].shape[2], sd["dec.conv_post.weight"].shape[2], noise
+
+    def decoder_reach(self):
+        k_pre, k_post, k_noise = self._decoder_geometry()
+        ups, uks = self.upsample_rates, self.upsample_kernel_sizes
+
+        def chain(k, dil):
+            h = (k - 1) // 2
+            return sum(h * d + (h if self.resblock == "1" else 0) for d in dil)
+        rb = max(chain(k, d) for k, d in zip(self.resblock_kernel_sizes, self.resblock_dilation_sizes))
+        r = (k_post - 1) // 2
+        src = 0
+        for i in reversed(range(len(ups))):
+            r += rb
+            if self.use_f0:
+                s = int(np.prod(ups[i + 1:]))
+                kn, pn = k_noise[i], (s // 2 if i + 1 < len(ups) else 0)
+                src = max(src, r * s + max(pn, kn - s - pn))
+            u, k = ups[i], uks[i]
+            p = (k - u) // 2
+            r = max((r + k - 1 - p) // u, -(-(r + p) // u))
+        r += (k_pre - 1) // 2
+        return max(r, -(-src // self.upp)), r, src
+
+    def decoder_granule(self):
+        L = 4
+        for dil in self.resblock_dilation_sizes:
+            for d in dil:
+                L = L * (2 * d) // math.gcd(L, 2 * d)
+        G, rate = 4, 1
+        for u in self.upsample_rates:
+            rate *= u
+            need = L // math.gcd(L, rate)
+            G = G * need // math.gcd(G, need)
+        return G
+
+    def decoder_window(self, T, keep):
+        lo, hi = keep
+        assert 0 <= lo <= hi <= T * self.upp
+        if any((k - u) % 2 for u, k in zip(self.upsample_rates, self.upsample_kernel_sizes)):
+            return None
+        reach, G = self.decoder_reach()[0], self.decoder_granule()
+        a0 = max(0, lo // self.upp - reach) // G * G
+        a1 = T - max(0, T - (-(-hi // self.upp) + reach)) // 4 * 4
+        if (a0 == 0 and a1 == T) or a1 <= a0:
+            return None
+        return a0, a1
+
+    def _decoder(self, P, x, f0, g, noise_src, window=None):
         T = x.shape[2]
+        a0, a1 = (0, T) if window is None else window
+        Tw = a1 - a0
+        plan = (lambda w: None) if window is None else (lambda w: int(w))
         har = None
         if self.use_f0:
             if noise_src is None:
                 noise_src = torch.randn(T * self.upp, device=x.device)
-            har = ops.sine_source(f0.reshape(-1)[:T], noise_src.to(x.device).reshape(-1), self.upp, float(self.sr), P["lin_w"], P["lin_b"])
+            if window is None:
+                halo = 0
+                har = ops.sine_source(f0.reshape(-1)[:T], noise_src.to(x.device).reshape(-1), self.upp, float(self.sr), P["lin_w"], P["lin_b"])
+            else:
+                halo = -(-max(s // 2 for s, _ in P["noise"]) // 4) * 4
+                har = ops.sine_source_window(f0.reshape(-1)[:T], noise_src.to(x.device).reshape(-1), self.upp, float(self.sr), P["lin_w"],
+                                             P["lin_b"], a0 * self.upp - halo, Tw * self.upp + 2 * halo)
+                x = x[:, :, a0:a1].contiguous()
+        elif window is not None:
+            x = x[:, :, a0:a1].contiguous()
         pre_bias = ops.conv(g, P["cond"], res=P["conv_pre_bias"])
-        x = ops.conv(x, P["conv_pre"], bias=pre_bias.reshape(-1))
+        x = ops.conv(x, P["conv_pre"], bias=pre_bias.reshape(-1), plan_w=plan(T))
         nk = len(self.resblock_kernel_sizes)
+        rate = 1
         for i, pt in enumerate(P["ups"]):
             add = None
             if har is not None:
                 s, nc = P["noise"][i]
-                L = har.numel()
+                L, Lfull = Tw * self.upp, T * self.upp
                 if s > 1:
-                    xp = F.pad(har, (s // 2, s // 2))
+                    xp = F.pad(har, (s // 2, s // 2)) if window is None else har[halo - s // 2: halo + L + s // 2]
                     phases = xp.view(L // s + 1, s).t().contiguous()
-                    add = ops.conv(phases.unsqueeze(0), nc)
+                    add = ops.conv(phases.unsqueeze(0), nc, plan_w=plan(Lfull // s + 1))
                 else:
-                    add = ops.conv(har.view(1, 1, L), nc)
-            x = ops.conv_transpose(x, pt, add=add, pre_act=ops.ACT_LRELU, pre_slope=LRELU_SLOPE)
+                    add = ops.conv(har[halo: halo + L].view(1, 1, L), nc, plan_w=plan(Lfull))
+            x = ops.conv_transpose(x, pt, add=add, pre_act=ops.ACT_LRELU, pre_slope=LRELU_SLOPE, plan_w=plan(T * rate))
+            rate *= self.upsample_rates[i]
+            pw = plan(T * rate)
             acc = torch.empty_like(x)
             streams = self._rb_streams(x.device, nk)
             main = torch.cuda.current_stream(x.device) if streams else None
@@ -284,24 +351,24 @@
                             src = c1
                             inp = y
                         else:
-                            ops.conv(y, c1, out=tmp, pre_act=ops.ACT_LRELU, pre_slope=LRELU_SLOPE, act=ops.ACT_LRELU, act_slope=LRELU_SLOPE)
+                            ops.conv(y, c1, out=tmp, pre_act=ops.ACT_LRELU, pre_slope=LRELU_SLOPE, act=ops.ACT_LRELU, act_slope=LRELU_SLOPE, plan_w=pw)
                             src, inp = c2, tmp
                         if last:
                             if streams and prev_acc is not None:
                                 st.wait_event(prev_acc)
                             pre = ops.ACT_NONE if c2 is not None else ops.ACT_LRELU
-                            ops.conv(inp, src, res=y, out=acc, pre_act=pre, pre_slope=LRELU_SLOPE, out_scale=1.0 / nk, accumulate=j > 0)
+                            ops.conv(inp, src, res=y, out=acc, pre_act=pre, pre_slope=LRELU_SLOPE, out_scale=1.0 / nk, accumulate=j > 0, plan_w=pw)
                             if streams:
                                 prev_acc = torch.cuda.Event()
                                 prev_acc.record(st)
                         else:
                             dst = ya if y is not ya else yb
-                            ops.conv(inp, src, res=y, out=dst, pre_act=ops.ACT_NONE if c2 is not None else ops.ACT_LRELU, pre_slope=LRELU_SLOPE)
+                            ops.conv(inp, src, res=y, out=dst, pre_act=ops.ACT_NONE if c2 is not None else ops.ACT_LRELU, pre_slope=LRELU_SLOPE, plan_w=pw)
                             y = dst
             if streams:
                 main.wait_event(prev_acc)
             x = acc
-        return ops.conv(x, P["conv_post"], pre_act=ops.ACT_LRELU, pre_slope=0.01, act=ops.ACT_TANH)
+        return ops.conv(x, P["conv_post"], pre_act=ops.ACT_LRELU, pre_slope=0.01, act=ops.ACT_TANH, plan_w=plan(T * rate))
 
     def _rb_streams(self, device, nk):
         if device.type != "cuda" or nk < 2 or _env.dev("AICG_RB_STREAMS", "0") != "1":
@@ -312,7 +379,7 @@
         return have
 
     def infer(self, phone, phone_lengths, pitch=None, nsff0=None, sid=None, max_len=None, noise_z=None, noise_src=None,
-              phone_ct=None):
+              phone_ct=None, keep=None):
         if not self.use_f0 and sid is None:
             sid, pitch = pitch, None
         P = self._prepare()
@@ -325,7 +392,7 @@
         else:
             T = phone_ct.shape[2]
         front = self.infer_front(phone_ct, pitch, sid, noise_z)
-        return self.infer_back(front, nsff0, noise_src, max_len)
+        return self.infer_back(front, nsff0, noise_src, max_len, keep=keep)
 
     def infer_front(self, phone_ct, pitch, sid, noise_z=None):
         P = self._prepare()
@@ -339,12 +406,20 @@
         z = self._flow_reverse(P, z_p.clone(), g)
         return {"z": z, "z_p": z_p, "stats": stats, "g": g, "T": T}
 
-    def infer_back(self, front, nsff0=None, noise_src=None, max_len=None):
+    def infer_back(self, front, nsff0=None, noise_src=None, max_len=None, keep=None):
         P = self._prepare()
         dev = self.device
         z, z_p, stats, g, T = front["z"], front["z_p"], front["stats"], front["g"], front["T"]
         zz = z if max_len is None else z[:, :, :max_len].contiguous()
-        o = self._decoder(P, zz, None if nsff0 is None else nsff0.to(dev).float(), g, noise_src)
+        f0 = None if nsff0 is None else nsff0.to(dev).float()
+        if keep is None:
+            o = self._decoder(P, zz, f0, g, noise_src)
+        else:
+            lo, hi = int(keep[0]), int(keep[1])
+            window = self.decoder_window(zz.shape[2], (lo, hi))
+            o = self._decoder(P, zz, f0, g, noise_src, window=window)
+            first = 0 if window is None else window[0] * self.upp
+            o = o[:, :, lo - first: hi - first]
         x_mask = torch.ones((1, 1, T), dtype=torch.float32, device=dev)
         m_p, logs_p = stats[:, : self.inter_channels], stats[:, self.inter_channels:]
         return o, x_mask, (z, z_p, m_p, logs_p)
diff --git a/aicovergen_amd/ops.py b/aicovergen_amd/ops.py
--- a/aicovergen_amd/ops.py
+++ b/aicovergen_amd/ops.py
@@ -358,13 +358,15 @@
 
 
 def conv(x, pc, res=None, out=None, pre_act=ACT_NONE, pre_slope=0.0, act=ACT_NONE, act_slope=0.0, out_scale=1.0,
-         accumulate=False, bias=None, res_before_act=False, out_len=None, shuffle=0, res_mul=False):
+         accumulate=False, bias=None, res_before_act=False, out_len=None, shuffle=0, res_mul=False, plan_w=None):
     is1d = x.dim() == 3
     x4 = _as4d(x)
     n, c, h, w = x4.shape
     assert c == pc.cin, "conv: input has %d channels, layer expects %d" % (c, pc.cin)
     assert x4.stride(3) == 1 or w == 1
     assert h == 1 or c == 1 or x4.stride(1) >= x4.stride(2) * (h - 1) + w, "conv: input rows must lie inside the channel stride"
+    assert plan_w is None or plan_w >= w
+    gate_w = w if plan_w is None else int(plan_w)
     ho, wo = pc.out_hw(h, w)
     if out_len is not None:
         assert out_len <= wo
@@ -408,7 +410,7 @@
     wino2 = (wino and winograd2d and getattr(pc, "w_wino2", None) is not None and w % 4 == 0 and x4.stride(0) % 4 == 0 and x4.stride(1) % 4 == 0
              and x4.stride(2) % 4 == 0 and x4.data_ptr() % 16 == 0)
     wino1 = (winograd1d and getattr(pc, "w_wino1", None) is not None and pc.cout >= 16 and is1d and not shuffle and out_len is None and w % 4 == 0
-             and n * w >= winograd1d_min_positions and pre_act in (ACT_NONE, ACT_LRELU) and 0.0 <= pre_slope <= 1.0
+             and n * gate_w >= winograd1d_min_positions and pre_act in (ACT_NONE, ACT_LRELU) and 0.0 <= pre_slope <= 1.0
              and not res_mul and w < (1 << 24) and x4.stride(1) < (1 << 24)
              and 15 * (-(-(c // pc.groups) // 32) * 32) * (-(-pc.cout // 32) * 32) * 4 < (1 << 31)
              and x4.data_ptr() % 16 == 0 and x4.stride(0) % 4 == 0 and x4.stride(1) % 4 == 0 and x4.stride(1) >= w
@@ -421,7 +423,11 @@
     if prof is not None and x.is_cuda:
         e0, e1 = torch.cuda.Event(enable_timing=True), torch.cuda.Event(enable_timing=True)
         e0.record()
-    _call("aicg_conv_forward", ctypes.addressof(d), _ptr(x4), _ptr(pc.wino2_image(w2kind) if wino2 else pc.w_wino if wino else pc.w_wino1 if wino1 else pc.w), _ptr(b), _ptr(r4), _ptr(o4), _stream(x))
+    w_image = pc.wino2_image(w2kind) if wino2 else pc.w_wino if wino else pc.w_wino1 if wino1 else pc.w
+    if plan_w is None:
+        _call("aicg_conv_forward", ctypes.addressof(d), _ptr(x4), _ptr(w_image), _ptr(b), _ptr(r4), _ptr(o4), _stream(x))
+    else:
+        _call("aicg_conv_forward_planned", ctypes.addressof(d), _ptr(x4), _ptr(w_image), _ptr(b), _ptr(r4), _ptr(o4), gate_w, _stream(x))
     if prof is not None and x.is_cuda:
         e1.record()
         prof.events.append((e0, e1))
@@ -462,7 +468,7 @@
         return ho, wo
 
 
-def conv_transpose(x, pt, out=None, add=None, pre_act=ACT_NONE, pre_slope=0.0, act=ACT_NONE, act_slope=0.0, mul=None):
+def conv_transpose(x, pt, out=None, add=None, pre_act=ACT_NONE, pre_slope=0.0, act=ACT_NONE, act_slope=0.0, mul=None, plan_w=None):
     is1d = x.dim() == 3
     x4 = _as4d(x)
     n, c, h, w = x4.shape
@@ -471,7 +477,7 @@
             and pt.output_padding == (0, 0)):
         return conv(x4, pt.gemm, res=add if mul is None else mul, out=out, pre_act=pre_act, pre_slope=pre_slope, act=act,
                     act_slope=act_slope, bias=pt.bias4, shuffle=2, res_mul=mul is not None)
-    cols = conv(x4, pt.gemm, pre_act=pre_act, pre_slope=pre_slope)
+    cols = conv(x4, pt.gemm, pre_act=pre_act, pre_slope=pre_slope, plan_w=plan_w)
     ho, wo = pt.out_hw(h, w)
     if out is None:
         out = torch.empty((n, pt.cout, wo) if is1d else (n, pt.cout, ho, wo), dtype=torch.float32, device=x.device)
@@ -501,6 +507,22 @@
     _call("aicg_sine_source", _ptr(f0), _ptr(noise), _ptr(prefix), _ptr(out), t, int(upp), float(sr), sine_amp,
               noise_std, float(lin_w), float(lin_b), _stream(f0))
     return out
+
+
+def sine_source_window(f0, noise, upp, sr, lin_w, lin_b, first, count, sine_amp=0.1, noise_std=0.003):
+    f0 = f0.contiguous().float()
+    noise = noise.contiguous().float()
+    t = f0.numel()
+    first, count = int(first), int(count)
+    assert noise.numel() == t * upp and count >= 0
+    _check(f0, noise)
+    lead = first % 4 if upp % 4 == 0 else 0
+    n = -(-(lead + count) // 4) * 4 if upp % 4 == 0 else count
+    prefix = torch.empty(max(t, 1), dtype=torch.float64, device=f0.device)
+    out = torch.empty(n, dtype=torch.float32, device=f0.device)
+    _call("aicg_sine_source_window", _ptr(f0), _ptr(noise), _ptr(prefix), _ptr(out), t, int(upp), float(sr), sine_amp,
+              noise_std, float(lin_w), float(lin_b), first - lead, n, _stream(f0))
+    return out[lead: lead + count]
 
 
 def gate_tanh_sigmoid(a, out=None):
@@ -1220,5 +1242,6 @@
 attention = _staged("attention", attention, lambda a, k, r: (4.0 * a[0].numel() * a[0].shape[1],
                                                              4.0 * _numel(a[0], a[1], a[2], r)))
 sine_source = _staged("sine_source", sine_source, lambda a, k, r: (0.0, 4.0 * _numel(a[0], a[1], r)))
+sine_source_window = _staged("sine_source", sine_source_window, lambda a, k, r: (0.0, 4.0 * _numel(a[0], r, r)))
 layernorm_ct = _staged("layernorm", layernorm_ct, lambda a, k, r: (0.0, 4.0 * _numel(a[0], k.get("res"), r)))
 rownorm_act = _staged("groupnorm_gelu", rownorm_act, lambda a, k, r: (0.0, 4.0 * _numel(a[0], r)))
diff --git a/aicovergen_amd/vc_infer_pipeline.py b/aicovergen_amd/vc_infer_pipeline.py
--- a/aicovergen_amd/vc_infer_pipeline.py
+++ b/aicovergen_amd/vc_infer_pipeline.py
@@ -268,14 +268,14 @@
         return ops.f0_coarse(f0, factor, f0_mel_min, f0_mel_max)
 
     def vc(self, model, net_g, sid, audio0, pitch, pitchf, times, index, big_npy, index_rate, version, protect,
-           noise=None, keep_on_device=False):
+           noise=None, keep_on_device=False, trim=0):
         t0 = ttime()
         feats, feats0 = self._vc_features(model, audio0, index, big_npy, index_rate, version,
                                           protect < 0.5 and pitch is not None and pitchf is not None)
         if self._sync():
             torch.cuda.synchronize()
         t1 = ttime()
-        o = self._vc_synth(net_g, sid, audio0.shape[0], feats, feats0, pitch, pitchf, protect, noise)
+        o = self._vc_synth(net_g, sid, audio0.shape[0], feats, feats0, pitch, pitchf, protect, noise, trim)
         if keep_on_device:
             if self._sync():
                 torch.cuda.synchronize()
@@ -320,13 +320,18 @@
             feats = torch.from_numpy(npy.astype("float32")).unsqueeze(0).to(self.device) * index_rate + (1 - index_rate) * feats
         return feats, feats0
 
-    def _vc_synth(self, net_g, sid, n_samples, feats, feats0, pitch, pitchf, protect, noise):
-        return self._vc_synth_back(net_g, self._vc_synth_front(net_g, sid, n_samples, feats, feats0, pitch, pitchf, protect, noise))
-
-    def _vc_synth_back(self, net_g, st):
+    def _vc_synth(self, net_g, sid, n_samples, feats, feats0, pitch, pitchf, protect, noise, trim=0):
+        return self._vc_synth_back(net_g, self._vc_synth_front(net_g, sid, n_samples, feats, feats0, pitch, pitchf, protect, noise), trim)
+
+    def _vc_synth_back(self, net_g, st, trim=0):
         if "front" not in st:
-            return st["o"]
-        return net_g.infer_back(st["front"], st["pitchf"], st["ns"])[0]
+            o = st["o"]
+        else:
+            n = st["front"]["z"].shape[2] * net_g.upp
+            if trim and n > 2 * trim and _env.dev("AICG_SYNTH_WINDOW", "1") != "0":
+                return net_g.infer_back(st["front"], st["pitchf"], st["ns"], keep=(trim, n - trim))[0]
+            o = net_g.infer_back(st["front"], st["pitchf"], st["ns"])[0]
+        return o[:, :, trim: o.shape[2] - trim] if trim else o
 
     def _vc_synth_front(self, net_g, sid, n_samples, feats, feats0, pitch, pitchf, protect, noise):
         p_len = n_samples // self.window
@@ -528,23 +533,23 @@
         pc, pcf = c.chunk_pitch(ci)
         if not c.overlap:
             out = self.vc(c.model, c.net_g, c.sid, c.audio_pad[s:e], pc, pcf, c.times, c.index, c.big_npy, c.index_rate, c.version,
-                          c.protect, noise=c.noise(ci), keep_on_device=True)
+                          c.protect, noise=c.noise(ci), keep_on_device=True, trim=self.t_pad_tgt)
         else:
             noise = c.noise(ci) if front is None else None
             ts0 = ttime()
             if front is not None:
                 st, ev, keep = front
                 c.main.wait_event(ev)
-                out = self._vc_synth_back(c.net_g, st)[0, 0]
+                out = self._vc_synth_back(c.net_g, st, self.t_pad_tgt)[0, 0]
                 if after is not None:
                     self._queue_front(c, after)
             else:
                 feats, feats0 = c.feats_of.pop(ci)
                 c.wait_pitch(c.main, ci)
-                out = self._vc_synth(c.net_g, c.sid, e - s, feats, feats0, pc, pcf, c.protect, noise)[0, 0]
+                out = self._vc_synth(c.net_g, c.sid, e - s, feats, feats0, pc, pcf, c.protect, noise, self.t_pad_tgt)[0, 0]
             c.drain()
             c.times[2] += ttime() - ts0
-        c.pieces[ci] = out[self.t_pad_tgt: -self.t_pad_tgt]
+        c.pieces[ci] = out
         return c.pieces[ci]
 
     def _chunk_loop(self, c):
diff --git a/include/aicg.h b/include/aicg.h
--- a/include/aicg.h
+++ b/include/aicg.h
@@ -64,6 +64,8 @@
 int aicg_conv_desc_size(void);
 int aicg_conv_forward(const aicg_conv_desc* desc, const float* x, const float* w_packed, const float* bias,
                       const float* res, float* y, void* stream);
+int aicg_conv_forward_planned(const aicg_conv_desc* desc, const float* x, const float* w_packed, const float* bias,
+                              const float* res, float* y, int plan_w, void* stream);
 
 int aicg_col2im(const float* cols, const float* bias, const float* add, float* out, int N, int Cout, int Hi,
                 int Wi, int Ho, int Wo, int KH, int KW, int stride_h, int stride_w, int pad_h, int pad_w,
@@ -72,6 +74,9 @@
 
 int aicg_sine_source(const float* f0, const float* noise, double* prefix_scratch, float* out, int T, int upp,
                      float sr, float sine_amp, float noise_std, float lin_w, float lin_b, void* stream);
+int aicg_sine_source_window(const float* f0, const float* noise, double* prefix_scratch, float* out, int T, int upp,
+                            float sr, float sine_amp, float noise_std, float lin_w, float lin_b, int64_t first, int64_t count,
+                            void* stream);
 
 int aicg_gate_tanh_sigmoid(const float* a, float* out, int N, int C, int64_t T, void* stream);
 
```

Result: faster. 395.2, median of 6 (+2.5%).
